# lambdaclass/AES_zero_knowledge_proof_circuit

Measured on AMD Instinct MI355X. Metric: AES-ECB blocks proven/sec (Marlin), proof verifies, higher is better.
Workload: dtype u32 limbs (253-bit Fr / 377-bit Fq modular integers)

## Files before the change

aes_zero_knowledge_proof_circuit_amd/csrc/ff29.cuh:

```cuda
#pragma once
#include "ff.cuh"

namespace zk {

template <class P>
struct Fp29 {
    static constexpr int N = 9;
    static constexpr int B = 29;
    static constexpr uint32_t MASK = (1u << B) - 1;
    uint32_t l[N];

    ZK_HD static constexpr uint32_t mod29(int i) {
        int bit = B * i, w = bit >> 5, sh = bit & 31;
        uint64_t two = (w < P::N ? (uint64_t)P::mod(w) : 0) | ((w + 1 < P::N ? (uint64_t)P::mod(w + 1) : 0) << 32);
        return (uint32_t)(two >> sh) & MASK;
    }
    static constexpr uint32_t PINV = P::INV & MASK;
    template <int K> ZK_HD static constexpr uint32_t kp_limb(int i) {
        uint64_t c = 0, v = 0;
        for (int j = 0; j <= i; j++) { v = (uint64_t)K * mod29(j) + c; c = v >> B; }
        return i == N - 1 ? (uint32_t)v : (uint32_t)v & MASK;
    }
    template <int K> ZK_HD static constexpr uint32_t kp_spread(int i) {
        return i == 0 ? kp_limb<K>(0) + (1u << B) : (i == N - 1 ? kp_limb<K>(i) - 1u : kp_limb<K>(i) + MASK);
// ... 8 lines not shown
            uint64_t two = (k < P::N ? (uint64_t)w[k] : 0) | ((k + 1 < P::N ? (uint64_t)w[k + 1] : 0) << 32);
            r.l[i] = (uint32_t)(two >> sh) & MASK;
        }
        return r;
    }
    ZK_HD void pack(uint32_t *w) const {
#pragma unroll
        for (int k = 0; k < P::N; k++) {
            int bit = 32 * k, i = bit / B, sh = bit % B;
            uint64_t v = (uint64_t)l[i] >> sh;
            int have = B - sh;
            if (i + 1 < N) v |= (uint64_t)l[i + 1] << have;
            if (have + B < 32 && i + 2 < N) v |= (uint64_t)l[i + 2] << (have + B);
            w[k] = (uint32_t)v;
        }
    }
    ZK_HD Fp29 operator+(const Fp29 &b) const {
        Fp29 r;
        uint32_t c = 0;
#pragma unroll
        for (int i = 0; i < N - 1; i++) { uint32_t v = l[i] + b.l[i] + c; r.l[i] = v & MASK; c = v >> B; }
        r.l[N - 1] = l[N - 1] + b.l[N - 1] + c;
        return r;
    }
    template <int K>
    ZK_HD Fp29 sub(const Fp29 &b) const {
        Fp29 r;
        uint32_t c = 0;
#pragma unroll
        for (int i = 0; i < N - 1; i++) { uint32_t v = l[i] + kp_spread<K>(i) - b.l[i] + c; r.l[i] = v & MASK; c = v >> B; }
        r.l[N - 1] = l[N - 1] + kp_spread<K>(N - 1) - b.l[N - 1] + c;
        return r;
    }
    ZK_HD Fp29 add_lazy(const Fp29 &b) const { Fp29 r; for (int i = 0; i < N; i++) r.l[i] = l[i] + b.l[i]; return r; }
    template <int K> ZK_HD Fp29 sub_lazy(const Fp29 &b) const {
        Fp29 r;
#pragma unroll
        for (int i = 0; i < N; i++) {
#if defined(__HIP_DEVICE_COMPILE__)
            if (i < N - 1) { asm("v_sad_u32 %0, %1, %2, %3" : "=v"(r.l[i]) : "s"(kp_spread<K>(i)), "v"(b.l[i]), "v"(l[i])); continue; }
#endif
            r.l[i] = l[i] + kp_spread<K>(i) - b.l[i];
        }
        return r;
    }
    ZK_HD Fp29 normalized() const {
        Fp29 r;
        uint32_t c = 0;
#pragma unroll
        for (int i = 0; i < N - 1; i++) { const uint64_t v = (uint64_t)l[i] + c; r.l[i] = (uint32_t)v & MASK; c = (uint32_t)(v >> B); }
        r.l[N - 1] = l[N - 1] + c;
        return r;
    }
    ZK_HD Fp29 operator*(const Fp29 &b) const {
        uint64_t t[2 * N];
#pragma unroll
        for (int i = 0; i < 2 * N; i++) t[i] = 0;
#pragma unroll
        for (int i = 0; i < N; i++) {
#pragma unroll
            for (int j = 0; j < N; j++) t[i + j] += (uint64_t)l[j] * b.l[i];
            if constexpr (mod29(0) == 1u && PINV == MASK) {
                const uint64_t u = t[i] + MASK;
                const uint32_t m = ~(uint32_t)u & MASK;
#pragma unroll
                for (int j = 1; j < N; j++) t[i + j] += (uint64_t)m * mod29(j);
                t[i + 1] += u >> B;
            } else {
                uint32_t m = (((uint32_t)t[i] & MASK) * PINV) & MASK;
#pragma unroll
                for (int j = 0; j < N; j++) t[i + j] += (uint64_t)m * mod29(j);
                t[i + 1] += t[i] >> B;
            }
        }
        Fp29 r;
        uint64_t c = 0;
#pragma unroll
        for (int i = 0; i < N - 1; i++) { uint64_t v = t[N + i] + c; r.l[i] = (uint32_t)v & MASK; c = v >> B; }
        r.l[N - 1] = (uint32_t)(t[2 * N - 1] + c);
        return r;
    }
    template <int N>
    ZK_HD static Fp29 dot(const Fp29 *a, const Fp29 *b) {
        static_assert(N >= 1 && N <= 4, "column accumulators hold at most four products per limb pair");
        static_assert(mod29(0) == 1u && PINV == MASK, "written for p = 1 (mod 2^29)");
        uint64_t t[2 * Fp29::N];
#pragma unroll
        for (int i = 0; i < 2 * Fp29::N; i++) t[i] = 0;
#pragma unroll
        for (int i = 0; i < Fp29::N; i++) {
#pragma unroll
            for (int n = 0; n < N; n++)
#pragma unroll
                for (int j = 0; j < Fp29::N; j++) t[i + j] += (uint64_t)a[n].l[j] * b[n].l[i];
            const uint64_t u = t[i] + MASK;
            const uint32_t m = ~(uint32_t)u & MASK;
#pragma unroll
            for (int j = 1; j < Fp29::N; j++) t[i + j] += (uint64_t)m * mod29(j);
            t[i + 1] += u >> B;
        }
        Fp29 r;
        uint64_t c = 0;
#pragma unroll
        for (int i = 0; i < Fp29::N - 1; i++) { uint64_t v = t[Fp29::N + i] + c; r.l[i] = (uint32_t)v & MASK; c = v >> B; }
        r.l[Fp29::N - 1] = (uint32_t)(t[2 * Fp29::N - 1] + c);
        return r;
    }
    ZK_HD Fp29 shl5() const {
        Fp29 r;
        r.l[0] = (l[0] << 5) & MASK;
#pragma unroll
        for (int i = 1; i < N; i++) r.l[i] = ((l[i] << 5) | (l[i - 1] >> (B - 5))) & (i == N - 1 ? 0xffffffffu : MASK);
        return r;
    }
    template <int LOG>
    ZK_HD Fp29 canonical() const {
        Fp29 v = *this;
#pragma unroll
        for (int k = LOG; k >= 0; k--) {
            int64_t c = 0;
            uint32_t tl[N];
#pragma unroll
            for (int i = 0; i < N - 1; i++) { int64_t x = (int64_t)v.l[i] - ((int64_t)mod29(i) << k) + c; tl[i] = (uint32_t)x & MASK; c = x >> B; }
            int64_t top = (int64_t)v.l[N - 1] - ((int64_t)mod29(N - 1) << k) + c;
            if (top >= 0) {
#pragma unroll
                for (int i = 0; i < N - 1; i++) v.l[i] = tl[i];
                v.l[N - 1] = (uint32_t)top;
            }
        }
        return v;
    }
    ZK_HD Fp29 reduce_by_top_limb() const {
        constexpr uint32_t RECIP = (uint32_t)((1ull << 32) / ((uint64_t)mod29(N - 1) + 1));
        static_assert(mod29(N - 1) >= (1u << 20), "the estimate's error bound assumes a modulus of at least 253 bits");
        static_assert(P::mod(P::N - 1) < (1u << 31), "the callers pack a remainder < 2 p into 8 x 32-bit words: needs 2 p < 2^256");
#if defined(__HIP_DEVICE_COMPILE__)
        const uint32_t q = __umulhi(l[N - 1], RECIP);
#else
        const uint32_t q = (uint32_t)(((uint64_t)l[N - 1] * RECIP) >> 32);
#endif
        Fp29 r;
        int64_t c = 0;
#pragma unroll
        for (int i = 0; i < N - 1; i++) { const int64_t x = (int64_t)l[i] - (int64_t)((uint64_t)q * mod29(i)) + c; r.l[i] = (uint32_t)x & MASK; c = x >> B; }
        r.l[N - 1] = (uint32_t)((int64_t)l[N - 1] - (int64_t)((uint64_t)q * mod29(N - 1)) + c);
        return r;
    }
    ZK_HD static Fp29 twiddle_from_std(const Fp<P> &w) {
        Fp<P> v = w;
        for (int i = 0; i < 261 - 32 * P::N; i++) v = v.dbl();
        return split(v.l);
    }
    ZK_HD static Fp29 from_std_relimb(const Fp<P> &a) { return split(a.l); }
    template <int LOG> ZK_HD Fp<P> to_std_relimb() const { Fp<P> r; canonical<LOG>().pack(r.l); return r; }
};

}
```

aes_zero_knowledge_proof_circuit_amd/csrc/gpu.hpp:

```cpp
#pragma once
#include <cstddef>
#include <cstdint>
#include <stdexcept>
#include <string>
#include <utility>
#include <vector>
#include "ec.cuh"
#include "te28.cuh"

namespace zk {
namespace gpu {

struct GpuError : std::runtime_error { using std::runtime_error::runtime_error; };
typedef void *stream_t;

int device_count();
void require_device();
int current_device();
void set_device(int ordinal);
void *dmalloc(size_t bytes);
#ifdef ZKAES_MEASURE
int knockin();
#endif
size_t mem_free_bytes();
void dfree(void *p);
void h2d(void *dst, const void *src, size_t bytes, stream_t s);
void d2h(void *dst, const void *src, size_t bytes, stream_t s);
void d2d(void *dst, const void *src, size_t bytes, stream_t s);
void dzero(void *dst, size_t bytes, stream_t s);
void sync(stream_t s);
bool throughput_mode();
struct ThroughputWaits { explicit ThroughputWaits(bool on); ~ThroughputWaits(); ThroughputWaits(const ThroughputWaits &) = delete; ThroughputWaits &operator=(const ThroughputWaits &) = delete; private: bool on_; };
stream_t stream_create();
stream_t stream_create_background();
void stream_destroy(stream_t s);
void *event_create();
void event_record(void *ev, stream_t s);
void stream_wait_event(stream_t s, void *ev);
float event_elapsed_ms(void *start, void *stop);
void event_destroy(void *ev);

void *pinned_alloc(size_t bytes);
void *pinned_device_address(void *host);
void pinned_free(void *host);

template <class T> struct DevElem { static constexpr size_t bytes = sizeof(T); };
template <> struct DevElem<void> { static constexpr size_t bytes = 1; };
template <class T> struct DevPtr {
    T *p = nullptr;
    size_t n = 0;
    DevPtr() = default;
    explicit DevPtr(size_t count) { alloc(count); }
    DevPtr(const DevPtr &) = delete; DevPtr &operator=(const DevPtr &) = delete;
    DevPtr(DevPtr &&o) noexcept : p(o.p), n(o.n) { o.p = nullptr; o.n = 0; }
    DevPtr &operator=(DevPtr &&o) noexcept { if (this != &o) { reset(); p = o.p; n = o.n; o.p = nullptr; o.n = 0; } return *this; }
    ~DevPtr() { dfree(p); }
    void reset() { dfree(p); p = nullptr; n = 0; }
    void alloc(size_t count) { reset(); p = (T *)dmalloc(count * DevElem<T>::bytes); n = count; }
    void grow(size_t count) { if (!p || count > n) alloc(count); }
    T *get() const { return p; }
    operator T *() const { return p; }
};
template <class... T> void grow_together(const size_t (&counts)[sizeof...(T)], DevPtr<T> &...bufs) {
    size_t i = 0;
    if (((bufs.p && counts[i++] <= bufs.n) && ...)) return;
    (bufs.reset(), ...);
    i = 0;
    try { (bufs.alloc(counts[i++]), ...); } catch (...) { (bufs.reset(), ...); throw; }
}
template <class H, H (*Create)(), void (*Destroy)(H)> struct Handle {
    H h = nullptr;
    Handle() : h(Create()) {}
    explicit Handle(H adopt) : h(adopt) {}
    Handle(const Handle &) = delete; Handle &operator=(const Handle &) = delete;
    Handle(Handle &&o) noexcept : h(o.h) { o.h = nullptr; }
    Handle &operator=(Handle &&o) noexcept { if (this != &o) { Destroy(h); h = o.h; o.h = nullptr; } return *this; }
    ~Handle() { Destroy(h); }
    operator H() const { return h; }
};
using StreamGuard = Handle<stream_t, stream_create, stream_destroy>;
using EventGuard = Handle<void *, event_create, event_destroy>;
struct PinnedPtr {
    void *host = nullptr, *dev = nullptr;
    PinnedPtr() = default;
    PinnedPtr(const PinnedPtr &) = delete; PinnedPtr &operator=(const PinnedPtr &) = delete;
    ~PinnedPtr() { pinned_free(host); }
    void alloc(size_t bytes) { pinned_free(host); host = dev = nullptr; host = pinned_alloc(bytes); dev = pinned_device_address(host); }
};

enum : int { OP_MSM_BUCKETS = 0, OP_MSM_SECOND_BASES = 1, OP_MSM_CLASS_SUM = 2 };
struct OpRecord { std::vector<std::pair<uint64_t, int>> ntt , msm ; };
void oplog_begin();
OpRecord oplog_end();
void oplog_ntt(uint64_t n, int count);
void oplog_msm(uint64_t points, int kind);

template <class Fr> void ntt(Fr *dst, const Fr *src, size_t in_len, int lg, bool inverse, stream_t s);
template <class Fr> void ntt_coset(Fr *dst, const Fr *src, size_t in_len, int lg, bool inverse, int coset_c, int lg_big, stream_t s);
template <class Fr> struct NttJob { Fr *dst; const Fr *src; int coset_c; };
template <class Fr> void ntt_batch(const NttJob<Fr> *jobs, int count, size_t in_len, int lg, bool inverse, int lg_big, stream_t s);
template <class Fr> DevPtr<void> coset_power_table(const Fr &g, size_t n, stream_t s);
template <class Fr> void ntt_scaled(Fr *dst, const Fr *src, size_t in_len, int lg, bool inverse, const void *table, stream_t s);
template <class Fr> const Fr *domain_elements(int lg);

struct MsmWorkspace;
MsmWorkspace *msm_workspace_create();
void msm_workspace_destroy(MsmWorkspace *ws);
using WorkspaceGuard = Handle<MsmWorkspace *, msm_workspace_create, msm_workspace_destroy>;
template <class Curve> void convert_bases(Affine28<typename Curve::FqP> *dst, const Affine<typename Curve::Fq> *src, size_t n, stream_t s);
template <class Curve>
XYZZ<typename Curve::Fq> msm(MsmWorkspace *ws, const Affine28<typename Curve::FqP> *bases, const typename Curve::Fr *scalars, size_t n, stream_t s);
template <class Curve>
void msm_prepare(MsmWorkspace *ws, const typename Curve::Fr *scal1, size_t n1, const typename Curve::Fr *scal2, size_t n2, size_t val_off2, stream_t s, int force_c = 0);
template <class Curve>
XYZZ<typename Curve::Fq> msm_finish(MsmWorkspace *ws, const Affine28<typename Curve::FqP> *bases, stream_t s);
template <class Curve> void convert_bases_te(Niels28<typename Curve::FqP> *dst, const Affine<typename Curve::Fq> *src, size_t n, stream_t s);
template <class Curve>
XYZZ<typename Curve::Fq> msm(MsmWorkspace *ws, const Niels28<typename Curve::FqP> *bases, const typename Curve::Fr *scalars, size_t n, stream_t s);
template <class Curve>
XYZZ<typename Curve::Fq> msm_finish(MsmWorkspace *ws, const Niels28<typename Curve::FqP> *bases, stream_t s);
template <class Curve>
void msm_finish2(MsmWorkspace *ws, const Niels28<typename Curve::FqP> *bases, const Niels28<typename Curve::FqP> *bases2, XYZZ<typename Curve::Fq> *out, stream_t s);
template <class Curve>
XYZZ<typename Curve::Fq> msm_table(MsmWorkspace *ws, const Niels28<typename Curve::FqP> *tables, size_t stride, size_t off, int c, const typename Curve::Fr *scalars, size_t n, stream_t s);
template <class Curve>
bool class_sum(MsmWorkspace *ws, const Niels28<typename Curve::FqP> *bases, const int8_t *vals, size_t n, XYZZ<typename Curve::Fq> *out, stream_t s);
template <class Curve> void msm_sharded_plan(size_t n_total, int *window_bits, int *n_windows);
template <class Curve>
void msm_window_sums_device(MsmWorkspace *ws, const Affine28<typename Curve::FqP> *bases, const typename Curve::Fr *scalars, size_t n_local, size_t n_total,
                            XYZZ<typename Curve::Fq> *dev_out, stream_t s);
template <class Curve>
XYZZ<typename Curve::Fq> msm_fold_window_sums_device(const XYZZ<typename Curve::Fq> *dev_in, int world, size_t n_total, stream_t s);
template <class Curve>
void msm_table_sum_device(MsmWorkspace *ws, const Niels28<typename Curve::FqP> *tables, size_t stride, size_t off, int c, const typename Curve::Fr *scalars, size_t n,
                          XYZZ<typename Curve::Fq> *dev_out, stream_t s);
template <class Curve>
XYZZ<typename Curve::Fq> msm_fold_points_device(const XYZZ<typename Curve::Fq> *dev_in, int world, stream_t s);
template <class Curve> int table_windows(int c);
template <class Curve> void build_window_tables(Affine<typename Curve::Fq> *tables, size_t stride, int c, stream_t s);
template <class Curve> void table_next(Affine<typename Curve::Fq> *next, const Affine<typename Curve::Fq> *prev, size_t count, int c, int j, stream_t s);
template <class Curve>
void msm_prepare_table(MsmWorkspace *ws, const typename Curve::Fr *scal1, size_t n1, size_t off1, const typename Curve::Fr *scal2, size_t n2, size_t off2, int c, size_t stride, stream_t s);
template <class Curve>
XYZZ<typename Curve::Fq> msm_table(MsmWorkspace *ws, const Affine28<typename Curve::FqP> *tables, size_t stride, size_t off, int c, const typename Curve::Fr *scalars, size_t n, stream_t s);
template <class Curve>
void fixed_base_powers(Affine<typename Curve::Fq> *out, const Affine<typename Curve::Fq> &base, const typename Curve::Fr &beta, size_t from, size_t count, stream_t s, size_t chunk = 0);
template <class Curve>
void fixed_base_scalars(Affine<typename Curve::Fq> *out, const Affine<typename Curve::Fq> &base, const typename Curve::Fr *scalars, size_t count, stream_t s, size_t chunk = 0);
template <class Curve>
bool class_sum(MsmWorkspace *ws, const Affine28<typename Curve::FqP> *bases, const int8_t *vals, size_t n, XYZZ<typename Curve::Fq> *out, stream_t s);
struct MsmStats { double accumulate_ms = 0; double total_ms = 0; uint64_t points = 0; uint64_t launches = 0; uint64_t pairs = 0; };
MsmStats msm_stats(bool reset);

}
}

namespace zk {
struct G1Compressed;
namespace gpu {
using F = Fr377;

void g1_decompress_check(const G1Compressed *pts, size_t n, Affine<Fq377> *out, uint8_t *status, stream_t s);
void fq_sqrt_batch(const Fq377 *in, size_t n, Fq377 *out, uint8_t *ok, stream_t s);
void public_input_eval(F *out, const F *betas, const uint32_t *bits, size_t words, size_t n, size_t n_bits, int lg_m, const F &gx, stream_t s);

void poly_set_at(F *p, size_t idx, const F &val, stream_t s);
void poly_add_at(F *p, size_t idx, const F &val, stream_t s);
void poly_scale(F *p, const F &sc, size_t n, stream_t s);
void poly_lincomb_n(F *out, size_t n, const F *const *polys, const size_t *lens, const F *scalars, int count, stream_t s);
size_t divide_by_vanishing_scratch(size_t len, size_t m);
void divide_by_vanishing(F *q, F *rem, const F *p, size_t len, size_t m, stream_t s, F *scratch = nullptr, size_t scratch_len = 0);
void divide_by_linear(F *q, const F *p, size_t len, const F &z, F *scratch, size_t scratch_elems, stream_t s);
size_t divide_by_linear_scratch(size_t len);
F poly_eval(const F *p, size_t len, const F &x, F *scratch, stream_t s);
size_t poly_eval_scratch(size_t len);
void poly_eval_multi(const F *const *p, const size_t *len, const F *x, int count, F *out, F *scratch, size_t scratch_elems, stream_t s);
void batch_inverse(F *v, size_t n, const F *post_or_null, stream_t s);
size_t vanishing_quotient_scratch(int lg_n, int ncosets);
void vanishing_quotient_evals(F *const *out, const F *g, int ncosets, const F &a, const F *elems, uint32_t n, int lg_n, F *scratch, size_t scratch_elems, stream_t s);
void f_evals_from_tables(F *out, const F *va, const F *vb, const F *vc, const F &ea, const F &eb, const F &ec, const F *ra, const F *rb, const uint32_t *ri, const uint32_t *ci, size_t k,
                         stream_t s);

void upload_sbox(const uint8_t table[256]);
void aes_trace(uint8_t *trace, size_t trace_stride, const uint8_t *msgs, const uint8_t *keys, uint32_t nproofs, uint32_t nblocks, stream_t s, size_t key_bytes = 16);
void aes_trace_cbc(uint8_t *trace, size_t trace_stride, const uint8_t *msgs, const uint8_t *keys, const uint8_t *ivs, uint32_t nproofs, uint32_t nblocks, stream_t s, size_t key_bytes = 16);
void aes_trace_ctr(uint8_t *trace, size_t trace_stride, const uint8_t *msgs, const uint8_t *keys, const uint8_t *icbs, uint32_t nproofs, uint32_t msg_len, stream_t s, size_t key_bytes = 16);
void aes_trace_gcm(uint8_t *trace, size_t trace_stride, const uint8_t *msgs, const uint8_t *keys, const uint8_t *hdrs, uint32_t nproofs, uint32_t msg_len, uint32_t aad_len, stream_t s, size_t key_bytes = 16);
void ghash_trace(uint8_t *trace, size_t trace_stride, uint32_t nproofs, uint32_t msg_len, uint32_t aad_len, stream_t s, size_t key_bytes = 16);
void key_tag_trace(uint8_t *trace, size_t trace_stride, size_t tag_off, const uint8_t *keys, uint32_t nproofs, uint32_t tag_blocks, stream_t s, size_t key_bytes = 16);
void sha256_trace(uint8_t *trace, size_t trace_stride, size_t digest_off, const uint8_t *msgs, const uint8_t *hdrs, size_t hdr_stride, size_t hin_off, uint32_t nproofs, size_t msg_len, int digest_kind,
                  uint64_t digest_prefix, stream_t s);
void aes_trace_gcm_seg(uint8_t *trace, size_t trace_stride, const uint8_t *msgs, const uint8_t *keys, const uint8_t *hdrs, uint32_t nproofs, int role, uint32_t msg_len, uint32_t aad_len, stream_t s,
                       size_t key_bytes = 16);
void ghash_trace_seg(uint8_t *trace, size_t trace_stride, uint32_t nproofs, int role, uint32_t msg_len, uint32_t aad_len, stream_t s, size_t key_bytes = 16);
void commit_trace(uint8_t *trace, size_t trace_stride, size_t seg_off, size_t yout_off, const uint8_t *keys, size_t key_bytes, const uint8_t *hdrs, size_t hdr_stride, uint32_t nproofs, int role,
                  uint32_t nblocks, stream_t s);
void witness_expand(uint8_t *z, const uint32_t *desc, uint32_t ncols, const uint8_t *trace, const uint32_t *sbox_in_off, const uint32_t *sbox_tmpl, stream_t s);
void spmv_bits(F *out, int8_t *small_out, size_t rows_out, const uint32_t *rowptr, const uint32_t *col, const int64_t *coeff, size_t rows, const uint8_t *z, stream_t s);
void w_classes(int8_t *out, const uint8_t *z, uint32_t n, uint32_t m, uint32_t num_witness, stream_t s);
void lagrange_scalars(F *lag, F *lag_w, const F *elems, const F &beta, uint32_t n, uint32_t m, stream_t s);
void w_evals(F *out, const uint8_t *z, const F *x_evals, uint32_t n, uint32_t m, uint32_t num_witness, stream_t s);
void bits_to_field(F *out, const uint8_t *z, size_t n, stream_t s);
constexpr uint32_t T_SEG = 32, T_HEAVY_SEGMENTS = 256;
void t_evals(F *out, uint32_t n, F *partial, uint32_t nseg, const uint32_t *col_seg_ptr, const uint32_t *seg_start, const uint32_t *seg_end, const uint32_t *heavy, uint32_t n_heavy,
             const uint32_t *row, const uint8_t *mat, const int64_t *coeff, const F *r_alpha, const F &eta_a, const F &eta_b, const F &eta_c, stream_t s);
uint64_t chacha_field_stream(F *out, size_t count, const uint32_t key[8], int rounds, uint64_t word_pos, void *scratch, size_t scratch_bytes, stream_t s, uint32_t max_cand = 0);
void mask_fixup(F *p, size_t n, stream_t s);
void q1_coset_pointwise(F *out, const F *r, const F *za, const F *zb, const F *t, const F *z, const F &ca, const F &cb, const F &cz, const F &eta_a, const F &eta_b, const F &eta_c,
                        size_t n, stream_t s);
void z_evals_h(F *out, const uint8_t *z, uint32_t n, uint32_t m, uint32_t num_witness, stream_t s);
void q1_combine(F *h1, F *g1, const F *q0, const F *q1, const F *q3, const F *mask, const F &inv2, const F &inv2zeta, size_t n, stream_t s);
void coset_scale(F *out, const F *in, const F &g, size_t in_len, size_t n, stream_t s);
void h2_coset(F *out, const F *row, const F *col, const F *va, const F *vb, const F *vc, const F *rc, const F *f, const F &alpha, const F &beta, const F &alpha_beta,
              const F &ea, const F &eb, const F &ec, const F &vinv, size_t k, stream_t s);
void index_evals(F *row, F *col, F *rowcol, F *va, F *vb, F *vc, F *tmp, const uint32_t *ci, const uint32_t *ri, const int64_t *ca, const int64_t *cb, const int64_t *cc, size_t cnt,
                 size_t k, const F *elems, uint32_t n, stream_t s);
void z_poly_from_w(F *zp, const F *w, size_t wlen, const F *x_poly, uint32_t m, size_t n, stream_t s);

}
}
```

aes_zero_knowledge_proof_circuit_amd/csrc/kernels_msm.hip:

```cpp
#include <cstring>
#include <rocprim/device/device_radix_sort.hpp>
#include <rocprim/device/device_scan.hpp>
#include <chrono>
#include <cstdio>
#include <cstdlib>
#include <mutex>
#include <vector>
#include "hip_util.hpp"
#include "te28.cuh"

namespace zk {
namespace gpu {

template <class P> struct WeierLaw { using Params = P; using Base = Affine28<P>; using Acc = Acc28<P>; static constexpr bool edwards = false; };
template <class P> struct EdwardsLaw { using Params = P; using Base = Niels28<P>; using Acc = AccTE<P>; static constexpr bool edwards = true; };

static MsmStats g_stats;
static std::mutex g_stats_mu;
MsmStats msm_stats(bool reset) {
    std::lock_guard<std::mutex> g(g_stats_mu);
    MsmStats s = g_stats;
    if (reset) g_stats = MsmStats();
    return s;
}

constexpr uint32_t VAL_SKIP = 1u << 30, VAL_INDEX = VAL_SKIP - 1;
template <class Fr>
__global__ void k_digits(const Fr *__restrict__ scalars, uint32_t n, uint32_t i_off, uint32_t ntot, uint32_t val_off, int c, int nwin, uint32_t nb,
                         uint32_t *__restrict__ keys, uint32_t *__restrict__ vals) {
    uint32_t i = blockIdx.x * blockDim.x + threadIdx.x;
    if (i >= n) return;
    uint32_t raw[Fr::N + 1];
    scalars[i].to_raw(raw);
    raw[Fr::N] = 0;
    const uint32_t mask = (1u << c) - 1, half = 1u << (c - 1);
    uint32_t carry = 0;
    for (int w = 0; w < nwin; w++) {
        int bit = w * c, limb = bit >> 5, sh = bit & 31;
        uint64_t two = limb <= Fr::N - 1 ? ((uint64_t)raw[limb] | ((uint64_t)raw[limb + 1] << 32)) : 0;
        uint32_t v = ((uint32_t)(two >> sh) & mask) + carry;
        uint32_t neg = 0;
        carry = 0;
        if (v > half) { v = (1u << c) - v; neg = 1u << 31; carry = 1; }
        keys[(size_t)w * ntot + i_off + i] = ((uint32_t)w << (c - 1)) | (v ? v - 1 : 0u);
        vals[(size_t)w * ntot + i_off + i] = v ? ((val_off + i) | neg) : VAL_SKIP;
    }
}

struct TableLayout {
    int nwin, c_hi, n_hi;
    __host__ __device__ int width(int j) const { return j < n_hi ? c_hi : c_hi - 1; }
    __host__ __device__ int offset(int j) const { return j < n_hi ? j * c_hi : n_hi * c_hi + (j - n_hi) * (c_hi - 1); }
};
static TableLayout table_layout(int total_bits, int c) {
    TableLayout L;
    L.nwin = (total_bits + c - 1) / c;
    int base = total_bits / L.nwin, rem = total_bits % L.nwin;
    L.c_hi = base + (rem ? 1 : 0);
    L.n_hi = rem ? rem : L.nwin;
    return L;
}
template <class Fr>
__global__ void k_digits_table(const Fr *__restrict__ scalars, uint32_t n, uint32_t i_off, uint32_t ntot, uint32_t val_off, TableLayout L, uint32_t stride,
                               uint32_t *__restrict__ keys, uint32_t *__restrict__ vals) {
    uint32_t i = blockIdx.x * blockDim.x + threadIdx.x;
    if (i >= n) return;
    uint32_t raw[Fr::N + 1];
    scalars[i].to_raw(raw);
    raw[Fr::N] = 0;
    uint32_t carry = 0;
    for (int w = 0; w < L.nwin; w++) {
        const int c = L.width(w), bit = L.offset(w), limb = bit >> 5, sh = bit & 31;
        const uint32_t mask = (1u << c) - 1, half = 1u << (c - 1);
        uint64_t two = limb <= Fr::N - 1 ? ((uint64_t)raw[limb] | ((uint64_t)raw[limb + 1] << 32)) : 0;
        uint32_t v = ((uint32_t)(two >> sh) & mask) + carry;
        uint32_t neg = 0;
        carry = 0;
        if (v > half) { v = (1u << c) - v; neg = 1u << 31; carry = 1; }
        keys[(size_t)w * ntot + i_off + i] = v ? v - 1 : 0u;
        vals[(size_t)w * ntot + i_off + i] = v ? (((uint32_t)w * stride + val_off + i) | neg) : VAL_SKIP;
    }
}
template <class Fq>
__global__ void __launch_bounds__(64) k_table_next(const Affine<Fq> *__restrict__ prev, Affine<Fq> *__restrict__ next, uint32_t count, int c) {
    constexpr int B = 8;
    uint32_t t = blockIdx.x * blockDim.x + threadIdx.x;
    uint32_t s0 = t * B;
    if (s0 >= count) return;
    uint32_t e = s0 + B < count ? s0 + B : count;
    Fq xs[B], ys[B], zz[B], zzz[B], pre[B];
    Fq acc = Fq::one();
    for (uint32_t i = s0; i < e; i++) {
        XYZZ<Fq> p = XYZZ<Fq>::from_affine(prev[i]);
        for (int k = 0; k < c; k++) p = p.dbl();
        xs[i - s0] = p.x; ys[i - s0] = p.y; zz[i - s0] = p.zz; zzz[i - s0] = p.zzz;
        pre[i - s0] = acc;
        if (!p.zzz.is_zero()) acc = acc * p.zzz;
    }
    acc = acc.inverse();
    for (uint32_t i = e; i-- > s0;) {
        uint32_t q = i - s0;
        if (zzz[q].is_zero()) { next[i] = Affine<Fq>::inf(); continue; }
        Fq zi3 = acc * pre[q];
        acc = acc * zzz[q];
        Fq zi2 = (zi3 * zz[q]).sqr();
        Affine<Fq> a; a.x = xs[q] * zi2; a.y = ys[q] * zi3;
        next[i] = a;
    }
}

__device__ __forceinline__ uint32_t bounds_rank(uint32_t key, int cbits, uint32_t nwin) { return nwin == 1 ? key : (key & ((1u << cbits) - 1)) * nwin + (key >> cbits); }
__device__ __forceinline__ uint32_t bounds_key(uint32_t rank, int cbits, uint32_t nwin) { return nwin == 1 ? rank : ((rank % nwin) << cbits) | (rank / nwin); }
__global__ void k_bounds(const uint32_t *__restrict__ keys, size_t total, int cbits, uint32_t nwin, uint32_t *__restrict__ start, uint32_t *__restrict__ end) {
    size_t i0 = ((size_t)blockIdx.x * blockDim.x + threadIdx.x) * 4;
    if (i0 >= total) return;
    const uint32_t nb = nwin << cbits;
    uint32_t k[6];
    if (i0 + 4 <= total) { uint4 v = *reinterpret_cast<const uint4 *>(keys + i0); k[1] = v.x; k[2] = v.y; k[3] = v.z; k[4] = v.w; }
    else { for (int j = 0; j < 4; j++) k[1 + j] = i0 + j < total ? keys[i0 + j] : 0u; }
    k[0] = i0 ? keys[i0 - 1] : 0u;
    k[5] = i0 + 4 < total ? keys[i0 + 4] : 0u;
#pragma unroll
    for (int j = 0; j < 4; j++) {
        size_t i = i0 + j;
        if (i >= total) break;
        const uint32_t key = k[1 + j];
        if (i == 0 || k[j] != key) {
            const uint32_t r1 = bounds_rank(key, cbits, nwin);
            uint32_t r0 = 0;
            if (i != 0) { end[k[j]] = (uint32_t)i; r0 = bounds_rank(k[j], cbits, nwin) + 1; }
            for (uint32_t r = r0; r < r1; r++) { const uint32_t g = bounds_key(r, cbits, nwin); start[g] = (uint32_t)i; end[g] = (uint32_t)i; }
            start[key] = (uint32_t)i;
        }
        if (i + 1 == total) {
            end[key] = (uint32_t)total;
            for (uint32_t r = bounds_rank(key, cbits, nwin) + 1; r < nb; r++) { const uint32_t g = bounds_key(r, cbits, nwin); start[g] = (uint32_t)total; end[g] = (uint32_t)total; }
        }
    }
}

template <class P>
__global__ void k_convert_bases(const Affine<Fp<P>> *__restrict__ src, Affine28<P> *__restrict__ dst, size_t n) {
    size_t i = (size_t)blockIdx.x * blockDim.x + threadIdx.x;
    if (i < n) dst[i] = Affine28<P>::from_std(src[i]);
}

constexpr uint32_t BUCKET_CAP = 2048, BUCKET_CAP_TABLE = 512;
constexpr uint32_t NO_SLOT = 0xffffffffu;

constexpr int ORD_BINS = 1024, ORD_THREADS = 256, ORD_MAX_BLOCKS = 128;
__device__ __forceinline__ uint32_t order_key(uint32_t sz) { return (ORD_BINS - 1) - (sz > ORD_BINS - 1 ? ORD_BINS - 1 : sz); }
__global__ void __launch_bounds__(ORD_THREADS) k_order_hist(const uint32_t *__restrict__ start, const uint32_t *__restrict__ end, uint32_t nb, uint32_t per_block, uint32_t cap,
                                                             uint32_t *__restrict__ ovf_slot, uint32_t *__restrict__ ovf_bucket, uint32_t *__restrict__ ovf_nseg, uint32_t ovf_cap,
                                                             uint32_t *__restrict__ ctrl, uint32_t *__restrict__ hist) {
    __shared__ uint32_t h[ORD_BINS];
    for (int b = threadIdx.x; b < ORD_BINS; b += ORD_THREADS) h[b] = 0;
    __syncthreads();
    const uint32_t lo = blockIdx.x * per_block, hi = lo + per_block < nb ? lo + per_block : nb;
    for (uint32_t k = lo + threadIdx.x; k < hi; k += ORD_THREADS) {
        const uint32_t sz = end[k] - start[k];
        uint32_t slot = NO_SLOT;
        if (sz > cap) {
// ... 211 lines not shown
    } else {
        if (threadIdx.x != 0) return;
        accumulate_fixup<P>(bases, buckets, deferred, deferred_cap, deferred_count);
    }
}
template <class A>
__global__ void __launch_bounds__(64) k_fold_overflow(A *__restrict__ buckets, const uint32_t *__restrict__ ctrl, const uint32_t *__restrict__ ovf_bucket, const uint32_t *__restrict__ ovf_off,
                                                       uint32_t max_segments, const A *__restrict__ partial) {
    const uint32_t q = blockIdx.x * blockDim.x + threadIdx.x;
    if (q >= ctrl[1]) return;
    uint32_t a = ovf_off[q], b = ovf_off[q + 1];
    if (b > max_segments) b = max_segments;
    if (a >= b) return;
    const uint32_t k = ovf_bucket[q];
    A acc = buckets[k];
    for (uint32_t w = a / 64; w * 64 < b; w++) { uint32_t i = w * 64 > a ? w * 64 : a; if (i < b) PtOps<A>::add(acc, partial[i]); }
    buckets[k] = acc;
}

constexpr int RED_L1 = 8, RED_L2 = 8;
template <class A>
__global__ void __launch_bounds__(64) k_reduce_l1(const A *__restrict__ buckets, int c, int nwin, A *__restrict__ seg_s, A *__restrict__ seg_w) {
    uint32_t segs = (1u << c) / RED_L1;
    uint32_t t = blockIdx.x * blockDim.x + threadIdx.x;
    if (t >= segs * (uint32_t)nwin) return;
    uint32_t w = t / segs, g = t % segs;
    const size_t k0 = ((size_t)w << c) + (size_t)g * RED_L1;
    A run = buckets[k0 + RED_L1 - 1], tot = run;
    for (int d = RED_L1 - 2; d >= 0; d--) {
        A b = buckets[k0 + d];
        if (d != RED_L1 - 2) PtOps<A>::add_inline(tot, run);
        PtOps<A>::add_inline(run, b);
    }
    PtOps<A>::add(tot, run);
    seg_s[t] = run;
    seg_w[t] = tot;
}
template <class A>
__global__ void __launch_bounds__(64) k_reduce_l1_pair(const A *__restrict__ buckets, int c, int nwin, A *__restrict__ seg_s, A *__restrict__ seg_w) {
    using P = typename PtOps<A>::Params;
    using G = FpMsm<P>;
    const uint32_t segs = (1u << c) / RED_L1;
    const uint32_t t = blockIdx.x * blockDim.x + threadIdx.x, seg = t >> 1;
    const bool odd = t & 1;
    if (seg >= segs * (uint32_t)nwin) return;
    const uint32_t w = seg / segs, g = seg % segs;
    const size_t k0 = ((size_t)w << c) + g;
    A acc = odd ? PtOps<A>::identity() : buckets[k0 + (size_t)(RED_L1 - 1) * segs];
    for (int d = RED_L1 - 2; d >= 0; d--) {
        A opnd;
        opnd.x = quad_move<QP_SWAP_PAIRS, G>(acc.x); opnd.y = quad_move<QP_SWAP_PAIRS, G>(acc.y); opnd.z = quad_move<QP_SWAP_PAIRS, G>(acc.z); opnd.t = quad_move<QP_SWAP_PAIRS, G>(acc.t);
        if (!odd) opnd = buckets[k0 + (size_t)d * segs];
        PtOps<A>::add_inline(acc, opnd);
    }
    (odd ? seg_w : seg_s)[seg] = acc;
}
template <class A>
__global__ void __launch_bounds__(64) k_reduce_l2(const A *__restrict__ seg_s, const A *__restrict__ seg_w, int c, int nwin, A *__restrict__ partial) {
    uint32_t segs = (1u << c) / RED_L1, groups = (segs + RED_L2 - 1) / RED_L2;
    const uint32_t role = blockIdx.x & 1;
    uint32_t t = (blockIdx.x >> 1) * blockDim.x + threadIdx.x;
    if (t >= groups * (uint32_t)nwin) return;
    uint32_t w = t / groups, h = t % groups;
    uint32_t g0 = h * RED_L2, g1 = g0 + RED_L2 < segs ? g0 + RED_L2 : segs;
    const A *S = seg_s + (size_t)w * segs, *W = seg_w + (size_t)w * segs;
    A *out = partial + (size_t)w * 2 * groups + 2 * h + role;
    if (role == 0) {
        A run = PtOps<A>::identity(), tot2 = PtOps<A>::identity(), sw = PtOps<A>::identity();
        for (int g = (int)g1 - 1; g >= (int)g0; g--) {
            PtOps<A>::add(run, S[g]);
            PtOps<A>::add(tot2, run);
            PtOps<A>::add(sw, W[g]);
        }
        A a = tot2;
        PtOps<A>::add(a, PtOps<A>::neg(run));
        for (int i = 0; i < 3; i++) PtOps<A>::dbl(a);
        PtOps<A>::add(sw, a);
        *out = sw;
    } else {
        A acc = PtOps<A>::identity();
        if (g0 != 0) {
            A run = PtOps<A>::identity();
            for (int g = (int)g1 - 1; g >= (int)g0; g--) PtOps<A>::add(run, S[g]);
            uint32_t m = RED_L1 * g0;
            int top = 31 - __clz(m);
            for (int bit = top; bit >= 0; bit--) {
                PtOps<A>::dbl(acc);
                if ((m >> bit) & 1) PtOps<A>::add(acc, run);
            }
        }
        *out = acc;
    }
}

template <class A>
__global__ void __launch_bounds__(256) k_reduce_window(const A *__restrict__ partial, uint32_t per_window, XYZZ<Fp<typename PtOps<A>::Params>> *__restrict__ out,
                                                        XYZZ<Fp<typename PtOps<A>::Params>> *__restrict__ out2) {
    __shared__ A sh[256];
    uint32_t w = blockIdx.x, t = threadIdx.x;
    A acc = PtOps<A>::identity();
    for (uint32_t i = t; i < per_window; i += 256) PtOps<A>::add(acc, partial[(size_t)w * per_window + i]);
    sh[t] = acc;
    __syncthreads();
    int s0 = 128;
    while (s0 >= 1 && (uint32_t)s0 >= per_window) s0 >>= 1;
    for (int s = s0; s > 0; s >>= 1) {
        if ((int)t < s) { A a = sh[t]; PtOps<A>::add(a, sh[t + s]); sh[t] = a; }
        __syncthreads();
    }
    if (t == 0) {
        const auto r = PtOps<A>::to_std(sh[0]);
        out[w] = r;
        if (out2) out2[w] = r;
    }
}

constexpr int RQ_THREADS = 256, RQ_QUADS = RQ_THREADS / 4;
constexpr int PT_WORDS = 4 * FpMsm<Fq377P>::N;
template <class P> __device__ __forceinline__ FpMsm<P> quad_load(const uint32_t *pt, int q) {
    FpMsm<P> r;
#pragma unroll
    for (int i = 0; i < FpMsm<P>::N; i++) r.l[i] = pt[q * FpMsm<P>::N + i];
    return r;
}
template <class P> __device__ __forceinline__ void quad_store(uint32_t *pt, int q, const FpMsm<P> &v) {
#pragma unroll
    for (int i = 0; i < FpMsm<P>::N; i++) pt[q * FpMsm<P>::N + i] = v.l[i];
}
template <class P>
__device__ __forceinline__ void quad_tree_sum(uint32_t *pt, uint32_t count, uint32_t quad, int q) {
    for (uint32_t half = count >> 1; half >= 1; half >>= 1) {
        if (quad < half) quad_store<P>(pt + quad * PT_WORDS, q, te_add_quad<P>(quad_load<P>(pt + quad * PT_WORDS, q), quad_load<P>(pt + (quad + half) * PT_WORDS, q), q));
        __syncthreads();
    }
}
template <class P>
__global__ void __launch_bounds__(RQ_THREADS) k_reduce_rc(const AccTE<P> *__restrict__ seg_s, const AccTE<P> *__restrict__ seg_w, int lgR, int lgC, AccTE<P> *__restrict__ out) {
    __shared__ uint32_t pt[RQ_QUADS * PT_WORDS];
    const uint32_t R = 1u << lgR, C = 1u << lgC, jobs = 2 * R + C;
    const uint32_t set = blockIdx.x / jobs, job = blockIdx.x % jobs, quad = threadIdx.x >> 2;
    const int q = threadIdx.x & 3;
    const AccTE<P> *src = (job < R ? seg_w : seg_s) + ((size_t)set << (lgR + lgC));
    uint32_t first, stride, len;
    if (job < 2 * R) { first = (job < R ? job : job - R) << lgC; stride = 1; len = C; }
    else { first = job - 2 * R; stride = C; len = R; }
    FpMsm<P> acc = te_identity_quad<P>(q);
    for (uint32_t i = quad; i < len; i += RQ_QUADS)
        acc = te_add_quad<P>(acc, quad_load<P>(reinterpret_cast<const uint32_t *>(src + first + (size_t)i * stride), q), q);
    quad_store<P>(pt + quad * PT_WORDS, q, acc);
    __syncthreads();
    quad_tree_sum<P>(pt, RQ_QUADS, quad, q);
    if (quad == 0) quad_store<P>(reinterpret_cast<uint32_t *>(out + (size_t)set * jobs + job), q, quad_load<P>(pt, q));
}
ZK_HD int quad_weighted_lc(uint32_t M) { int m = 0; while ((1u << m) < M) m++; return M <= 16 ? m : (m + 1) / 2; }
constexpr int RF_OUT = 6;
constexpr int RT_THREADS = 256, RT_QUADS = RT_THREADS / 4;
constexpr int RT_PLANES = RT_QUADS, RT_IDENT = RT_QUADS + 32, RT_SLOTS = RT_IDENT + 1;
__device__ __forceinline__ uint32_t rt_plane_member(uint32_t b, uint32_t i) {
    const uint32_t lo = i & ((1u << b) - 1), hi = i >> b;
    return (hi << (b + 1)) | (1u << b) | lo;
}
template <class P>
__global__ void __launch_bounds__(RT_THREADS) k_reduce_terms(const AccTE<P> *__restrict__ rc, int lgR, int lgC, AccTE<P> *__restrict__ part, XYZZ<Fp<P>> *__restrict__ out, bool to_host) {
    __shared__ uint32_t pt[RT_SLOTS * PT_WORDS];
    const uint32_t R = 1u << lgR, C = 1u << lgC, jobs = 2 * R + C;
    const uint32_t set = blockIdx.x / RF_OUT, term = blockIdx.x % RF_OUT, quad = threadIdx.x >> 2;
    const int q = threadIdx.x & 3;
    const bool plain = term < 2, second = term & 1;
    const AccTE<P> *src = rc + (size_t)set * jobs + (term == 0 ? 0 : (term == 2 || term == 3) ? 2 * R : R);
    const uint32_t M = (term == 2 || term == 3) ? C : R;
    uint32_t first = 0, stride = 0, count = 0;
    if (plain) { first = quad; stride = RT_QUADS; count = quad < M ? (M - quad + RT_QUADS - 1) / RT_QUADS : 0; }
    else {
        const int lc = quad_weighted_lc(M);
        const uint32_t c1 = 1u << lc, r1 = M >> lc, G = second ? r1 : c1, S = second ? c1 : r1, g = quad >> 2, p = quad & 3;
        if (g < G && p < S) { count = (S - p + 3) / 4; first = second ? g * c1 + p : p * c1 + g; stride = second ? 4 : 4 * c1; }
    }
    FpMsm<P> acc = te_identity_quad<P>(q);
    for (uint32_t i = 0; i < count; i++) acc = te_add_quad<P>(acc, quad_load<P>(reinterpret_cast<const uint32_t *>(src + first + (size_t)i * stride), q), q);
    quad_store<P>(pt + quad * PT_WORDS, q, acc);
    if (quad == 0) quad_store<P>(pt + RT_IDENT * PT_WORDS, q, te_identity_quad<P>(q));
    __syncthreads();
    const int nsteps = plain ? 6 : 11;
    for (int step = 0; step < nsteps; step++) {
        bool active = false;
        uint32_t dst = 0, a = 0, b = 0;
        if (plain) { const uint32_t half = (RT_QUADS / 2) >> step; active = quad < half; dst = a = quad; b = quad + half; }
        else if (step == 0) { active = (quad & 3) < 2; dst = a = quad; b = quad + 2; }
        else if (step == 1) { active = (quad & 3) == 0; dst = a = quad; b = quad + 1; }
        else if (step == 2) { active = quad < 16; const uint32_t pl = quad >> 2, j = quad & 3; dst = RT_PLANES + 8 * pl + j; a = 4 * rt_plane_member(pl, 2 * j); b = 4 * rt_plane_member(pl, 2 * j + 1); }
        else if (step == 3) { active = quad < 8; const uint32_t pl = quad >> 1, j = quad & 1; dst = a = RT_PLANES + 8 * pl + j; b = a + 2; }
        else if (step == 4) { active = quad < 4; dst = a = RT_PLANES + 8 * quad; b = a + 1; }
        else { active = quad == 0; dst = a = RT_PLANES + 24; const int h = step - 5; b = (h & 1) ? RT_PLANES + 8 * (2 - h / 2) : a; }
        if (active) quad_store<P>(pt + dst * PT_WORDS, q, te_add_quad<P>(quad_load<P>(pt + a * PT_WORDS, q), quad_load<P>(pt + b * PT_WORDS, q), q));
        __syncthreads();
    }
    const uint32_t *res = pt + (plain ? 0 : RT_PLANES + 24) * PT_WORDS;
    if (to_host) { if (threadIdx.x == 0) out[(size_t)set * RF_OUT + term] = te_to_std_point<P>(*reinterpret_cast<const AccTE<P> *>(res)); }
    else if (quad == 0) quad_store<P>(reinterpret_cast<uint32_t *>(part + (size_t)set * RF_OUT + term), q, quad_load<P>(res, q));
}
template <class P>
__global__ void __launch_bounds__(64) k_reduce_combine(const AccTE<P> *__restrict__ part, int lgR, int lgC, XYZZ<Fp<P>> *__restrict__ out, XYZZ<Fp<P>> *__restrict__ dev_total) {
    __shared__ uint32_t pt[RF_OUT * PT_WORDS];
    __shared__ uint8_t prog[64][3];
    __shared__ int nprog;
    const uint32_t set = blockIdx.x, quad = threadIdx.x >> 2;
    const int q = threadIdx.x & 3;
    if (quad < RF_OUT) quad_store<P>(pt + quad * PT_WORDS, q, quad_load<P>(reinterpret_cast<const uint32_t *>(part + (size_t)set * RF_OUT + quad), q));
    if (threadIdx.x == 0) {
        int n = 0;
        auto op = [&](int d, int a, int b) { prog[n][0] = (uint8_t)d; prog[n][1] = (uint8_t)a; prog[n][2] = (uint8_t)b; n++; };
        const int lcC = quad_weighted_lc(1u << lgC), lcR = quad_weighted_lc(1u << lgR);
        for (int i = 0; i < lcR; i++) op(5, 5, 5);
        op(5, 5, 4);
        for (int i = 0; i < lcC; i++) op(3, 3, 3);
        op(3, 3, 2);
        for (int i = 0; i < lgR; i++) op(0, 0, 0);
        op(0, 0, 5);
        for (int i = 0; i < lgC; i++) op(0, 0, 0);
        op(0, 0, 3); op(0, 0, 1);
        nprog = n;
    }
    __syncthreads();
    const int n = nprog;
    for (int i = 0; i < n; i++) {
        const FpMsm<P> v = te_add_quad<P>(quad_load<P>(pt + prog[i][1] * PT_WORDS, q), quad_load<P>(pt + prog[i][2] * PT_WORDS, q), q);
        __syncthreads();
        if (quad == 0) quad_store<P>(pt + prog[i][0] * PT_WORDS, q, v);
        __syncthreads();
    }
    if (threadIdx.x == 0) {
        const auto r = te_to_std_point<P>(*reinterpret_cast<const AccTE<P> *>(pt));
        out[set] = r;
        if (dev_total) dev_total[set] = r;
    }
}
template <class Fq>
static XYZZ<Fq> reduce_host_tail(const XYZZ<Fq> *o, int lgR, int lgC) {
    auto shl = [](XYZZ<Fq> v, int k) { for (int i = 0; i < k; i++) v = v.dbl(); return v; };
    const int lcC = quad_weighted_lc(1u << lgC), lcR = quad_weighted_lc(1u << lgR);
    XYZZ<Fq> row = shl(o[5], lcR);
    row.add(o[4]);
    XYZZ<Fq> col = shl(o[3], lcC);
    col.add(o[2]);
    XYZZ<Fq> t = shl(o[0], lgR);
    t.add(row);
    t = shl(t, lgC);
    t.add(col);
    t.add(o[1]);
    return t;
}

template <class A> __global__ void k_sum_tree(const A *__restrict__ in, uint32_t total, uint32_t per, A *__restrict__ out, uint32_t in_stride, uint32_t out_stride);

constexpr uint32_t DEFERRED_CAP = 1u << 20;
constexpr size_t ACC_BYTES = sizeof(Acc28<Fq377P>);
static_assert(sizeof(Acc28<Fq381P>) == ACC_BYTES, "bucket size differs between the curves");
static_assert(sizeof(AccTE<Fq377P>) == ACC_BYTES, "the Edwards accumulator must fit the XYZZ bucket slots");
constexpr int MAX_WSUMS = 64;
struct MsmWorkspace {
    DevPtr<uint32_t> keys_a, keys_b, vals_a, vals_b;
    uint32_t *sorted_keys = nullptr, *sorted_vals = nullptr;
    DevPtr<uint32_t> start, end, order, ovf_slot;
    DevPtr<uint32_t> ovf_bucket, ovf_nseg, ovf_off; DevPtr<void> ovf_partial;
    DevPtr<uint32_t> part_hist, part_offs;
    DevPtr<uint32_t> canon;
    DevPtr<void> buckets, seg_s, seg_w, partial;
    DevPtr<void> tmp;
    bool ctrl_dirty = false;
    size_t plan_n = 0, plan_pairs = 0; int plan_c = 0, plan_nwin = 0;
    bool plan_table = false; uint32_t plan_cap = BUCKET_CAP;
    EventGuard ev[4] = {EventGuard(nullptr), EventGuard(nullptr), EventGuard(nullptr), EventGuard(nullptr)};
    DevPtr<uint32_t> deferred, deferred_count;
    DevPtr<uint32_t> ord_hist, ord_offs;
    DevPtr<uint32_t> ctrl;
    PinnedPtr h_res;
};
constexpr size_t RES_BYTES = 192 * MAX_WSUMS * 6 + 64;
static void ensure_result(MsmWorkspace &S, size_t buckets) {
    grow_together({buckets * ACC_BYTES, (buckets / RED_L1 + 64) * ACC_BYTES, (buckets / RED_L1 + 64) * ACC_BYTES, (2 * (buckets / (RED_L1 * RED_L2)) + 2 * 64 * 64) * ACC_BYTES},
                  S.buckets, S.seg_s, S.seg_w, S.partial);
}
static void ensure_scratch(MsmWorkspace &S, size_t pairs, size_t buckets, size_t cap) {
    if (cap == 0) cap = BUCKET_CAP;
    if (!S.h_res.dev) {
        for (auto &e : S.ev) e = EventGuard();
        S.deferred.alloc(2 * DEFERRED_CAP); S.deferred_count.alloc(2);
        HIP_CHECK(hipMemset(S.deferred_count, 0, 8));
        S.ord_hist.alloc((size_t)ORD_BINS * ORD_MAX_BLOCKS); S.ord_offs.alloc((size_t)ORD_BINS * ORD_MAX_BLOCKS);
        S.ctrl.alloc(8);
        HIP_CHECK(hipMemset(S.ctrl, 0, 32));
        S.h_res.alloc(RES_BYTES);
    }
    const size_t ovf = pairs / cap + 64;
    grow_together({2 * ovf * ACC_BYTES , ovf, ovf, ovf + 1}, S.ovf_partial, S.ovf_bucket, S.ovf_nseg, S.ovf_off);
    grow_together({pairs, pairs, pairs, pairs}, S.keys_a, S.keys_b, S.vals_a, S.vals_b);
    grow_together({buckets, buckets, buckets, buckets}, S.start, S.end, S.order, S.ovf_slot);
    ensure_result(S, buckets);
}
MsmWorkspace *msm_workspace_create() { return new MsmWorkspace(); }
void msm_workspace_destroy(MsmWorkspace *w) { delete w; }

static void order_buckets(MsmWorkspace &S, size_t nb, uint32_t cap, hipStream_t s) {
    if (S.ctrl_dirty) HIP_CHECK(hipMemsetAsync(S.ctrl, 0, 8, s));
    S.ctrl_dirty = true;
    unsigned nblk = (unsigned)((nb + 4095) / 4096);
    if (nblk > (unsigned)ORD_MAX_BLOCKS) nblk = ORD_MAX_BLOCKS;
    if (nblk < 1) nblk = 1;
    const uint32_t per_block = (uint32_t)((nb + nblk - 1) / nblk);
    hipLaunchKernelGGL(k_order_hist, dim3(nblk), dim3(ORD_THREADS), 0, s, S.start, S.end, (uint32_t)nb, per_block, cap, S.ovf_slot, S.ovf_bucket, S.ovf_nseg, (uint32_t)S.ovf_bucket.n - 1, S.ctrl, S.ord_hist);
    HIP_LAUNCH_CHECK();
    hipLaunchKernelGGL(k_order_scan, dim3(1), dim3(ORD_BINS), 0, s, S.ord_hist, S.ord_offs, nblk, S.ctrl, S.ovf_nseg, S.ovf_off, (uint32_t)S.ovf_bucket.n - 1);
    HIP_LAUNCH_CHECK();
    hipLaunchKernelGGL(k_order_scatter, dim3(nblk), dim3(ORD_THREADS), 0, s, S.start, S.end, (uint32_t)nb, per_block, S.ord_offs, S.order);
    HIP_LAUNCH_CHECK();
    S.ctrl_dirty = false;
}

template <class P>
static void prepare_buckets(MsmWorkspace &S, size_t pairs, int c, int nsets, int sort_bits, uint32_t cap, hipStream_t s, int begin_bit = 0) {
    size_t nb = (size_t)nsets << c;
    int key_bits = 1;
    while (((size_t)1 << key_bits) < nb) key_bits++;
    if (sort_bits > 0 && sort_bits < key_bits) key_bits = sort_bits;
    size_t tmp_bytes = 0;
    rocprim::double_buffer<uint32_t> dk(S.keys_a, S.keys_b), dv(S.vals_a, S.vals_b);
    HIP_CHECK(rocprim::radix_sort_pairs(nullptr, tmp_bytes, dk, dv, pairs, (unsigned)begin_bit, (unsigned)key_bits, s));
    S.tmp.grow(tmp_bytes);
    HIP_CHECK(rocprim::radix_sort_pairs(S.tmp.p, tmp_bytes, dk, dv, pairs, (unsigned)begin_bit, (unsigned)key_bits, s));
#ifdef ZKAES_MEASURE
    if (knockin() & 1) HIP_CHECK(rocprim::radix_sort_pairs(S.tmp.p, tmp_bytes, dk, dv, pairs, (unsigned)begin_bit, (unsigned)key_bits, s));
#endif
    S.sorted_keys = dk.current(); S.sorted_vals = dv.current();
    hipLaunchKernelGGL(k_bounds, dim3((unsigned)(((pairs + 3) / 4 + 255) / 256)), dim3(256), 0, s, S.sorted_keys, pairs, c, (uint32_t)nsets, S.start, S.end);
    HIP_LAUNCH_CHECK();
    order_buckets(S, nb, cap, s);
}
template <class Law>
static std::vector<XYZZ<Fp<typename Law::Params>>> run_buckets(MsmWorkspace &S, const typename Law::Base *bases, size_t pairs, int c, int nsets_one, size_t n_points, uint32_t cap, hipStream_t s, float *acc_ms,
                                            XYZZ<Fp<typename Law::Params>> *dev_wsum_out = nullptr, const typename Law::Base *bases2 = nullptr) {
    using P = typename Law::Params;
    using A = typename Law::Acc;
    using Fq = Fp<P>;
    const int nrep = bases2 ? 2 : 1, nsets = nsets_one * nrep;
    if (bases2 && !Law::edwards) throw GpuError("msm: two base arrays per prepared state need the Edwards law");
    if (nsets > MAX_WSUMS) throw GpuError("msm: too many windows");
    const size_t nb = (size_t)nsets_one << c;
    ensure_result(S, nb * nrep);
    if constexpr (!Law::edwards) HIP_CHECK(hipMemsetAsync(S.deferred_count, 0, 8, s));
#ifdef ZKAES_MEASURE
    if (knockin() & 8) {
        hipLaunchKernelGGL((k_accumulate<Law>), dim3((unsigned)((nb + 63) / 64)), dim3(64), 0, s, bases, S.sorted_vals, S.start, S.end, S.order, (uint32_t)nb, cap,
                           (A *)S.buckets.p, S.deferred, DEFERRED_CAP, S.deferred_count);
        if constexpr (!Law::edwards) HIP_CHECK(hipMemsetAsync(S.deferred_count, 0, 8, s));
    }
#endif
    uint32_t max_seg = (uint32_t)(pairs / cap + 1);
    for (int rep = 0; rep < nrep; rep++) {
        const typename Law::Base *src = rep ? bases2 : bases;
        HIP_CHECK(hipEventRecord((hipEvent_t)S.ev[2 * rep].h, s));
        hipLaunchKernelGGL((k_accumulate<Law>), dim3((unsigned)((nb + 63) / 64)), dim3(64), 0, s, src, S.sorted_vals, S.start, S.end, S.order, (uint32_t)nb, cap,
                           (A *)S.buckets.p + rep * nb, S.deferred, DEFERRED_CAP, S.deferred_count);
        HIP_LAUNCH_CHECK();
        HIP_CHECK(hipEventRecord((hipEvent_t)S.ev[2 * rep + 1].h, s));
        hipLaunchKernelGGL((k_accumulate_tail<Law>), dim3((max_seg + 63) / 64), dim3(64), 0, s, src, S.sorted_vals, S.start, S.end, S.ctrl, S.ovf_bucket, S.ovf_off, max_seg, cap,
                           (A *)S.ovf_partial.p + rep * S.ovf_bucket.n, (A *)S.buckets.p + rep * nb, S.deferred, DEFERRED_CAP, S.deferred_count);
        HIP_LAUNCH_CHECK();
    }
    if constexpr (!Law::edwards) for (int rep = 0; rep < nrep; rep++) {
        hipLaunchKernelGGL((k_fold_overflow<A>), dim3((max_seg + 63) / 64), dim3(64), 0, s, (A *)S.buckets.p + rep * nb, S.ctrl, S.ovf_bucket, S.ovf_off, max_seg, (const A *)S.ovf_partial.p + rep * S.ovf_bucket.n);
        HIP_LAUNCH_CHECK();
    }
    XYZZ<Fq> *res = (XYZZ<Fq> *)S.h_res.dev;
    uint32_t segs = (1u << c) / RED_L1, groups = (segs + RED_L2 - 1) / RED_L2;
    [[maybe_unused]] int te_lgR = 0, te_lgC = 0;
    [[maybe_unused]] bool te_host_tail = false;
#ifdef ZKAES_MEASURE
    for (int rep = (knockin() & 2) ? 0 : 1; rep < 2; rep++)
#endif
    {
    if constexpr (Law::edwards)
        hipLaunchKernelGGL((k_reduce_l1_pair<A>), dim3((unsigned)((2 * segs * nsets + 63) / 64)), dim3(64), 0, s, (const A *)S.buckets.p, c, nsets, (A *)S.seg_s.p, (A *)S.seg_w.p);
    else
        hipLaunchKernelGGL((k_reduce_l1<A>), dim3((unsigned)((segs * nsets + 63) / 64)), dim3(64), 0, s, (const A *)S.buckets.p, c, nsets, (A *)S.seg_s.p, (A *)S.seg_w.p);
    HIP_LAUNCH_CHECK();
    if constexpr (Law::edwards) {
        const int lgG = c - 3 > 0 ? c - 3 : 0, lgC = (lgG + 1) / 2, lgR = lgG - lgC;
        if (lgC > 8) throw GpuError("msm: more than 2^19 buckets per set");
        const unsigned jobs = 2u * (1u << lgR) + (1u << lgC);
        A *rc = (A *)S.partial.p, *part = rc + (size_t)nsets * jobs;
        hipLaunchKernelGGL((k_reduce_rc<P>), dim3((unsigned)nsets * jobs), dim3(RQ_THREADS), 0, s, (const A *)S.seg_s.p, (const A *)S.seg_w.p, lgR, lgC, rc);
        HIP_LAUNCH_CHECK();
        te_host_tail = !dev_wsum_out && nsets <= 4;
        hipLaunchKernelGGL((k_reduce_terms<P>), dim3((unsigned)(RF_OUT * nsets)), dim3(RT_THREADS), 0, s, (const A *)rc, lgR, lgC, part, res, te_host_tail);
        HIP_LAUNCH_CHECK();
        if (!te_host_tail) {
            hipLaunchKernelGGL((k_reduce_combine<P>), dim3((unsigned)nsets), dim3(64), 0, s, (const A *)part, lgR, lgC, res, dev_wsum_out);
            HIP_LAUNCH_CHECK();
        }
        te_lgR = lgR; te_lgC = lgC;
    } else {
    hipLaunchKernelGGL((k_reduce_l2<A>), dim3(2u * (unsigned)((groups * nsets + 63) / 64)), dim3(64), 0, s, (const A *)S.seg_s.p, (const A *)S.seg_w.p, c, nsets, (A *)S.partial.p);
    HIP_LAUNCH_CHECK();
    const uint32_t parts = 2 * groups;
    if (nsets == 1 && parts > 2048) {
        uint32_t mid = (parts + 255) / 256;
        hipLaunchKernelGGL((k_sum_tree<A>), dim3(mid), dim3(256), 0, s, (const A *)S.partial.p, parts, 256u, (A *)S.seg_s.p, 0u, 0u);
        HIP_LAUNCH_CHECK();
        hipLaunchKernelGGL((k_reduce_window<A>), dim3(1), dim3(256), 0, s, (const A *)S.seg_s.p, mid, res, dev_wsum_out);
    } else {
        hipLaunchKernelGGL((k_reduce_window<A>), dim3((unsigned)nsets), dim3(256), 0, s, (const A *)S.partial.p, parts, res, dev_wsum_out);
    }
    HIP_LAUNCH_CHECK();
    }
    }
    std::vector<XYZZ<Fq>> ws(nsets);
    uint32_t n_deferred = 0;
    sync((stream_t)s);
    if (Law::edwards && te_host_tail) {
        std::vector<XYZZ<Fq>> terms((size_t)nsets * RF_OUT);
        memcpy(terms.data(), S.h_res.host, sizeof(XYZZ<Fq>) * terms.size());
        for (int i = 0; i < nsets; i++) ws[i] = reduce_host_tail<Fq>(terms.data() + (size_t)i * RF_OUT, te_lgR, te_lgC);
    } else memcpy(ws.data(), S.h_res.host, sizeof(XYZZ<Fq>) * nsets);
    if constexpr (!Law::edwards) {
        HIP_CHECK(hipMemcpyAsync(&n_deferred, S.deferred_count, 4, hipMemcpyDeviceToHost, s));
        sync((stream_t)s);
        if (n_deferred > DEFERRED_CAP) throw GpuError("msm: more than 2^20 degenerate additions (repeated base points); refusing to return a wrong sum");
    }
    for (int rep = 0; rep < nrep; rep++) HIP_CHECK(hipEventElapsedTime(acc_ms + rep, (hipEvent_t)S.ev[2 * rep].h, (hipEvent_t)S.ev[2 * rep + 1].h));
    (void)n_points;
    return ws;
}
static void add_stats(const float *acc_ms, int launches, size_t n, size_t pairs, std::chrono::steady_clock::time_point t_begin) {
    std::lock_guard<std::mutex> g(g_stats_mu);
    for (int i = 0; i < launches; i++) g_stats.accumulate_ms += acc_ms[i];
    g_stats.points += n * (size_t)launches;
    g_stats.pairs += pairs * (size_t)launches;
    g_stats.launches += (uint64_t)launches;
    g_stats.total_ms += std::chrono::duration<double, std::milli>(std::chrono::steady_clock::now() - t_begin).count();
}

__global__ void __launch_bounds__(64) k_convert_bases_te(const Affine<Fq377> *__restrict__ src, Niels28<Fq377P> *__restrict__ dst, size_t n, uint32_t *__restrict__ bad) {
    constexpr int B = 8;
    size_t s0 = ((size_t)blockIdx.x * blockDim.x + threadIdx.x) * B;
    if (s0 >= n) return;
    size_t e = s0 + B < n ? s0 + B : n;
    TeMapParts m[B];
    Fq377 pre[B];
    bool skip[B];
    Fq377 acc = Fq377::one();
    for (size_t i = s0; i < e; i++) {
        Affine<Fq377> p = src[i];
        int q = (int)(i - s0);
        skip[q] = p.is_inf();
        if (!skip[q]) {
            m[q] = te_map_parts(p);
            if (m[q].den.is_zero()) { skip[q] = true; atomicOr(bad, 1u); }
        }
        pre[q] = acc;
        if (!skip[q]) acc = acc * m[q].den;
    }
    acc = acc.inverse();
    for (size_t i = e; i-- > s0;) {
        int q = (int)(i - s0);
        if (skip[q]) { dst[i] = niels_identity<Fq377P>(); continue; }
        Fq377 inv = acc * pre[q];
        acc = acc * m[q].den;
        dst[i] = te_niels_finish(m[q], inv);
    }
}
template <class Curve>
void convert_bases_te(Niels28<typename Curve::FqP> *dst, const Affine<typename Curve::Fq> *src, size_t n, stream_t s_) {
    static_assert(Curve::ID == 377, "only BLS12-377's G1 has a twisted Edwards model");
    if (!n) return;
    hipStream_t s = (hipStream_t)s_;
    DevPtr<uint32_t> d_bad(1);
    uint32_t h_bad = 0;
    HIP_CHECK(hipMemsetAsync(d_bad, 0, 4, s));
    size_t lanes = (n + 7) / 8;
    hipLaunchKernelGGL(k_convert_bases_te, dim3((unsigned)((lanes + 63) / 64)), dim3(64), 0, s, src, dst, n, d_bad.get());
    HIP_LAUNCH_CHECK();
    sync((stream_t)s);
    HIP_CHECK(hipMemcpyAsync(&h_bad, d_bad, 4, hipMemcpyDeviceToHost, s));
    sync((stream_t)s);
    if (h_bad) throw GpuError("convert_bases_te: a base point has order 2 or 4 -- the Edwards path needs points of the prime-order subgroup");
}
template void convert_bases_te<Bls377>(Niels28<Fq377P> *, const Affine<Fq377> *, size_t, stream_t);

template <class Curve>
void convert_bases(Affine28<typename Curve::FqP> *dst, const Affine<typename Curve::Fq> *src, size_t n, stream_t s_) {
    if (!n) return;
    hipLaunchKernelGGL((k_convert_bases<typename Curve::FqP>), dim3((unsigned)((n + 255) / 256)), dim3(256), 0, (hipStream_t)s_, src, dst, n);
    HIP_LAUNCH_CHECK();
}

template <class Curve>
void msm_prepare(MsmWorkspace *ws_, const typename Curve::Fr *scal1, size_t n1, const typename Curve::Fr *scal2, size_t n2, size_t val_off2, stream_t s_, int force_c) {
    using Fr = typename Curve::Fr;
    hipStream_t s = (hipStream_t)s_;
    if (!ws_) throw GpuError("msm: null workspace");
    MsmWorkspace &S = *ws_;
    size_t n = n1 + n2;
    S.plan_n = n;
    if (n == 0) return;
    if (n >= (1u << 30) || val_off2 + n2 >= (1u << 30)) throw GpuError("msm: too many points");
    int lg = 0;
    while (((size_t)1 << lg) < n) lg++;
    int c = lg - 2;
    if (c < 7) c = 7;
    if (c > 17) c = 17;
    if (force_c >= 4 && force_c <= 22) c = force_c;
    const int nwin = (Fr::BITS + 1 + c - 1) / c;
    size_t pairs = n * (size_t)nwin;
    if (pairs >= ((size_t)1 << 31)) throw GpuError("msm: n x windows exceeds the 2^31 pairs the sort indexes with int");
    const size_t nb = (size_t)nwin << (c - 1);
    S.plan_c = c; S.plan_nwin = nwin; S.plan_pairs = pairs; S.plan_table = false; S.plan_cap = BUCKET_CAP;
    ensure_scratch(S, pairs, nb, BUCKET_CAP);
    if (n1) { hipLaunchKernelGGL((k_digits<Fr>), dim3((unsigned)((n1 + 255) / 256)), dim3(256), 0, s, scal1, (uint32_t)n1, 0u, (uint32_t)n, 0u, c, nwin, (uint32_t)nb, S.keys_a, S.vals_a); HIP_LAUNCH_CHECK(); }
    if (n2) { hipLaunchKernelGGL((k_digits<Fr>), dim3((unsigned)((n2 + 255) / 256)), dim3(256), 0, s, scal2, (uint32_t)n2, (uint32_t)n1, (uint32_t)n, (uint32_t)val_off2, c, nwin, (uint32_t)nb, S.keys_a, S.vals_a); HIP_LAUNCH_CHECK(); }
    prepare_buckets<typename Curve::FqP>(S, pairs, c - 1, nwin, c - 1, BUCKET_CAP, s);
}
template <class Curve, class Law>
static XYZZ<typename Curve::Fq> msm_finish_impl(MsmWorkspace *ws_, const typename Law::Base *bases, stream_t s_, const typename Law::Base *bases2 = nullptr,
                                                XYZZ<typename Curve::Fq> *out2 = nullptr) {
    using Fq = typename Curve::Fq;
    static_assert(sizeof(XYZZ<Fq>) == 192, "XYZZ layout");
    hipStream_t s = (hipStream_t)s_;
    if (!ws_) throw GpuError("msm: null workspace");
    MsmWorkspace &S = *ws_;
    if (out2) *out2 = XYZZ<Fq>::inf();
    if (S.plan_n == 0) return XYZZ<Fq>::inf();
    auto t_begin = std::chrono::steady_clock::now();
    const int c = S.plan_c, nwin = S.plan_nwin;
    oplog_msm(S.plan_n, OP_MSM_BUCKETS);
    if (bases2) oplog_msm(S.plan_n, OP_MSM_SECOND_BASES);
    float ms[2] = {0, 0};
    if (S.plan_table) {
        std::vector<XYZZ<Fq>> one = run_buckets<Law>(S, bases, S.plan_pairs, c - 1, 1, S.plan_n, S.plan_cap, s, ms, nullptr, bases2);
        add_stats(ms, bases2 ? 2 : 1, S.plan_n, S.plan_pairs, t_begin);
        if (bases2) *out2 = one[1];
        return one[0];
    }
    if (bases2 && 2 * nwin > MAX_WSUMS) {
        *out2 = msm_finish_impl<Curve, Law>(ws_, bases2, s_);
// ... 64 lines not shown
        sync((stream_t)s);
        return;
    }
    msm_prepare<Curve>(ws_, scalars, n_local, nullptr, 0, 0, s_, c);
    MsmWorkspace &S = *ws_;
    if (S.plan_nwin != nwin) throw GpuError("msm_window_sums_device: window plan mismatch");
    float ms = 0;
    auto t_begin = std::chrono::steady_clock::now();
    oplog_msm(n_local, OP_MSM_BUCKETS);
    run_buckets<WeierLaw<typename Curve::FqP>>(S, bases, S.plan_pairs, c - 1, nwin, n_local, S.plan_cap, s, &ms, dev_out);
    add_stats(&ms, 1, n_local, S.plan_pairs, t_begin);
}
template <class Fq>
__global__ void k_fold_ranks(const XYZZ<Fq> *__restrict__ in, int world, int nwin, XYZZ<Fq> *__restrict__ out) {
    int w = blockIdx.x * blockDim.x + threadIdx.x;
    if (w >= nwin) return;
    XYZZ<Fq> acc = in[w];
    for (int r = 1; r < world; r++) acc.add(in[(size_t)r * nwin + w]);
    out[w] = acc;
}
template <class Curve>
XYZZ<typename Curve::Fq> msm_fold_window_sums_device(const XYZZ<typename Curve::Fq> *dev_in, int world, size_t n_total, stream_t s_) {
    using Fq = typename Curve::Fq;
    hipStream_t s = (hipStream_t)s_;
    int c, nwin;
    msm_sharded_plan<Curve>(n_total, &c, &nwin);
    DevPtr<XYZZ<Fq>> d_out((size_t)nwin);
    hipLaunchKernelGGL((k_fold_ranks<Fq>), dim3(1), dim3(64), 0, s, dev_in, world, nwin, d_out.get());
    HIP_LAUNCH_CHECK();
    std::vector<XYZZ<Fq>> ws(nwin);
    sync((stream_t)s);
    HIP_CHECK(hipMemcpyAsync(ws.data(), d_out, sizeof(XYZZ<Fq>) * nwin, hipMemcpyDeviceToHost, s));
    sync((stream_t)s);
    XYZZ<Fq> total = XYZZ<Fq>::inf();
    for (int w = nwin - 1; w >= 1; w--) {
        total.add(ws[w]);
        for (int k = 0; k < c; k++) total = total.dbl();
    }
    total.add(ws[0]);
    return total;
}

template <class Curve>
void msm_table_sum_device(MsmWorkspace *ws_, const Niels28<typename Curve::FqP> *tables, size_t stride, size_t off, int c, const typename Curve::Fr *scalars, size_t n,
                          XYZZ<typename Curve::Fq> *dev_out, stream_t s_) {
    using Fq = typename Curve::Fq;
    hipStream_t s = (hipStream_t)s_;
    if (n == 0) {
        HIP_CHECK(hipMemsetAsync(dev_out, 0, sizeof(XYZZ<Fq>), s));
        sync((stream_t)s);
        return;
    }
    msm_prepare_table<Curve>(ws_, scalars, n, off, nullptr, 0, 0, c, stride, s_);
    MsmWorkspace &S = *ws_;
    float ms = 0;
    auto t_begin = std::chrono::steady_clock::now();
    oplog_msm(n, OP_MSM_BUCKETS);
    run_buckets<EdwardsLaw<typename Curve::FqP>>(S, tables, S.plan_pairs, S.plan_c - 1, 1, n, S.plan_cap, s, &ms, dev_out);
    add_stats(&ms, 1, n, S.plan_pairs, t_begin);
}
template <class Curve>
XYZZ<typename Curve::Fq> msm_fold_points_device(const XYZZ<typename Curve::Fq> *dev_in, int world, stream_t s_) {
    using Fq = typename Curve::Fq;
    hipStream_t s = (hipStream_t)s_;
    DevPtr<XYZZ<Fq>> d_out(1);
    hipLaunchKernelGGL((k_fold_ranks<Fq>), dim3(1), dim3(64), 0, s, dev_in, world, 1, d_out.get());
    HIP_LAUNCH_CHECK();
    XYZZ<Fq> r;
    sync((stream_t)s);
    HIP_CHECK(hipMemcpyAsync(&r, d_out, sizeof r, hipMemcpyDeviceToHost, s));
    sync((stream_t)s);
    return r;
}

template <class Curve>
int table_windows(int c) { return table_layout(Curve::Fr::BITS + 1, c).nwin; }

template <class Curve>
void build_window_tables(Affine<typename Curve::Fq> *tables, size_t stride, int c, stream_t s_) {
    using Fq = typename Curve::Fq;
    hipStream_t s = (hipStream_t)s_;
    const TableLayout L = table_layout(Curve::Fr::BITS + 1, c);
    for (int j = 1; j < L.nwin; j++) {
        uint32_t lanes = (uint32_t)((stride + 7) / 8);
        hipLaunchKernelGGL((k_table_next<Fq>), dim3((lanes + 63) / 64), dim3(64), 0, s, tables + (size_t)(j - 1) * stride, tables + (size_t)j * stride, (uint32_t)stride, L.width(j - 1));
        HIP_LAUNCH_CHECK();
    }
    sync((stream_t)s);
}

template <class Curve>
void table_next(Affine<typename Curve::Fq> *next, const Affine<typename Curve::Fq> *prev, size_t count, int c, int j, stream_t s_) {
    const TableLayout L = table_layout(Curve::Fr::BITS + 1, c);
    if (j < 1 || j >= L.nwin) throw GpuError("table_next: window index out of range");
    uint32_t lanes = (uint32_t)((count + 7) / 8);
    hipLaunchKernelGGL((k_table_next<typename Curve::Fq>), dim3((lanes + 63) / 64), dim3(64), 0, (hipStream_t)s_, prev, next, (uint32_t)count, L.width(j - 1));
    HIP_LAUNCH_CHECK();
}

constexpr int PART_FINE_BITS = 9, PART_FINE = 1 << PART_FINE_BITS, PART_WBITS = 4, PART_KEYS = PART_FINE << PART_WBITS;
constexpr int PART_THREADS = 512, PART_SPT = 2, PART_TILE = PART_THREADS * PART_SPT;
constexpr int PART_MAXW = 1 << PART_WBITS;
constexpr int PART_STAGE = PART_TILE * PART_MAXW;
constexpr uint32_t PART_NBIN_MAX = 1024;
constexpr uint32_t PART_GRID = 512, PART_NONE = 0xffffffffu;
constexpr int PART_FINE_THREADS = 1024, PART_FINE_UNROLL = 8;

template <int NW>
__device__ __forceinline__ void part_digits(const uint32_t (&raw)[NW + 1], const TableLayout &L, uint32_t d[PART_MAXW]) {
    uint32_t carry = 0;
#pragma unroll
    for (int w = 0; w < PART_MAXW; w++) {
        d[w] = PART_NONE;
        if (w < L.nwin) {
            const int c = L.width(w), bit = L.offset(w), limb = bit >> 5, sh = bit & 31;
            const uint32_t mask = (1u << c) - 1, half = 1u << (c - 1);
            uint64_t two = limb <= NW - 1 ? ((uint64_t)raw[limb] | ((uint64_t)raw[limb + 1] << 32)) : 0;
            uint32_t v = ((uint32_t)(two >> sh) & mask) + carry;
            uint32_t neg = 0;
            carry = 0;
            if (v > half) { v = (1u << c) - v; neg = 1u << 31; carry = 1; }
            if (v) d[w] = (v - 1) | neg;
        }
    }
}
template <int THREADS>
__device__ __forceinline__ void part_block_scan(uint32_t *cnt, uint32_t len, uint32_t *wave_sums, uint32_t *total_out) {
    const uint32_t per = len / THREADS, t = threadIdx.x, base = t * per;
    uint32_t sum = 0;
    for (uint32_t i = 0; i < per; i++) sum += cnt[base + i];
    uint32_t incl = sum;
    for (int d = 1; d < 64; d <<= 1) { uint32_t v = __shfl_up(incl, d, 64); if ((int)(t & 63) >= d) incl += v; }
    if ((t & 63) == 63) wave_sums[t >> 6] = incl;
    __syncthreads();
    uint32_t run = incl - sum;
    for (uint32_t w = 0; w < (t >> 6); w++) run += wave_sums[w];
    for (uint32_t i = 0; i < per; i++) { const uint32_t c = cnt[base + i]; cnt[base + i] = run; run += c; }
    if (t == THREADS - 1) *total_out = run;
    __syncthreads();
}
template <class Fr>
__global__ void __launch_bounds__(PART_THREADS) k_part_hist(const Fr *__restrict__ s1, uint32_t n1, const Fr *__restrict__ s2, uint32_t n2, TableLayout L, uint32_t nbin,
                                                            uint32_t *__restrict__ canon, uint32_t *__restrict__ hist) {
    __shared__ uint32_t sh[PART_NBIN_MAX];
    for (uint32_t b = threadIdx.x; b < nbin; b += PART_THREADS) sh[b] = 0;
    __syncthreads();
    const uint32_t n = n1 + n2, ntiles = (n + PART_TILE - 1) / PART_TILE, per_wg = (ntiles + gridDim.x - 1) / gridDim.x;
    const uint32_t tile_lo = blockIdx.x * per_wg, tile_hi = tile_lo + per_wg < ntiles ? tile_lo + per_wg : ntiles;
    for (uint32_t tile = tile_lo; tile < tile_hi; tile++)
        for (int q = 0; q < PART_SPT; q++) {
            const uint32_t g = tile * PART_TILE + q * PART_THREADS + threadIdx.x;
            if (g >= n) continue;
            uint32_t d[PART_MAXW], raw[Fr::N + 1];
            (g < n1 ? s1[g] : s2[g - n1]).to_raw(raw);
            raw[Fr::N] = 0;
            part_digits<Fr::N>(raw, L, d);
#pragma unroll
            for (int w = 0; w < PART_MAXW; w++) if (d[w] != PART_NONE) atomicAdd(&sh[(d[w] & 0x7fffffffu) >> PART_FINE_BITS], 1u);
            static_assert(Fr::N == 8, "the canonical scalar is stored as two 16-byte words");
            uint4 *dst = reinterpret_cast<uint4 *>(canon + (size_t)g * Fr::N);
            dst[0] = make_uint4(raw[0], raw[1], raw[2], raw[3]); dst[1] = make_uint4(raw[4], raw[5], raw[6], raw[7]);
        }
    __syncthreads();
    for (uint32_t b = threadIdx.x; b < nbin; b += PART_THREADS) hist[(size_t)b * gridDim.x + blockIdx.x] = sh[b];
    if (blockIdx.x == 0 && threadIdx.x == 0) hist[(size_t)nbin * gridDim.x] = 0;
}
template <int NW>
__global__ void __launch_bounds__(PART_THREADS) k_part_scatter(const uint32_t *__restrict__ canon, uint32_t n, uint32_t n1, TableLayout L, uint32_t off1, uint32_t off2, uint32_t stride,
                                                               uint32_t nbin, const uint32_t *__restrict__ offs, uint32_t *__restrict__ out_val, uint16_t *__restrict__ out_key) {
    __shared__ uint32_t cursor[PART_NBIN_MAX], cnt[PART_NBIN_MAX], fill[PART_NBIN_MAX], st_val[PART_STAGE], st_key[PART_STAGE];
    __shared__ uint32_t wave_sums[PART_THREADS / 64], total;
    for (uint32_t b = threadIdx.x; b < nbin; b += PART_THREADS) cursor[b] = offs[(size_t)b * gridDim.x + blockIdx.x];
    const uint32_t ntiles = (n + PART_TILE - 1) / PART_TILE, per_wg = (ntiles + gridDim.x - 1) / gridDim.x;
    const uint32_t tile_lo = blockIdx.x * per_wg, tile_hi = tile_lo + per_wg < ntiles ? tile_lo + per_wg : ntiles;
    for (uint32_t tile = tile_lo; tile < tile_hi; tile++) {
        for (uint32_t b = threadIdx.x; b < PART_NBIN_MAX; b += PART_THREADS) { cnt[b] = 0; fill[b] = 0; }
        __syncthreads();
        uint32_t d[PART_SPT][PART_MAXW];
#pragma unroll
        for (int q = 0; q < PART_SPT; q++) {
            const uint32_t g = tile * PART_TILE + q * PART_THREADS + threadIdx.x;
            if (g < n) {
                uint32_t raw[NW + 1];
                const uint4 *src = reinterpret_cast<const uint4 *>(canon + (size_t)g * NW);
                const uint4 a = src[0], b = src[1];
                raw[0] = a.x; raw[1] = a.y; raw[2] = a.z; raw[3] = a.w; raw[4] = b.x; raw[5] = b.y; raw[6] = b.z; raw[7] = b.w; raw[NW] = 0;
                part_digits<NW>(raw, L, d[q]);
            } else {
#pragma unroll
                for (int w = 0; w < PART_MAXW; w++) d[q][w] = PART_NONE;
            }
#pragma unroll
            for (int w = 0; w < PART_MAXW; w++) if (d[q][w] != PART_NONE) atomicAdd(&cnt[(d[q][w] & 0x7fffffffu) >> PART_FINE_BITS], 1u);
        }
        __syncthreads();
        part_block_scan<PART_THREADS>(cnt, PART_NBIN_MAX, wave_sums, &total);
#pragma unroll
        for (int q = 0; q < PART_SPT; q++) {
            const uint32_t g = tile * PART_TILE + q * PART_THREADS + threadIdx.x;
            const uint32_t base = g < n1 ? off1 + g : off2 + (g - n1);
#pragma unroll
            for (int w = 0; w < PART_MAXW; w++) {
                if (d[q][w] == PART_NONE) continue;
                const uint32_t bucket = d[q][w] & 0x7fffffffu, bin = bucket >> PART_FINE_BITS;
                const uint32_t e = cnt[bin] + atomicAdd(&fill[bin], 1u);
                st_val[e] = ((uint32_t)w * stride + base) | (d[q][w] & 0x80000000u);
                st_key[e] = bucket | ((uint32_t)w << 20);
            }
        }
        __syncthreads();
        const uint32_t tot = total;
        for (uint32_t e = threadIdx.x; e < tot; e += PART_THREADS) {
            const uint32_t key = st_key[e], bucket = key & 0xfffffu, bin = bucket >> PART_FINE_BITS, dst = cursor[bin] + (e - cnt[bin]);
            out_val[dst] = st_val[e];
            out_key[dst] = (uint16_t)(((bucket & (PART_FINE - 1)) << PART_WBITS) | (key >> 20));
        }
        __syncthreads();
        for (uint32_t b = threadIdx.x; b < nbin; b += PART_THREADS) cursor[b] += fill[b];
        __syncthreads();
    }
}
constexpr uint32_t PART_FINE_STAGE = 30720;
__global__ void __launch_bounds__(PART_FINE_THREADS) k_part_fine(const uint32_t *__restrict__ offs, uint32_t grid_a, const uint32_t *__restrict__ in_val, const uint16_t *__restrict__ in_key,
                                                                 uint32_t *__restrict__ out_val, uint32_t *__restrict__ start, uint32_t *__restrict__ end) {
    __shared__ uint32_t cur[PART_KEYS], stage[PART_FINE_STAGE], wave_sums[PART_FINE_THREADS / 64], total, split_key;
    const uint32_t bin = blockIdx.x, t = threadIdx.x;
    const uint32_t lo = offs[(size_t)bin * grid_a], hi = offs[(size_t)(bin + 1) * grid_a];
    for (uint32_t f = t; f < PART_KEYS; f += PART_FINE_THREADS) cur[f] = 0;
    __syncthreads();
    for (uint32_t e0 = lo + t; e0 < hi; e0 += PART_FINE_THREADS * PART_FINE_UNROLL) {
        uint32_t key[PART_FINE_UNROLL];
#pragma unroll
        for (int u = 0; u < PART_FINE_UNROLL; u++) { const uint32_t e = e0 + u * PART_FINE_THREADS; key[u] = e < hi ? in_key[e] : PART_NONE; }
#pragma unroll
        for (int u = 0; u < PART_FINE_UNROLL; u++) if (key[u] != PART_NONE) atomicAdd(&cur[key[u]], 1u);
    }
    __syncthreads();
    part_block_scan<PART_FINE_THREADS>(cur, PART_KEYS, wave_sums, &total);
    for (uint32_t f = t; f < PART_FINE; f += PART_FINE_THREADS) {
        const uint32_t k = bin * PART_FINE + f;
        start[k] = lo + cur[f << PART_WBITS];
        end[k] = lo + (f + 1 < PART_FINE ? cur[(f + 1) << PART_WBITS] : total);
    }
    __syncthreads();
    const uint32_t tot = total;
    uint32_t k_lo = 0, base = 0;
    while (base < tot) {
        const uint32_t lim = base + PART_FINE_STAGE;
        if (tot <= lim) { if (t == 0) split_key = PART_KEYS; }
        else for (uint32_t f = k_lo + t; f < PART_KEYS; f += PART_FINE_THREADS) {
            const uint32_t e_f = f + 1 < PART_KEYS ? cur[f + 1] : tot;
            if (cur[f] <= lim && e_f > lim) split_key = f;
        }
        __syncthreads();
        uint32_t k_hi = split_key;
        const bool direct = k_hi == k_lo;
        if (direct) k_hi = k_lo + 1;
        const uint32_t stop = k_hi < PART_KEYS ? cur[k_hi] : tot;
        __syncthreads();
        for (uint32_t e0 = lo + t; e0 < hi; e0 += PART_FINE_THREADS * PART_FINE_UNROLL) {
            uint32_t key[PART_FINE_UNROLL], val[PART_FINE_UNROLL];
#pragma unroll
            for (int u = 0; u < PART_FINE_UNROLL; u++) {
                const uint32_t e = e0 + u * PART_FINE_THREADS;
                key[u] = PART_NONE;
                if (e < hi) { key[u] = in_key[e]; val[u] = in_val[e]; }
            }
#pragma unroll
            for (int u = 0; u < PART_FINE_UNROLL; u++) if (key[u] >= k_lo && key[u] < k_hi) {
                const uint32_t pos = atomicAdd(&cur[key[u]], 1u);
                if (direct) out_val[lo + pos] = val[u]; else stage[pos - base] = val[u];
            }
        }
        __syncthreads();
        if (!direct) for (uint32_t i = t; i < stop - base; i += PART_FINE_THREADS) out_val[lo + base + i] = stage[i];
        __syncthreads();
        base = stop; k_lo = k_hi;
    }
}
template <class Fr>
static void partition_buckets(MsmWorkspace &S, const Fr *scal1, size_t n1, size_t off1, const Fr *scal2, size_t n2, size_t off2, const TableLayout &L, size_t stride, uint32_t cap, hipStream_t s) {
    const int B = L.c_hi - 1;
    const uint32_t nbin = 1u << (B - PART_FINE_BITS), G = PART_GRID;
    const size_t n = n1 + n2, nb = (size_t)1 << B, nh = (size_t)nbin * G + 1;
    S.canon.grow(n * Fr::N);
    grow_together({nh, nh}, S.part_hist, S.part_offs);
#ifdef ZKAES_MEASURE
    for (int rep = (knockin() & 1) ? 0 : 1; rep < 2; rep++)
#endif
    {
    hipLaunchKernelGGL((k_part_hist<Fr>), dim3(G), dim3(PART_THREADS), 0, s, scal1, (uint32_t)n1, scal2, (uint32_t)n2, L, nbin, S.canon, S.part_hist);
    HIP_LAUNCH_CHECK();
    size_t tb = 0;
    HIP_CHECK(rocprim::exclusive_scan(nullptr, tb, S.part_hist.p, S.part_offs.p, 0u, nh, rocprim::plus<uint32_t>(), s));
    S.tmp.grow(tb);
    HIP_CHECK(rocprim::exclusive_scan(S.tmp.p, tb, S.part_hist.p, S.part_offs.p, 0u, nh, rocprim::plus<uint32_t>(), s));
    hipLaunchKernelGGL((k_part_scatter<Fr::N>), dim3(G), dim3(PART_THREADS), 0, s, (const uint32_t *)S.canon, (uint32_t)n, (uint32_t)n1, L, (uint32_t)off1, (uint32_t)off2, (uint32_t)stride, nbin,
                       (const uint32_t *)S.part_offs, S.vals_a, (uint16_t *)S.keys_a.p);
    HIP_LAUNCH_CHECK();
    hipLaunchKernelGGL(k_part_fine, dim3(nbin), dim3(PART_FINE_THREADS), 0, s, (const uint32_t *)S.part_offs, G, (const uint32_t *)S.vals_a, (const uint16_t *)S.keys_a.p, S.vals_b, S.start, S.end);
    HIP_LAUNCH_CHECK();
    }
    S.sorted_vals = S.vals_b; S.sorted_keys = nullptr;
    order_buckets(S, nb, cap, s);
}

template <class Curve>
// ... 290 lines not shown
```

aes_zero_knowledge_proof_circuit_amd/csrc/kernels_poly.hip:

```cpp
#include <cstring>
#include <rocprim/device/device_scan.hpp>
#include "ff29.cuh"
#include "hip_util.hpp"

namespace zk {
namespace gpu {

#define GRID(n) dim3((unsigned)(((n) + 255) / 256)), dim3(256)

__global__ void k_set_at(F *p, size_t idx, F val, bool add) { if (threadIdx.x == 0 && blockIdx.x == 0) p[idx] = add ? p[idx] + val : val; }
void poly_set_at(F *p, size_t idx, const F &val, stream_t s) { hipLaunchKernelGGL(k_set_at, dim3(1), dim3(64), 0, (hipStream_t)s, p, idx, val, false); HIP_LAUNCH_CHECK(); }
void poly_add_at(F *p, size_t idx, const F &val, stream_t s) { hipLaunchKernelGGL(k_set_at, dim3(1), dim3(64), 0, (hipStream_t)s, p, idx, val, true); HIP_LAUNCH_CHECK(); }

__global__ void k_scale(F *p, F sc, size_t n) { size_t i = (size_t)blockIdx.x * blockDim.x + threadIdx.x; if (i < n) p[i] = p[i] * sc; }
void poly_scale(F *p, const F &sc, size_t n, stream_t s) { if (!n) return; hipLaunchKernelGGL(k_scale, GRID(n), 0, (hipStream_t)s, p, sc, n); HIP_LAUNCH_CHECK(); }
using G29 = Fp29<Fr377P>;
__device__ __forceinline__ G29 ld29(const F &x) { return G29::split(x.l); }
__device__ __forceinline__ F st29(const G29 &g) { F r; g.template canonical<1>().pack(r.l); return r; }
struct LincombArgs { const F *p[8]; size_t len[8]; G29 sc[8]; int count; };
__global__ void k_lincomb_n(F *__restrict__ out, LincombArgs a, size_t n) {
    size_t i = (size_t)blockIdx.x * blockDim.x + threadIdx.x;
    if (i >= n) return;
    G29 v[8];
#pragma unroll
    for (int j = 0; j < 8; j++) v[j] = (j < a.count && i < a.len[j]) ? ld29(a.p[j][i]) : G29::zero();
    G29 acc = G29::dot<4>(v, a.sc);
    if (a.count > 4) acc = acc + G29::dot<4>(v + 4, a.sc + 4);
    out[i] = st29(acc);
}
void poly_lincomb_n(F *out, size_t n, const F *const *polys, const size_t *lens, const F *scalars, int count, stream_t s) {
    if (!n) return;
    if (count < 1 || count > 8) throw GpuError("poly_lincomb_n: 1..8 terms");
    LincombArgs a;
    a.count = count;
    for (int j = 0; j < 8; j++) { a.p[j] = j < count ? polys[j] : nullptr; a.len[j] = j < count ? lens[j] : 0; a.sc[j] = j < count ? G29::twiddle_from_std(scalars[j]) : G29::zero(); }
    hipLaunchKernelGGL(k_lincomb_n, GRID(n), 0, (hipStream_t)s, out, a, n); HIP_LAUNCH_CHECK();
}

__global__ void k_div_vanishing(F *__restrict__ q, F *__restrict__ rem, const F *__restrict__ p, size_t len, size_t m) {
    size_t j = (size_t)blockIdx.x * blockDim.x + threadIdx.x;
    if (j >= m) return;
    size_t qlen = len - m;
    F carry = F::zero();
    if (qlen > j) {
        size_t top = j + ((qlen - 1 - j) / m) * m;
        for (size_t i = top;; i -= m) {
            carry = p[i + m] + carry;
            q[i] = carry;
            if (i < m) break;
        }
    }
    if (rem) rem[j] = (j < len ? p[j] : F::zero()) + carry;
}
__global__ void k_divvan_sums(F *__restrict__ part, const F *__restrict__ p, size_t qlen, size_t m, size_t C, size_t S) {
    size_t idx = (size_t)blockIdx.x * blockDim.x + threadIdx.x;
    if (idx >= S * m) return;
    const size_t seg = idx / m, j = idx % m;
    F sum = F::zero();
    for (size_t t = seg * C; t < (seg + 1) * C; t++) { size_t i = j + t * m; if (i < qlen) sum = sum + p[i + m]; }
    part[idx] = sum;
}
__global__ void k_divvan_apply(F *__restrict__ q, F *__restrict__ rem, const F *__restrict__ p, const F *__restrict__ part, size_t len, size_t m, size_t C, size_t S) {
    size_t idx = (size_t)blockIdx.x * blockDim.x + threadIdx.x;
    if (idx >= S * m) return;
    const size_t seg = idx / m, j = idx % m, qlen = len - m;
    F carry = F::zero();
    for (size_t u = S; u-- > seg + 1;) carry = carry + part[u * m + j];
    for (size_t t = (seg + 1) * C; t-- > seg * C;) { size_t i = j + t * m; if (i < qlen) { carry = carry + p[i + m]; q[i] = carry; } }
    if (seg == 0 && rem) rem[j] = (j < len ? p[j] : F::zero()) + carry;
}
size_t divide_by_vanishing_scratch(size_t len, size_t m) {
    if (m == 0 || len <= m) return 0;
    const size_t chain = (len - m + m - 1) / m;
    return chain >= 64 ? (chain + 15) / 16 * m : 0;
}
void divide_by_vanishing(F *q, F *rem, const F *p, size_t len, size_t m, stream_t s, F *scratch, size_t scratch_len) {
    if (m == 0 || len <= m) throw GpuError("divide_by_vanishing: dividend shorter than divisor");
    const size_t chain = (len - m + m - 1) / m;
    const size_t C = 16, S = (chain + C - 1) / C;
    if (chain >= 64 && scratch && S * m <= scratch_len) {
        hipLaunchKernelGGL(k_divvan_sums, GRID(S * m), 0, (hipStream_t)s, scratch, p, len - m, m, C, S); HIP_LAUNCH_CHECK();
        hipLaunchKernelGGL(k_divvan_apply, GRID(S * m), 0, (hipStream_t)s, q, rem, p, (const F *)scratch, len, m, C, S); HIP_LAUNCH_CHECK();
        return;
    }
    hipLaunchKernelGGL(k_div_vanishing, GRID(m), 0, (hipStream_t)s, q, rem, p, len, m); HIP_LAUNCH_CHECK();
}

constexpr int DL_B = 16;
__global__ void k_divlin_local(F *__restrict__ q, const F *__restrict__ p, size_t len, F z, F *__restrict__ v, F *__restrict__ zp) {
    if (blockIdx.x == 0 && threadIdx.x < DL_B) zp[threadIdx.x] = z.pow_u64(threadIdx.x);
    const size_t t = (size_t)blockIdx.x * blockDim.x + threadIdx.x, s0 = t * DL_B;
    if (s0 >= len) return;
    const size_t e = s0 + DL_B < len ? s0 + DL_B : len;
    F l = F::zero();
    for (size_t i = e; i-- > s0;) {
        if (i + 1 < len) q[i] = l;
        l = p[i] + z * l;
    }
    v[t] = l;
}
constexpr int DL_TOP_THREADS = 256;
constexpr size_t DL_TOP = (size_t)DL_TOP_THREADS * DL_B;
__global__ void __launch_bounds__(DL_TOP_THREADS) k_divlin_top(F *__restrict__ q, const F *__restrict__ p, size_t len, F z) {
    __shared__ F sh[DL_TOP_THREADS];
    const uint32_t t = threadIdx.x;
    const size_t s0 = (size_t)t * DL_B, e = s0 + DL_B < len ? s0 + DL_B : len;
    F l = F::zero();
    if (s0 < len) {
        for (size_t i = e; i-- > s0;) {
            if (i + 1 < len) q[i] = l;
            l = p[i] + z * l;
        }
    }
    sh[t] = l;
    __syncthreads();
    F y = z.pow_u64(DL_B);
    for (int k = 1; k < DL_TOP_THREADS; k <<= 1) {
        const F other = t + k < DL_TOP_THREADS ? sh[t + k] : F::zero();
        __syncthreads();
        sh[t] = sh[t] + y * other;
        __syncthreads();
        y = y.sqr();
    }
    if (s0 >= len || e >= len) return;
    const F c = sh[t + 1];
    F w = F::one();
    for (size_t i = e; i-- > s0;) { q[i] = q[i] + w * c; w = w * z; }
}
__global__ void __launch_bounds__(256) k_divlin_apply(F *__restrict__ q, size_t qlen, const F *__restrict__ zp_table, const F *__restrict__ carry, size_t nblocks) {
    __shared__ F zp[DL_B];
    if (threadIdx.x < DL_B) zp[threadIdx.x] = zp_table[threadIdx.x];
    __syncthreads();
    const size_t i = (size_t)blockIdx.x * blockDim.x + threadIdx.x;
    if (i >= qlen) return;
    const size_t t = i / DL_B;
    if (t + 1 >= nblocks) return;
    const size_t e = (t + 1) * DL_B;
    q[i] = q[i] + zp[e - 1 - i] * carry[t];
}
size_t divide_by_linear_scratch(size_t len) {
    size_t total = 8;
    for (size_t n = len; n > DL_B; ) { n = (n + DL_B - 1) / DL_B; total += 2 * n + 2 + DL_B; }
    return total;
}
static void divlin_rec(F *q, const F *p, size_t len, const F &z, F *scratch, hipStream_t s) {
    if (len < 2) return;
    if (len <= DL_TOP) { hipLaunchKernelGGL(k_divlin_top, dim3(1), dim3(DL_TOP_THREADS), 0, s, q, p, len, z); HIP_LAUNCH_CHECK(); return; }
    const size_t nblocks = (len + DL_B - 1) / DL_B;
    F *v = scratch, *carry = scratch + nblocks + 1, *zp = carry + nblocks + 1;
    hipLaunchKernelGGL(k_divlin_local, GRID(nblocks), 0, s, q, p, len, z, v, zp); HIP_LAUNCH_CHECK();
    divlin_rec(carry, v, nblocks, z.pow_u64(DL_B), zp + DL_B, s);
    hipLaunchKernelGGL(k_divlin_apply, GRID(len - 1), 0, s, q, len - 1, (const F *)zp, (const F *)carry, nblocks); HIP_LAUNCH_CHECK();
}
void divide_by_linear(F *q, const F *p, size_t len, const F &z, F *scratch, size_t scratch_elems, stream_t s_) {
    hipStream_t s = (hipStream_t)s_;
    if (len < 2) return;
    if (len >= ((size_t)1 << 31)) throw GpuError("divide_by_linear: polynomial too long");
    if (z.is_zero()) { HIP_CHECK(hipMemcpyAsync(q, p + 1, (len - 1) * sizeof(F), hipMemcpyDeviceToDevice, s)); return; }
    if (divide_by_linear_scratch(len) > scratch_elems) throw GpuError("divide_by_linear: scratch too small");
    divlin_rec(q, p, len, z, scratch, s);
}

constexpr size_t EV_CHUNK = 16, EV_COMBINE_MAX = 1024;
__global__ void k_eval_chunks(const F *__restrict__ p, size_t len, F x, F *__restrict__ partial) {
    size_t t = (size_t)blockIdx.x * blockDim.x + threadIdx.x;
    size_t nch = (len + EV_CHUNK - 1) / EV_CHUNK;
    if (t >= nch) return;
    size_t s0 = t * EV_CHUNK, e = s0 + EV_CHUNK < len ? s0 + EV_CHUNK : len;
    F acc = F::zero();
    for (size_t i = e; i-- > s0;) acc = acc * x + p[i];
    partial[t] = acc;
}
__global__ void __launch_bounds__(256) k_eval_combine(const F *__restrict__ partial, size_t nch, F y, F *__restrict__ out) {
    __shared__ F sh[256];
    uint32_t t = threadIdx.x;
    F y256 = y.pow_u64(256), pw = y.pow_u64(t), acc = F::zero();
    for (size_t i = t; i < nch; i += 256) { acc = acc + partial[i] * pw; pw = pw * y256; }
    sh[t] = acc;
    __syncthreads();
    for (int s = 128; s > 0; s >>= 1) { if ((int)t < s) sh[t] = sh[t] + sh[t + s]; __syncthreads(); }
    if (t == 0) out[0] = sh[0];
}
size_t poly_eval_scratch(size_t len) {
    size_t tot = 0, n = len;
    do { n = (n + EV_CHUNK - 1) / EV_CHUNK; tot += n; } while (n > EV_COMBINE_MAX);
    return tot;
}
static void eval_launch(const F *p, size_t len, F x, F *scratch, F *out, hipStream_t s) {
    const F *src = p;
    size_t n = len;
    F y = x;
    do {
        size_t nch = (n + EV_CHUNK - 1) / EV_CHUNK;
        hipLaunchKernelGGL(k_eval_chunks, GRID(nch), 0, s, src, n, y, scratch); HIP_LAUNCH_CHECK();
        src = scratch; scratch += nch; n = nch; y = y.pow_u64(EV_CHUNK);
    } while (n > EV_COMBINE_MAX);
    hipLaunchKernelGGL(k_eval_combine, dim3(1), dim3(256), 0, s, src, n, y, out); HIP_LAUNCH_CHECK();
}
void poly_eval_multi(const F *const *p, const size_t *len, const F *x, int count, F *out, F *scratch, size_t scratch_elems, stream_t s_) {
    hipStream_t s = (hipStream_t)s_;
    if (count < 1 || count > 8) throw GpuError("poly_eval_multi: 1..8 polynomials");
    size_t need = 8;
    for (int i = 0; i < count; i++) need += poly_eval_scratch(len[i]);
    if (need > scratch_elems) throw GpuError("poly_eval_multi: scratch too small");
    F *res = scratch, *at = scratch + 8;
    bool any = false;
    for (int i = 0; i < count; i++) {
        if (!len[i]) continue;
        eval_launch(p[i], len[i], x[i], at, res + i, s);
        at += poly_eval_scratch(len[i]); any = true;
    }
    F host[8];
    if (any) {
        sync((stream_t)s);
        HIP_CHECK(hipMemcpyAsync(host, res, count * sizeof(F), hipMemcpyDeviceToHost, s));
        sync((stream_t)s);
    }
    for (int i = 0; i < count; i++) out[i] = len[i] ? host[i] : F::zero();
}
F poly_eval(const F *p, size_t len, const F &x, F *scratch, stream_t s_) {
    F out;
    poly_eval_multi(&p, &len, &x, 1, &out, scratch, 8 + poly_eval_scratch(len), s_);
    return out;
}

constexpr int BI_BLOCK = 512;
template <int BI_CHUNK>
__global__ void __launch_bounds__(BI_BLOCK) k_batch_inverse(F *__restrict__ v, size_t n, bool has_post, F post) {
    __shared__ F pre_s[BI_BLOCK], suf_s[BI_BLOCK];
    __shared__ F inv_total;
    const int lane = threadIdx.x;
    size_t t = (size_t)blockIdx.x * BI_BLOCK + lane;
    size_t s0 = t * BI_CHUNK;
    if (s0 > n) s0 = n;
    size_t e = s0 + BI_CHUNK < n ? s0 + BI_CHUNK : n;
    F pre[BI_CHUNK];
    F acc = F::one();
    for (size_t i = s0; i < e; i++) { pre[i - s0] = acc; F x = v[i]; if (!x.is_zero()) acc = acc * x; }
    pre_s[lane] = acc; suf_s[lane] = acc;
    __syncthreads();
    for (int d = 1; d < BI_BLOCK; d <<= 1) {
        F a, b;
        const bool ha = lane >= d, hb = lane + d < BI_BLOCK;
        if (ha) a = pre_s[lane - d];
        if (hb) b = suf_s[lane + d];
        __syncthreads();
        if (ha) pre_s[lane] = pre_s[lane] * a;
        if (hb) suf_s[lane] = suf_s[lane] * b;
        __syncthreads();
    }
    if (lane == 0) { F iv = BI_CHUNK == 4 ? suf_s[0].inverse() : suf_s[0].inverse_fermat(); inv_total = has_post ? iv * post : iv; }
    __syncthreads();
    acc = inv_total;
    if (lane > 0) acc = acc * pre_s[lane - 1];
    if (lane + 1 < BI_BLOCK) acc = acc * suf_s[lane + 1];
    for (size_t i = e; i-- > s0;) {
        F x = v[i];
        if (x.is_zero()) continue;
        v[i] = acc * pre[i - s0];
        acc = acc * x;
    }
}
constexpr int VQ_MAX_COSETS = 3, VQ_STEP = 10;
struct VqArgs { F *out[VQ_MAX_COSETS]; const F *tab; const F *elems; uint32_t n; int lg_n; bool unit_g[VQ_MAX_COSETS]; };
__device__ __forceinline__ F vq_factor(const VqArgs &A, int c, int k, uint32_t j) {
    const F e = A.elems[(size_t)j << k];
    return A.tab[k] + (A.unit_g[c] ? e : e * A.tab[(size_t)(c + 1) * A.lg_n + k]);
}
__global__ void __launch_bounds__(1024) k_vq_top(VqArgs A, F *__restrict__ mid) {
    __shared__ F buf[2][1 << VQ_STEP];
    const int c = blockIdx.x, L = A.lg_n, k_stop = L > VQ_STEP ? L - VQ_STEP : 0;
    const uint32_t t = threadIdx.x;
    if (t == 0) buf[0][0] = F::one();
    __syncthreads();
    int cur = 0;
    for (int k = L - 1; k >= k_stop; k--) {
        const uint32_t s = A.n >> k;
        if (t < s) buf[cur ^ 1][t] = vq_factor(A, c, k, t) * buf[cur][t & ((s >> 1) - 1)];
        __syncthreads();
        cur ^= 1;
    }
    const uint32_t s = A.n >> k_stop;
    F *dst = k_stop == 0 ? A.out[c] : mid + (size_t)c * (1u << VQ_STEP);
    if (t < s) dst[t] = buf[cur][t];
}
__global__ void __launch_bounds__(256) k_vq_expand(VqArgs A, const F *__restrict__ src, F *__restrict__ dst, int k_hi, int k_lo) {
    __shared__ F buf[2][1 << VQ_STEP];
    const uint32_t s_hi = A.n >> k_hi;
    const int c = blockIdx.x / s_hi;
    const uint32_t j = blockIdx.x % s_hi, t = threadIdx.x;
    if (t == 0) buf[0][0] = src[(size_t)c * s_hi + j];
    __syncthreads();
    int cur = 0;
    for (int k = k_hi - 1; k >= k_lo; k--) {
        const uint32_t cnt = 1u << (k_hi - k);
        for (uint32_t m = t; m < cnt; m += 256) buf[cur ^ 1][m] = vq_factor(A, c, k, j + m * s_hi) * buf[cur][m & ((cnt >> 1) - 1)];
        __syncthreads();
        cur ^= 1;
    }
    const uint32_t cnt = 1u << (k_hi - k_lo);
    F *o = k_lo == 0 ? A.out[c] : dst + (size_t)c * (A.n >> k_lo);
    for (uint32_t m = t; m < cnt; m += 256) o[j + (size_t)m * s_hi] = buf[cur][m];
}
static inline int vq_next_level(int k_hi) { const int r = k_hi % VQ_STEP; return k_hi - (r ? r : VQ_STEP); }
size_t vanishing_quotient_scratch(int lg_n, int ncosets) {
    size_t tab = (size_t)(ncosets + 1) * (lg_n > 0 ? lg_n : 1), mids = 0;
    for (int k = lg_n - VQ_STEP; k > 0; k = vq_next_level(k)) mids += (size_t)ncosets << (lg_n - k);
    return tab + mids + 8;
}
void vanishing_quotient_evals(F *const *out, const F *g, int ncosets, const F &a, const F *elems, uint32_t n, int lg_n, F *scratch, size_t scratch_elems, stream_t s_) {
    hipStream_t s = (hipStream_t)s_;
    if (ncosets < 1 || ncosets > VQ_MAX_COSETS) throw GpuError("vanishing_quotient_evals: 1..3 cosets");
    if (n == 0 || n != (1u << lg_n)) throw GpuError("vanishing_quotient_evals: n must be 2^lg_n");
    if (vanishing_quotient_scratch(lg_n, ncosets) > scratch_elems) throw GpuError("vanishing_quotient_evals: scratch too small");
    if (lg_n == 0) { for (int c = 0; c < ncosets; c++) { F one = F::one(); h2d(out[c], &one, sizeof(F), s_); } return; }
    std::vector<F> tab((size_t)(ncosets + 1) * lg_n);
    F v = a;
    for (int k = 0; k < lg_n; k++) { tab[k] = v; v = v.sqr(); }
    VqArgs A;
    for (int c = 0; c < VQ_MAX_COSETS; c++) { A.out[c] = c < ncosets ? out[c] : nullptr; A.unit_g[c] = true; }
    for (int c = 0; c < ncosets; c++) {
        A.unit_g[c] = g[c] == F::one();
        v = g[c];
        for (int k = 0; k < lg_n; k++) { tab[(size_t)(c + 1) * lg_n + k] = v; v = v.sqr(); }
    }
    h2d(scratch, tab.data(), tab.size() * sizeof(F), s_);
    A.tab = scratch; A.elems = elems; A.n = n; A.lg_n = lg_n;
    F *mid = scratch + tab.size();
    hipLaunchKernelGGL(k_vq_top, dim3(ncosets), dim3(1024), 0, s, A, mid); HIP_LAUNCH_CHECK();
    for (int k_hi = lg_n - VQ_STEP; k_hi > 0; ) {
        const int k_lo = vq_next_level(k_hi);
        F *dst = mid + ((size_t)ncosets << (lg_n - k_hi));
        hipLaunchKernelGGL(k_vq_expand, dim3((unsigned)((size_t)ncosets * (n >> k_hi))), dim3(256), 0, s, A, (const F *)mid, dst, k_hi, k_lo); HIP_LAUNCH_CHECK();
        mid = dst; k_hi = k_lo;
    }
}
__global__ void k_f_from_tables(F *__restrict__ out, const F *__restrict__ va, const F *__restrict__ vb, const F *__restrict__ vc, G29 ea, G29 eb, G29 ec, const F *__restrict__ ra,
                                const F *__restrict__ rb, const uint32_t *__restrict__ ri, const uint32_t *__restrict__ ci, size_t k) {
    size_t i = (size_t)blockIdx.x * blockDim.x + threadIdx.x;
    if (i >= k) return;
    const G29 v[3] = {ld29(va[i]), ld29(vb[i]), ld29(vc[i])}, w[3] = {ea, eb, ec};
    const F num = st29(G29::dot<3>(v, w));
    out[i] = num.is_zero() ? num : num * (rb[ci[i]] * ra[ri[i]]);
}
void f_evals_from_tables(F *out, const F *va, const F *vb, const F *vc, const F &ea, const F &eb, const F &ec, const F *ra, const F *rb, const uint32_t *ri, const uint32_t *ci, size_t k,
                         stream_t s) {
    if (!k) return;
    hipLaunchKernelGGL(k_f_from_tables, GRID(k), 0, (hipStream_t)s, out, va, vb, vc, G29::twiddle_from_std(ea), G29::twiddle_from_std(eb), G29::twiddle_from_std(ec), ra, rb, ri, ci, k);
    HIP_LAUNCH_CHECK();
}
void batch_inverse(F *v, size_t n, const F *post, stream_t s) {
    if (!n) return;
    const F post_v = post ? *post : F::one();
    if (throughput_mode() || n > ((size_t)1 << 21)) {
        size_t threads = (n + 15) / 16;
        hipLaunchKernelGGL(k_batch_inverse<16>, dim3((unsigned)((threads + BI_BLOCK - 1) / BI_BLOCK)), dim3(BI_BLOCK), 0, (hipStream_t)s, v, n, post != nullptr, post_v); HIP_LAUNCH_CHECK();
    } else {
        size_t threads = (n + 3) / 4;
        hipLaunchKernelGGL(k_batch_inverse<4>, dim3((unsigned)((threads + BI_BLOCK - 1) / BI_BLOCK)), dim3(BI_BLOCK), 0, (hipStream_t)s, v, n, post != nullptr, post_v); HIP_LAUNCH_CHECK();
    }
}

__global__ void k_q1_coset(F *__restrict__ out, const F *__restrict__ r, const F *__restrict__ za, const F *__restrict__ zb, const F *__restrict__ t, const F *__restrict__ z,
                           F ca, F cb, F cz, G29 ea, G29 eb, G29 ec, size_t n) {
    size_t i = (size_t)blockIdx.x * blockDim.x + threadIdx.x;
    if (i >= n) return;
    const G29 a = ld29(za[i]) + ld29(ca), b = ld29(zb[i]) + ld29(cb), zz = ld29(z[i]) + ld29(cz);
    const G29 v[3] = {a.shl5() * b, a, b}, w[3] = {ec, ea, eb};
    const G29 sum = G29::dot<3>(v, w);
    const G29 l[2] = {ld29(r[i]).shl5(), ld29(t[i]).shl5()}, m[2] = {sum, G29::zero().template sub<2>(zz)};
    out[i] = st29(G29::dot<2>(l, m));
}
void q1_coset_pointwise(F *out, const F *r, const F *za, const F *zb, const F *t, const F *z, const F &ca, const F &cb, const F &cz, const F &ea, const F &eb, const F &ec, size_t n, stream_t s) {
    hipLaunchKernelGGL(k_q1_coset, GRID(n), 0, (hipStream_t)s, out, r, za, zb, t, z, ca, cb, cz, G29::twiddle_from_std(ea), G29::twiddle_from_std(eb), G29::twiddle_from_std(ec), n); HIP_LAUNCH_CHECK();
}
__global__ void k_z_evals_h(F *__restrict__ out, const uint8_t *__restrict__ z, uint32_t n, uint32_t m, uint32_t num_witness) {
    uint32_t k = blockIdx.x * blockDim.x + threadIdx.x;
    if (k >= n) return;
    const uint32_t ratio = n / m;
    uint8_t bit;
    if (k % ratio == 0) bit = z[k / ratio];
    else { const uint32_t wi = k - k / ratio - 1; bit = wi < num_witness ? z[m + wi] : 0; }
    out[k] = bit ? F::one() : F::zero();
}
void z_evals_h(F *out, const uint8_t *z, uint32_t n, uint32_t m, uint32_t num_witness, stream_t s) {
    hipLaunchKernelGGL(k_z_evals_h, GRID(n), 0, (hipStream_t)s, out, z, n, m, num_witness); HIP_LAUNCH_CHECK();
}
__global__ void k_q1_combine(F *__restrict__ h1, F *__restrict__ g1, const F *__restrict__ q0, const F *__restrict__ q1, const F *__restrict__ q3, const F *__restrict__ mask,
                             F inv2, F inv2zeta, size_t n) {
    size_t i = (size_t)blockIdx.x * blockDim.x + threadIdx.x;
    if (i >= n) return;
    const F a = q1[i], b = q3[i], c = q0[i];
    const F q_mid = (a - b) * inv2zeta;
    const F q_hi = ((c - q_mid) - (a + b) * inv2) * inv2;
    const F m_lo = mask[i], m_mid = mask[n + i], m_hi = mask[2 * n + i];
    h1[i] = q_mid + q_hi + m_mid + m_hi;
    h1[n + i] = q_hi + m_hi;
    if (i >= 1) g1[i - 1] = c + m_lo + m_mid + m_hi;
}
void q1_combine(F *h1, F *g1, const F *q0, const F *q1, const F *q3, const F *mask, const F &inv2, const F &inv2zeta, size_t n, stream_t s) {
    hipLaunchKernelGGL(k_q1_combine, GRID(n), 0, (hipStream_t)s, h1, g1, q0, q1, q3, mask, inv2, inv2zeta, n); HIP_LAUNCH_CHECK();
}
__global__ void k_coset_scale(F *__restrict__ out, const F *__restrict__ in, F g, size_t in_len, size_t n) {
    size_t t = (size_t)blockIdx.x * blockDim.x + threadIdx.x;
    size_t j0 = t * 16;
    if (j0 >= n) return;
    size_t e = j0 + 16 < n ? j0 + 16 : n;
    F pw = g.pow_u64(j0);
    for (size_t j = j0; j < e; j++) { out[j] = j < in_len ? in[j] * pw : F::zero(); pw = pw * g; }
}
void coset_scale(F *out, const F *in, const F &g, size_t in_len, size_t n, stream_t s) {
    if (!n) return;
    hipLaunchKernelGGL(k_coset_scale, GRID((n + 15) / 16), 0, (hipStream_t)s, out, in, g, in_len, n); HIP_LAUNCH_CHECK();
}
__global__ void k_h2_coset(F *__restrict__ out, const F *__restrict__ row, const F *__restrict__ col, const F *__restrict__ va, const F *__restrict__ vb,
                           const F *__restrict__ vc, const F *__restrict__ rc, const F *__restrict__ f, G29 alpha, G29 beta, F alpha_beta, G29 ea, G29 eb, G29 ec, G29 vinv, size_t k) {
    size_t i = (size_t)blockIdx.x * blockDim.x + threadIdx.x;
    if (i >= k) return;
    const G29 v3[3] = {ld29(va[i]), ld29(vb[i]), ld29(vc[i])}, w3[3] = {ea, eb, ec};
    const G29 a = G29::dot<3>(v3, w3);
    const G29 v2[2] = {ld29(row[i]), ld29(col[i])}, w2[2] = {alpha, beta};
    const G29 b = (ld29(alpha_beta) + ld29(rc[i])).template sub<2>(G29::dot<2>(v2, w2));
    const G29 bf = b.shl5() * ld29(f[i]);
    out[i] = st29(a.template sub<2>(bf) * vinv);
}
void h2_coset(F *out, const F *row, const F *col, const F *va, const F *vb, const F *vc, const F *rc, const F *f, const F &alpha, const F &beta, const F &alpha_beta,
              const F &ea, const F &eb, const F &ec, const F &vinv, size_t k, stream_t s) {
    hipLaunchKernelGGL(k_h2_coset, GRID(k), 0, (hipStream_t)s, out, row, col, va, vb, vc, rc, f, G29::twiddle_from_std(alpha), G29::twiddle_from_std(beta), alpha_beta,
                       G29::twiddle_from_std(ea), G29::twiddle_from_std(eb), G29::twiddle_from_std(ec), G29::twiddle_from_std(vinv), k); HIP_LAUNCH_CHECK();
}
__global__ void k_z_poly(F *__restrict__ zp, const F *__restrict__ w, size_t wlen, const F *__restrict__ x, uint32_t m, size_t n1) {
    size_t i = (size_t)blockIdx.x * blockDim.x + threadIdx.x;
    if (i >= n1) return;
    F v = F::zero();
    if (i >= m && i - m < wlen) v = w[i - m];
    if (i < wlen) v = v - w[i];
    if (i < m) v = v + x[i];
    zp[i] = v;
}
void z_poly_from_w(F *zp, const F *w, size_t wlen, const F *x_poly, uint32_t m, size_t n, stream_t s) { hipLaunchKernelGGL(k_z_poly, GRID(n + 1), 0, (hipStream_t)s, zp, w, wlen, x_poly, m, n + 1); HIP_LAUNCH_CHECK(); }

__device__ __forceinline__ uint32_t rotl32(uint32_t x, int n) { return (x << n) | (x >> (32 - n)); }
__global__ void k_chacha_blocks(uint32_t *__restrict__ words, uint64_t first_block, uint32_t nblocks, uint32_t k0, uint32_t k1, uint32_t k2, uint32_t k3, uint32_t k4, uint32_t k5,
                                uint32_t k6, uint32_t k7, int rounds) {
    uint32_t b = blockIdx.x * blockDim.x + threadIdx.x;
    if (b >= nblocks) return;
    uint64_t ctr = first_block + b;
    uint32_t s[16] = {0x61707865u, 0x3320646eu, 0x79622d32u, 0x6b206574u, k0, k1, k2, k3, k4, k5, k6, k7, (uint32_t)ctr, (uint32_t)(ctr >> 32), 0, 0};
    uint32_t x[16];
#pragma unroll
    for (int i = 0; i < 16; i++) x[i] = s[i];
#define ZK_QR(a, b, c, d) \
    x[a] += x[b]; x[d] = rotl32(x[d] ^ x[a], 16); x[c] += x[d]; x[b] = rotl32(x[b] ^ x[c], 12); \
    x[a] += x[b]; x[d] = rotl32(x[d] ^ x[a], 8); x[c] += x[d]; x[b] = rotl32(x[b] ^ x[c], 7);
    for (int r = 0; r < rounds; r += 2) {
        ZK_QR(0, 4, 8, 12) ZK_QR(1, 5, 9, 13) ZK_QR(2, 6, 10, 14) ZK_QR(3, 7, 11, 15)
        ZK_QR(0, 5, 10, 15) ZK_QR(1, 6, 11, 12) ZK_QR(2, 7, 8, 13) ZK_QR(3, 4, 9, 14)
    }
#undef ZK_QR
#pragma unroll
    for (int i = 0; i < 16; i++) words[(size_t)b * 16 + i] = x[i] + s[i];
}
__global__ void k_rand_flags(const uint32_t *__restrict__ words, uint32_t word_off, uint32_t ncand, uint32_t *__restrict__ flags) {
    uint32_t j = blockIdx.x * blockDim.x + threadIdx.x;
    if (j >= ncand) return;
    uint32_t l[8];
#pragma unroll
    for (int i = 0; i < 8; i++) l[i] = words[(size_t)word_off + 8 * (size_t)j + i];
    l[7] &= 0xffffffffu >> (256 - F::BITS);
    flags[j] = F::geq_mod(l) ? 0u : 1u;
}
__global__ void k_rand_compact(const uint32_t *__restrict__ words, uint32_t word_off, uint32_t ncand, const uint32_t *__restrict__ flags, const uint32_t *__restrict__ pos,
                               F *__restrict__ out, uint32_t count, uint32_t *__restrict__ last_cand) {
    uint32_t j = blockIdx.x * blockDim.x + threadIdx.x;
    if (j >= ncand || !flags[j]) return;
    uint32_t q = pos[j];
    if (q >= count) return;
    F v;
#pragma unroll
    for (int i = 0; i < 8; i++) v.l[i] = words[(size_t)word_off + 8 * (size_t)j + i];
    v.l[7] &= 0xffffffffu >> (256 - F::BITS);
    out[q] = v;
    if (q + 1 == count) *last_cand = j;
}
uint64_t chacha_field_stream(F *out, size_t count, const uint32_t key[8], int rounds, uint64_t word_pos, void *scratch, size_t scratch_bytes, stream_t s_, uint32_t max_cand) {
    hipStream_t s = (hipStream_t)s_;
    if (count == 0) return word_pos;
    const double accept = 0.58;
    uint64_t pos_words = word_pos;
    size_t done = 0;
    while (done < count) {
        size_t want = count - done;
        uint32_t ncand = (uint32_t)((double)want / accept * 1.02) + 4096;
        if (max_cand && ncand > max_cand) ncand = max_cand;
        uint64_t first_block = pos_words / 16;
        uint32_t word_off = (uint32_t)(pos_words % 16);
        uint32_t nblocks = (uint32_t)(((uint64_t)word_off + 8ull * ncand + 15) / 16);
        size_t need = (size_t)nblocks * 64 + (size_t)ncand * 8 + 64 + (1 << 20);
        if (need > scratch_bytes) throw GpuError("chacha_field_stream: scratch too small");
        uint32_t *words = (uint32_t *)scratch, *flags = words + (size_t)nblocks * 16, *pos = flags + ncand, *last = pos + ncand;
        void *tmp = (void *)(last + 16);
        size_t tmp_bytes = scratch_bytes - ((char *)tmp - (char *)scratch);
        hipLaunchKernelGGL(k_chacha_blocks, GRID(nblocks), 0, s, words, first_block, nblocks, key[0], key[1], key[2], key[3], key[4], key[5], key[6], key[7], rounds); HIP_LAUNCH_CHECK();
        hipLaunchKernelGGL(k_rand_flags, GRID(ncand), 0, s, (const uint32_t *)words, word_off, ncand, flags); HIP_LAUNCH_CHECK();
        size_t tb = 0;
        HIP_CHECK(rocprim::exclusive_scan(nullptr, tb, flags, pos, 0u, (size_t)ncand, rocprim::plus<uint32_t>(), s));
        if (tb > tmp_bytes) throw GpuError("chacha_field_stream: scan scratch too small");
        HIP_CHECK(rocprim::exclusive_scan(tmp, tb, flags, pos, 0u, (size_t)ncand, rocprim::plus<uint32_t>(), s));
        HIP_CHECK(hipMemsetAsync(last, 0xff, 4, s));
        hipLaunchKernelGGL(k_rand_compact, GRID(ncand), 0, s, (const uint32_t *)words, word_off, ncand, (const uint32_t *)flags, (const uint32_t *)pos, out + done, (uint32_t)want, last); HIP_LAUNCH_CHECK();
        uint32_t h_last = 0, h_tail[2] = {0, 0};
        sync((stream_t)s);
        HIP_CHECK(hipMemcpyAsync(&h_last, last, 4, hipMemcpyDeviceToHost, s));
        HIP_CHECK(hipMemcpyAsync(&h_tail[0], pos + ncand - 1, 4, hipMemcpyDeviceToHost, s));
        HIP_CHECK(hipMemcpyAsync(&h_tail[1], flags + ncand - 1, 4, hipMemcpyDeviceToHost, s));
        sync((stream_t)s);
        if (h_last != 0xffffffffu) { pos_words += 8ull * ((uint64_t)h_last + 1); done = count; }
        else { done += (size_t)h_tail[0] + h_tail[1]; pos_words += 8ull * ncand; }
    }
    return pos_words;
}
__global__ void k_mask_fixup(F *p, size_t n) { if (blockIdx.x == 0 && threadIdx.x == 0) p[0] = p[0] - (p[0] + p[n] + p[2 * n]); }
void mask_fixup(F *p, size_t n, stream_t s) { hipLaunchKernelGGL(k_mask_fixup, dim3(1), dim3(64), 0, (hipStream_t)s, p, n); HIP_LAUNCH_CHECK(); }

__global__ void k_index_rowcol(F *__restrict__ row, F *__restrict__ col, F *__restrict__ rowcol, F *__restrict__ u, const uint32_t *__restrict__ ci, const uint32_t *__restrict__ ri,
                               size_t cnt, size_t k, const F *__restrict__ elems, uint32_t n, F n_fe) {
    size_t i = (size_t)blockIdx.x * blockDim.x + threadIdx.x;
    if (i >= k) return;
    if (i < cnt) {
        uint32_t c = ci[i], r = ri[i];
        F rv = elems[c], cv = elems[r];
        row[i] = rv; col[i] = cv; rowcol[i] = rv * cv;
        u[i] = elems[(n - c) & (n - 1)] * n_fe;
    } else {
        row[i] = elems[0]; col[i] = elems[0]; rowcol[i] = elems[0]; u[i] = F::zero();
    }
}
__global__ void k_index_vals(F *__restrict__ va, F *__restrict__ vb, F *__restrict__ vc, const F *__restrict__ uinv, const int64_t *__restrict__ ca, const int64_t *__restrict__ cb,
                             const int64_t *__restrict__ cc, size_t cnt, size_t k) {
    size_t i = (size_t)blockIdx.x * blockDim.x + threadIdx.x;
    if (i >= k) return;
    if (i < cnt) {
        F w = uinv[i];
        va[i] = ca[i] ? F::from_i64(ca[i]) * w : F::zero();
        vb[i] = cb[i] ? F::from_i64(cb[i]) * w : F::zero();
        vc[i] = cc[i] ? F::from_i64(cc[i]) * w : F::zero();
    } else { va[i] = F::zero(); vb[i] = F::zero(); vc[i] = F::zero(); }
}
void index_evals(F *row, F *col, F *rowcol, F *va, F *vb, F *vc, F *tmp, const uint32_t *ci, const uint32_t *ri, const int64_t *ca, const int64_t *cb, const int64_t *cc, size_t cnt,
                 size_t k, const F *elems, uint32_t n, stream_t s) {
    hipLaunchKernelGGL(k_index_rowcol, GRID(k), 0, (hipStream_t)s, row, col, rowcol, tmp, ci, ri, cnt, k, elems, n, F::from_u64(n)); HIP_LAUNCH_CHECK();
    batch_inverse(tmp, k, nullptr, s);
    hipLaunchKernelGGL(k_index_vals, GRID(k), 0, (hipStream_t)s, va, vb, vc, tmp, ca, cb, cc, cnt, k); HIP_LAUNCH_CHECK();
}
// ... 4 lines not shown
```

aes_zero_knowledge_proof_circuit_amd/csrc/kernels_witness.hip:

```cpp
#include <mutex>
#include "hip_util.hpp"
#include "trace_layout.h"

namespace zk {
namespace gpu {

#define GRID(n) dim3((unsigned)(((n) + 255) / 256)), dim3(256)

static uint8_t *g_sbox_dev[64] = {nullptr};
static std::mutex g_sbox_mu;
static uint8_t *sbox_here() {
    int d = 0;
    HIP_CHECK(hipGetDevice(&d));
    if (d < 0 || d >= 64) throw GpuError("device ordinal out of range");
    std::lock_guard<std::mutex> g(g_sbox_mu);
    return g_sbox_dev[d];
}
void upload_sbox(const uint8_t table[256]) {
    int d = 0;
    HIP_CHECK(hipGetDevice(&d));
    if (d < 0 || d >= 64) throw GpuError("device ordinal out of range");
    std::lock_guard<std::mutex> g(g_sbox_mu);
    if (!g_sbox_dev[d]) g_sbox_dev[d] = (uint8_t *)dmalloc(256);
    HIP_CHECK(hipMemcpy(g_sbox_dev[d], table, 256, hipMemcpyHostToDevice));
}

static int trace_nk(const char *who, size_t key_bytes) {
    if (key_bytes != 16 && key_bytes != 24 && key_bytes != 32) throw GpuError(std::string(who) + ": the AES key must have 16, 24 or 32 bytes");
    return (int)(key_bytes / 4);
}
static size_t trace_bytes_of(int nk, size_t b4, size_t b6, size_t b8) { return nk == 4 ? b4 : nk == 6 ? b6 : b8; }

__device__ __forceinline__ uint8_t xtime(uint8_t c) { return (uint8_t)((c << 1) ^ (((c >> 7) & 1) * 0x1B)); }

template <bool STORE, int NK = 4>
__device__ __forceinline__ void aes_block_rounds(uint8_t s[16], const uint8_t (*w)[4], const uint8_t *__restrict__ sbox, uint8_t *__restrict__ bl) {
    uint8_t u[16], v[16];
    for (int r = 1; r <= TRK_NR(NK); r++) {
        for (int i = 0; i < 16; i++) { v[i] = sbox[s[i]]; if (STORE) bl[TRK_BL_SB(NK) + 16 * (r - 1) + i] = v[i]; }
        for (int c = 0; c < 4; c++) for (int rr = 0; rr < 4; rr++) u[4 * c + rr] = v[4 * ((c + rr) & 3) + rr];
        if (r <= TRK_NR(NK) - 1) {
            for (int c = 0; c < 4; c++) {
                uint8_t a[4], xb[4];
                for (int k = 0; k < 4; k++) { a[k] = u[4 * c + k]; xb[k] = xtime(a[k]); if (STORE) bl[TRK_BL_XT(NK) + 16 * (r - 1) + 4 * c + k] = xb[k]; }
                const uint8_t term[4][5] = {{xb[0], a[3], a[2], xb[1], a[1]}, {xb[1], a[0], a[3], xb[2], a[2]}, {xb[2], a[1], a[0], xb[3], a[3]}, {xb[3], a[2], a[1], xb[0], a[0]}};
                for (int o = 0; o < 4; o++) {
                    uint8_t acc = term[o][0];
                    for (int q = 1; q < 5; q++) { acc ^= term[o][q]; if (STORE) bl[TRK_BL_MP(NK) + 64 * (r - 1) + 4 * (4 * c + o) + (q - 1)] = acc; }
                    v[4 * c + o] = acc;
                }
            }
        } else {
            for (int i = 0; i < 16; i++) v[i] = u[i];
        }
        for (int i = 0; i < 16; i++) { s[i] = v[i] ^ w[4 * r + i / 4][i % 4]; if (STORE) bl[TRK_BL_S(NK) + 16 * r + i] = s[i]; }
    }
}

template <int NK = 4>
__device__ __forceinline__ void aes_key_schedule(const uint8_t *__restrict__ key, const uint8_t *__restrict__ sbox, uint8_t (*w)[4], uint8_t *__restrict__ tr) {
    const uint8_t rc[10] = {0x01, 0x02, 0x04, 0x08, 0x10, 0x20, 0x40, 0x80, 0x1B, 0x36};
    for (int i = 0; i < NK; i++) for (int k = 0; k < 4; k++) w[i][k] = key[4 * i + k];
    for (int i = NK; i < TRK_KS_WORDS(NK); i++) {
        if (i % NK == 0) {
            int q = TRK_KS_INST_OF(NK, i);
            uint8_t sub[4], pre[4];
            for (int k = 0; k < 4; k++) sub[k] = sbox[w[i - 1][(k + 1) & 3]];
            for (int k = 0; k < 4; k++) { pre[k] = w[i - NK][k] ^ sub[k]; w[i][k] = pre[k]; }
            w[i][0] ^= rc[i / NK - 1];
            if (tr) for (int k = 0; k < 4; k++) { tr[TRK_KS_SUB(NK) + 4 * q + k] = sub[k]; tr[TRK_KS_PRE(NK) + 4 * q + k] = pre[k]; }
        } else if (NK == 8 && i % 8 == 4) {
            int q = TRK_KS_INST_OF(NK, i);
            uint8_t sub[4];
            for (int k = 0; k < 4; k++) sub[k] = sbox[w[i - 1][k]];
            for (int k = 0; k < 4; k++) w[i][k] = w[i - NK][k] ^ sub[k];
            if (tr) for (int k = 0; k < 4; k++) { tr[TRK_KS_SUB(NK) + 4 * q + k] = sub[k]; tr[TRK_KS_PRE(NK) + 4 * q + k] = w[i][k]; }
        } else {
            for (int k = 0; k < 4; k++) w[i][k] = w[i - NK][k] ^ w[i - 1][k];
        }
    }
}
template <int NK = 4>
__device__ __forceinline__ void aes_store_schedule(uint8_t *__restrict__ tr, const uint8_t *__restrict__ key, const uint8_t (*w)[4]) {
    for (int i = 0; i < TRK_KEY_BYTES(NK); i++) tr[TR_KEY + i] = key[i];
    for (int i = 0; i < TRK_KS_WORDS(NK); i++) for (int k = 0; k < 4; k++) tr[TRK_KS_W(NK) + 4 * i + k] = w[i][k];
}

template <bool CBC, int NK = 4>
__global__ void k_aes_trace(uint8_t *__restrict__ trace, size_t stride, const uint8_t *__restrict__ msgs, const uint8_t *__restrict__ keys, const uint8_t *__restrict__ ivs,
                            uint32_t nproofs, uint32_t nblocks, const uint8_t *__restrict__ sbox) {
    uint32_t t = blockIdx.x * blockDim.x + threadIdx.x;
    if (t >= nproofs * (nblocks + 1)) return;
    uint32_t p = t / (nblocks + 1), which = t % (nblocks + 1);
    uint8_t *tr = trace + (size_t)p * stride;
    const uint8_t *key = keys + TRK_KEY_BYTES(NK) * (size_t)p;
    uint8_t w[TRK_KS_WORDS(NK)][4];
    aes_key_schedule<NK>(key, sbox, w, which == 0 ? tr : nullptr);
    uint8_t *tail = tr + TRK_CBC(NK, (size_t)nblocks);
    if (which == 0) {
        aes_store_schedule<NK>(tr, key, w);
        if (CBC) for (int i = 0; i < 16; i++) tail[TR_CBC_IV + i] = ivs[16 * (size_t)p + i];
        return;
    }
    uint32_t b = which - 1;
    uint8_t *bl = tr + TRK_BLOCK0(NK) + (size_t)b * TRK_BLOCK_STRIDE(NK);
    const uint8_t *msg = msgs + ((size_t)p * nblocks + b) * 16;
    uint8_t s[16];
    if (CBC) {
        uint8_t prev[16];
        for (int i = 0; i < 16; i++) prev[i] = ivs[16 * (size_t)p + i];
        for (uint32_t j = 0; j < b; j++) {
            const uint8_t *mj = msgs + ((size_t)p * nblocks + j) * 16;
            for (int i = 0; i < 16; i++) s[i] = mj[i] ^ prev[i] ^ key[i];
            aes_block_rounds<false, NK>(s, w, sbox, nullptr);
            for (int i = 0; i < 16; i++) prev[i] = s[i];
        }
        for (int i = 0; i < 16; i++) {
            uint8_t x = msg[i] ^ prev[i];
            bl[TR_BL_MSG + i] = msg[i]; tail[TR_CBC_X + 16 * b + i] = x; s[i] = x ^ key[i]; bl[TR_BL_S + i] = s[i];
        }
    } else {
        for (int i = 0; i < 16; i++) { bl[TR_BL_MSG + i] = msg[i]; s[i] = msg[i] ^ key[i]; bl[TR_BL_S + i] = s[i]; }
    }
    aes_block_rounds<true, NK>(s, w, sbox, bl);
}

__device__ __forceinline__ void ctr_add(const uint8_t *__restrict__ in, uint32_t n, uint8_t out[16]) {
    uint32_t c = n;
    for (int i = 15; i >= 0; i--) { uint32_t t = in[i] + (c & 0xff); out[i] = (uint8_t)t; c = (c >> 8) + (t >> 8); }
}

template <int NK = 4>
__global__ void k_aes_trace_ctr(uint8_t *__restrict__ trace, size_t stride, const uint8_t *__restrict__ msgs, const uint8_t *__restrict__ keys, const uint8_t *__restrict__ icbs,
                                uint32_t nproofs, uint32_t nblocks, uint32_t msg_len, const uint8_t *__restrict__ sbox) {
    uint32_t t = blockIdx.x * blockDim.x + threadIdx.x;
    if (t >= nproofs * (nblocks + 1)) return;
    uint32_t p = t / (nblocks + 1), which = t % (nblocks + 1);
    uint8_t *tr = trace + (size_t)p * stride;
    const uint8_t *key = keys + TRK_KEY_BYTES(NK) * (size_t)p, *icb = icbs + 16 * (size_t)p;
    uint8_t w[TRK_KS_WORDS(NK)][4];
    aes_key_schedule<NK>(key, sbox, w, which == 0 ? tr : nullptr);
    uint8_t *tail = tr + TRK_CTR(NK, (size_t)nblocks);
    if (which == 0) {
        aes_store_schedule<NK>(tr, key, w);
        for (int i = 0; i < 16; i++) tail[TR_CTR_ICB + i] = icb[i];
        return;
    }
    uint32_t b = which - 1;
    uint8_t *bl = tr + TRK_BLOCK0(NK) + (size_t)b * TRK_BLOCK_STRIDE(NK), *slot = tail + TR_CTR_BLOCK0 + (size_t)b * TR_CTR_BLOCK_STRIDE;
    uint8_t ctr[16], carry[16], s[16], m[16];
    ctr_add(icb, b, ctr);
    for (int i = 0; i < 16; i++) carry[i] = 0;
    if (b) {
// ... 275 lines not shown
void ghash_trace(uint8_t *trace, size_t stride, uint32_t nproofs, uint32_t msg_len, uint32_t aad_len, stream_t s, size_t key_bytes) {
    uint32_t nblocks, naad;
    const int nk = gcm_shape("ghash_trace", trace, stride, nproofs, msg_len, aad_len, key_bytes, nblocks, naad);
    uint32_t lanes = nproofs * (naad + nblocks + 2) * 16;
    const dim3 grid((lanes + 63) / 64), block(64);
    if (nk == 4) hipLaunchKernelGGL(k_ghash_trace<4>, grid, block, 0, (hipStream_t)s, trace, stride, nproofs, nblocks, naad, msg_len, aad_len);
    else if (nk == 6) hipLaunchKernelGGL(k_ghash_trace<6>, grid, block, 0, (hipStream_t)s, trace, stride, nproofs, nblocks, naad, msg_len, aad_len);
    else hipLaunchKernelGGL(k_ghash_trace<8>, grid, block, 0, (hipStream_t)s, trace, stride, nproofs, nblocks, naad, msg_len, aad_len);
    HIP_LAUNCH_CHECK();
}
static int gcm_seg_shape(const char *who, const uint8_t *trace, size_t stride, uint32_t nproofs, int role, uint32_t msg_len, uint32_t aad_len, size_t key_bytes, uint32_t &nblocks, uint32_t &naad) {
    const int nk = trace_nk(who, key_bytes);
    if (role != TRS_HEAD && role != TRS_MID && role != TRS_TAIL) throw GpuError(std::string(who) + ": the role must be 0 (head), 1 (mid) or 2 (tail)");
    if (msg_len == 0 || msg_len > (1u << 16) || aad_len > (1u << 16)) throw GpuError(std::string(who) + ": the message must have 1 .. 65536 bytes, the aad at most 65536");
    if (role != TRS_TAIL && msg_len % 16) throw GpuError(std::string(who) + ": a head or mid segment takes whole blocks");
    if (role != TRS_HEAD && aad_len) throw GpuError(std::string(who) + ": only a head segment takes aad");
    if (!trace) throw GpuError(std::string(who) + ": no trace buffer");
    nblocks = (msg_len + 15) / 16; naad = (aad_len + 15) / 16;
    const size_t na = naad, nb = nblocks;
    if (stride < trace_bytes_of(nk, TRS_BYTES(4, role, na, nb), TRS_BYTES(6, role, na, nb), TRS_BYTES(8, role, na, nb))) throw GpuError(std::string(who) + ": trace stride is short of the segment region");
    if (stride % 16 || (uintptr_t)trace % 16) throw GpuError(std::string(who) + ": traces must be 16-byte aligned");
    if (nproofs == 0 || nproofs > (1u << 20)) throw GpuError(std::string(who) + ": 1 .. 2^20 proofs per launch");
    return nk;
}
void aes_trace_gcm_seg(uint8_t *trace, size_t stride, const uint8_t *msgs, const uint8_t *keys, const uint8_t *hdrs, uint32_t nproofs, int role, uint32_t msg_len, uint32_t aad_len, stream_t s, size_t key_bytes) {
    if (!msgs || !keys || !hdrs) throw GpuError("aes_trace_gcm_seg: no message, key or header buffer");
    uint32_t nblocks, naad;
    const int nk = gcm_seg_shape("aes_trace_gcm_seg", trace, stride, nproofs, role, msg_len, aad_len, key_bytes, nblocks, naad);
    uint8_t *g_sbox = sbox_here();
    if (!g_sbox) throw GpuError("aes_trace_gcm_seg: S-box table not uploaded on this device");
    uint32_t lanes = nproofs * (TRS_SLOTS(role, nblocks) + 1);
    const dim3 grid((lanes + 63) / 64), block(64);
    if (nk == 4) hipLaunchKernelGGL(k_aes_trace_gcm_seg<4>, grid, block, 0, (hipStream_t)s, trace, stride, msgs, keys, hdrs, nproofs, (uint32_t)role, nblocks, naad, msg_len, aad_len, g_sbox);
    else if (nk == 6) hipLaunchKernelGGL(k_aes_trace_gcm_seg<6>, grid, block, 0, (hipStream_t)s, trace, stride, msgs, keys, hdrs, nproofs, (uint32_t)role, nblocks, naad, msg_len, aad_len, g_sbox);
    else hipLaunchKernelGGL(k_aes_trace_gcm_seg<8>, grid, block, 0, (hipStream_t)s, trace, stride, msgs, keys, hdrs, nproofs, (uint32_t)role, nblocks, naad, msg_len, aad_len, g_sbox);
    HIP_LAUNCH_CHECK();
}
void ghash_trace_seg(uint8_t *trace, size_t stride, uint32_t nproofs, int role, uint32_t msg_len, uint32_t aad_len, stream_t s, size_t key_bytes) {
    uint32_t nblocks, naad;
    const int nk = gcm_seg_shape("ghash_trace_seg", trace, stride, nproofs, role, msg_len, aad_len, key_bytes, nblocks, naad);
    uint32_t lanes = nproofs * (TRS_MULS(role, naad, nblocks) + 1) * 16;
    const dim3 grid((lanes + 63) / 64), block(64);
    if (nk == 4) hipLaunchKernelGGL(k_ghash_trace_seg<4>, grid, block, 0, (hipStream_t)s, trace, stride, nproofs, (uint32_t)role, nblocks, naad);
    else if (nk == 6) hipLaunchKernelGGL(k_ghash_trace_seg<6>, grid, block, 0, (hipStream_t)s, trace, stride, nproofs, (uint32_t)role, nblocks, naad);
    else hipLaunchKernelGGL(k_ghash_trace_seg<8>, grid, block, 0, (hipStream_t)s, trace, stride, nproofs, (uint32_t)role, nblocks, naad);
    HIP_LAUNCH_CHECK();
}
void key_tag_trace(uint8_t *trace, size_t stride, size_t tag_off, const uint8_t *keys, uint32_t nproofs, uint32_t tag_blocks, stream_t s, size_t key_bytes) {
    const int nk = trace_nk("key_tag_trace", key_bytes);
    if (!trace || !keys) throw GpuError("key_tag_trace: no trace or key buffer");
    if (tag_blocks != 1 && tag_blocks != 2) throw GpuError("key_tag_trace: 1 or 2 tag blocks");
    const size_t slot = trace_bytes_of(nk, TRK_BLOCK_STRIDE(4), TRK_BLOCK_STRIDE(6), TRK_BLOCK_STRIDE(8));
    if (tag_off < trace_bytes_of(nk, TRK_BLOCK0(4), TRK_BLOCK0(6), TRK_BLOCK0(8)) || tag_off > stride || stride - tag_off < tag_blocks * slot)
        throw GpuError("key_tag_trace: trace stride " + std::to_string(stride) + " does not hold " + std::to_string(tag_blocks) + " tag slots of " + std::to_string(slot) + " bytes at offset " + std::to_string(tag_off));
    if (tag_off % 16 || stride % 16 || (uintptr_t)trace % 16) throw GpuError("key_tag_trace: tagged traces and the tag offset must be 16-byte aligned");
    if (nproofs == 0 || nproofs > (1u << 20)) throw GpuError("key_tag_trace: 1 .. 2^20 proofs per launch");
    uint8_t *g_sbox = sbox_here();
    if (!g_sbox) throw GpuError("key_tag_trace: S-box table not uploaded on this device");
    uint32_t lanes = nproofs * tag_blocks;
    const dim3 grid((lanes + 63) / 64), block(64);
    if (nk == 4) hipLaunchKernelGGL(k_key_tag_trace<4>, grid, block, 0, (hipStream_t)s, trace, stride, tag_off, keys, nproofs, tag_blocks, g_sbox);
    else if (nk == 6) hipLaunchKernelGGL(k_key_tag_trace<6>, grid, block, 0, (hipStream_t)s, trace, stride, tag_off, keys, nproofs, tag_blocks, g_sbox);
    else hipLaunchKernelGGL(k_key_tag_trace<8>, grid, block, 0, (hipStream_t)s, trace, stride, tag_off, keys, nproofs, tag_blocks, g_sbox);
    HIP_LAUNCH_CHECK();
}

__global__ void k_witness_expand(uint8_t *__restrict__ z, const uint32_t *__restrict__ desc, uint32_t ncols, const uint8_t *__restrict__ trace,
                                 const uint32_t *__restrict__ sbox_in_off, const uint32_t *__restrict__ sbox_tmpl, const uint8_t *__restrict__ sbox) {
    uint32_t i = blockIdx.x * blockDim.x + threadIdx.x;
    if (i >= ncols) return;
    uint32_t d = desc[i], kind = d >> WD_KIND_SHIFT, bit;
    if (kind == WD_BYTEBIT) {
        uint32_t off = (d >> 4) & 0x3ffffff, b = (d >> 1) & 7;
        bit = ((trace[off] >> b) & 1) ^ (d & 1);
    } else if (kind == WD_SBOX) {
        uint32_t inst = (d >> 11) & 0x7ffff, te = sbox_tmpl[(d >> 1) & 0x3ff];
        uint32_t lvl = (te >> 12) & 7, node = (te >> 4) & 0xff, b = (te >> 1) & 7;
        uint32_t x = trace[sbox_in_off[inst]];
        uint32_t idx = (node << (lvl + 1)) | (x & ((2u << lvl) - 1));
        bit = ((sbox[idx] >> b) & 1) ^ (d & 1);
    } else {
        bit = d & 1;
    }
    z[i] = (uint8_t)bit;
}
void witness_expand(uint8_t *z, const uint32_t *desc, uint32_t ncols, const uint8_t *trace, const uint32_t *sbox_in_off, const uint32_t *sbox_tmpl, stream_t s) {
    uint8_t *g_sbox = sbox_here();
    if (!g_sbox) throw GpuError("witness_expand: S-box table not uploaded on this device");
    hipLaunchKernelGGL(k_witness_expand, GRID(ncols), 0, (hipStream_t)s, z, desc, ncols, trace, sbox_in_off, sbox_tmpl, g_sbox);
    HIP_LAUNCH_CHECK();
}

__device__ __forceinline__ F small_to_field(long long v) { return F::from_i64(v); }

__global__ void k_spmv_bits(F *__restrict__ out, int8_t *__restrict__ small_out, size_t rows_out, const uint32_t *__restrict__ rowptr, const uint32_t *__restrict__ col, const int64_t *__restrict__ coeff,
                            size_t rows, const uint8_t *__restrict__ z) {
    size_t r = (size_t)blockIdx.x * blockDim.x + threadIdx.x;
    if (r >= rows_out) return;
    long long acc = 0;
    if (r < rows) for (uint32_t i = rowptr[r]; i < rowptr[r + 1]; i++) acc += z[col[i]] ? coeff[i] : 0;
    out[r] = acc == 0 ? F::zero() : small_to_field(acc);
    if (small_out) small_out[r] = (int8_t)(acc > 127 ? 127 : (acc < -127 ? -127 : acc));
}
void spmv_bits(F *out, int8_t *small_out, size_t rows_out, const uint32_t *rowptr, const uint32_t *col, const int64_t *coeff, size_t rows, const uint8_t *z, stream_t s) {
    hipLaunchKernelGGL(k_spmv_bits, GRID(rows_out), 0, (hipStream_t)s, out, small_out, rows_out, rowptr, col, coeff, rows, z); HIP_LAUNCH_CHECK();
}
__global__ void k_w_classes(int8_t *__restrict__ out, const uint8_t *__restrict__ z, uint32_t n, uint32_t m, uint32_t num_witness) {
    uint32_t k = blockIdx.x * blockDim.x + threadIdx.x;
    if (k >= n) return;
    uint32_t ratio = n / m;
    if (k % ratio == 0) { out[k] = 0; return; }
    uint32_t wi = k - k / ratio - 1;
    out[k] = (wi < num_witness && z[m + wi]) ? 1 : 0;
}
void w_classes(int8_t *out, const uint8_t *z, uint32_t n, uint32_t m, uint32_t num_witness, stream_t s) {
    hipLaunchKernelGGL(k_w_classes, GRID(n), 0, (hipStream_t)s, out, z, n, m, num_witness); HIP_LAUNCH_CHECK();
}
__global__ void k_lagrange_finish(F *__restrict__ lag, F *__restrict__ lag_w, const F *__restrict__ elems, uint32_t n, uint32_t m, F vx_inv, F n_inv) {
    uint32_t k = blockIdx.x * blockDim.x + threadIdx.x;
    if (k >= n) return;
    F v = lag[k] * (elems[k] * n_inv);
    lag[k] = v;
    lag_w[k] = (k % (n / m) == 0) ? F::zero() : v * vx_inv;
}
void lagrange_scalars(F *lag, F *lag_w, const F *elems, const F &beta, uint32_t n, uint32_t m, stream_t s) {
    int lg_n = 0;
    while ((1u << lg_n) < n) lg_n++;
    F vx_inv = (beta.pow_u64(m) - F::one()).inverse();
    const size_t need = vanishing_quotient_scratch(lg_n, 1);
    DevPtr<F> scratch(need);
    F *outs[1] = {lag};
    const F one = F::one();
    vanishing_quotient_evals(outs, &one, 1, beta, elems, n, lg_n, scratch, need, s);
    hipLaunchKernelGGL(k_lagrange_finish, GRID(n), 0, (hipStream_t)s, lag, lag_w, elems, n, m, vx_inv, F::from_u64(n).inverse()); HIP_LAUNCH_CHECK();
    sync(s);
}

__global__ void k_w_evals(F *__restrict__ out, const uint8_t *__restrict__ z, const F *__restrict__ x_evals, uint32_t n, uint32_t m, uint32_t num_witness) {
    uint32_t k = blockIdx.x * blockDim.x + threadIdx.x;
    if (k >= n) return;
    uint32_t ratio = n / m;
    if (k % ratio == 0) { out[k] = F::zero(); return; }
    uint32_t wi = k - k / ratio - 1;
    F w = (wi < num_witness && z[m + wi]) ? F::one() : F::zero();
    out[k] = w - x_evals[k];
}
void w_evals(F *out, const uint8_t *z, const F *x_evals, uint32_t n, uint32_t m, uint32_t num_witness, stream_t s) {
    hipLaunchKernelGGL(k_w_evals, GRID(n), 0, (hipStream_t)s, out, z, x_evals, n, m, num_witness); HIP_LAUNCH_CHECK();
}
__global__ void k_bits_to_field(F *__restrict__ out, const uint8_t *__restrict__ z, size_t n) { size_t i = (size_t)blockIdx.x * blockDim.x + threadIdx.x; if (i < n) out[i] = z[i] ? F::one() : F::zero(); }
void bits_to_field(F *out, const uint8_t *z, size_t n, stream_t s) { if (!n) return; hipLaunchKernelGGL(k_bits_to_field, GRID(n), 0, (hipStream_t)s, out, z, n); HIP_LAUNCH_CHECK(); }

__global__ void k_t_partials(F *__restrict__ partial, uint32_t nseg, const uint32_t *__restrict__ seg_start, const uint32_t *__restrict__ seg_end, const uint32_t *__restrict__ row,
                             const uint8_t *__restrict__ mat, const int64_t *__restrict__ coeff, const F *__restrict__ r_alpha, F eta_a, F eta_b, F eta_c) {
    uint32_t sgi = blockIdx.x * blockDim.x + threadIdx.x;
    if (sgi >= nseg) return;
    F acc = F::zero();
    for (uint32_t i = seg_start[sgi]; i < seg_end[sgi]; i++) {
        F eta = mat[i] == 0 ? eta_a : (mat[i] == 1 ? eta_b : eta_c);
        long long c = coeff[i];
        F term = eta * r_alpha[row[i]];
        if (c == 1) acc = acc + term;
        else if (c == -1) acc = acc - term;
        else acc = acc + term * small_to_field(c);
    }
    partial[sgi] = acc;
}
__global__ void k_t_columns(F *__restrict__ out, uint32_t n, const uint32_t *__restrict__ col_seg_ptr, const F *__restrict__ partial) {
    uint32_t h = blockIdx.x * blockDim.x + threadIdx.x;
    if (h >= n) return;
    uint32_t a = col_seg_ptr[h], b = col_seg_ptr[h + 1];
    if (b - a > T_HEAVY_SEGMENTS) return;
    F acc = F::zero();
    for (uint32_t i = a; i < b; i++) acc = acc + partial[i];
    out[h] = acc;
}
__global__ void __launch_bounds__(256) k_t_heavy(F *__restrict__ out, const uint32_t *__restrict__ heavy, const uint32_t *__restrict__ col_seg_ptr, const F *__restrict__ partial) {
    __shared__ F sh[256];
    uint32_t h = heavy[blockIdx.x], t = threadIdx.x;
    F acc = F::zero();
    for (uint32_t i = col_seg_ptr[h] + t; i < col_seg_ptr[h + 1]; i += 256) acc = acc + partial[i];
    sh[t] = acc;
    __syncthreads();
    for (int s = 128; s > 0; s >>= 1) { if ((int)t < s) sh[t] = sh[t] + sh[t + s]; __syncthreads(); }
    if (t == 0) out[h] = sh[0];
}
void t_evals(F *out, uint32_t n, F *partial, uint32_t nseg, const uint32_t *col_seg_ptr, const uint32_t *seg_start, const uint32_t *seg_end, const uint32_t *heavy, uint32_t n_heavy,
             const uint32_t *row, const uint8_t *mat, const int64_t *coeff, const F *r_alpha, const F &eta_a, const F &eta_b, const F &eta_c, stream_t s) {
    if (nseg) { hipLaunchKernelGGL(k_t_partials, GRID(nseg), 0, (hipStream_t)s, partial, nseg, seg_start, seg_end, row, mat, coeff, r_alpha, eta_a, eta_b, eta_c); HIP_LAUNCH_CHECK(); }
    hipLaunchKernelGGL(k_t_columns, GRID(n), 0, (hipStream_t)s, out, n, col_seg_ptr, partial); HIP_LAUNCH_CHECK();
    if (n_heavy) { hipLaunchKernelGGL(k_t_heavy, dim3(n_heavy), dim3(256), 0, (hipStream_t)s, out, heavy, col_seg_ptr, partial); HIP_LAUNCH_CHECK(); }
}

}
}
```

aes_zero_knowledge_proof_circuit_amd/csrc/marlin.cpp:

```cpp
#include "marlin.hpp"
#include "statement.hpp"
#include "../../include/zkaes.h"
#include <algorithm>
#include <cstdio>
#include <chrono>
#include <cstdlib>
#include <cstring>
#include <atomic>
#include <map>
#include <mutex>
#include <future>
#include <deque>
#include <condition_variable>
#include <thread>
#include <functional>
#include <stdexcept>
#include <cerrno>
#include <sys/random.h>
#include "gpu.hpp"
#include "trace_layout.h"
#include "transcript.hpp"
#include "marlin_host.hpp"
#include "verify_batch.hpp"

// ... 654 lines not shown
        for (int i = 0; i < 2; i++) {
            const Fr zc = i == 0 ? zeta : zeta.neg();
            gpu::q1_coset_pointwise(cs_buf[i][5], cs_buf[i][2], cs_buf[i][0], cs_buf[i][1], cs_buf[i][3], cs_buf[i][4], R.rhos[1] * zc, R.rhos[2] * zc, R.rhos[0] * zc, R.eta_a, R.eta_b, R.eta_c, n, s);
        }
        const Job inv13[2] = {{Q1, cs_buf[0][5], 1}, {Q3, cs_buf[1][5], 3}};
        gpu::ntt_batch<F>(inv13, 2, n, lg_n, true, lg_n4, s);
        gpu::q1_combine(cx.poly[6].p, cx.poly[5].p, Q0, Q1, Q3, cx.poly[3].p, inv2, inv2zeta, n, s);
        cx.poly_len[6] = 2 * n; cx.poly_len[5] = n - 1;
    }
    R.jobs.start(2, [&](Lane &ln) { mpc_commit(cx, ln, R.r2[1]); }, true);
    R.jobs.start(4, [&](Lane &ln) { mpc_commit(cx, ln, R.r2[2]); }, true);
    R.jobs.join();
    { Bytes o; for (auto &lp : R.r2) o.commitment_tobytes(lp.comm); R.fs.absorb(o.b); }
    R.beta = sample_outside_h(R.fs);
    cx.timings.round2_ms = ms_since(R.t0); R.t0 = Clock::now();
}

void ProvingKeyImpl::prove_round3(ProofRun &R) {
    ProverContext &cx = R.cx;
    gpu::stream_t s = cx.stream;
    const F *elems = gpu::domain_elements<F>(lg_n);
    for (auto &lp : R.r3) draw_rand(lp, R.zk);
    R.vh_beta = eval_vanishing(n, R.beta);
    const Fr vv = R.vh_alpha * R.vh_beta;
    R.ea_vv = R.eta_a * vv; R.eb_vv = R.eta_b * vv; R.ec_vv = R.eta_c * vv; R.alpha_beta = R.alpha * R.beta;
    {
        F *outs[1] = {cx.ra_poly.p};
        const Fr one = Fr::one();
        gpu::vanishing_quotient_evals(outs, &one, 1, R.beta, elems, (uint32_t)n, lg_n, cx.e[0].p, cx.e[0].n, s);
        gpu::f_evals_from_tables(cx.e[1].p, ix_ev[2].p, ix_ev[3].p, ix_ev[4].p, R.eta_a, R.eta_b, R.eta_c, cx.ra_ev.p, cx.ra_poly.p, d_ix_ri, d_ix_ci, k, s);
    }
    gpu::ntt<F>(cx.f_poly.p, cx.e[1].p, k, lg_k, true, s);
    gpu::d2d(cx.poly[7].p, cx.f_poly.p + 1, (k - 1) * sizeof(F), s); cx.poly_len[7] = k - 1;
    R.jobs.start(1, [&](Lane &ln) { mpc_commit(cx, ln, R.r3[0]); }, true);
    gpu::ntt_scaled<F>(cx.e[2].p, cx.f_poly.p, k, lg_k, false, coset_tab, s);
    gpu::h2_coset(cx.e[0].p, ix_cs[0].p, ix_cs[1].p, ix_cs[2].p, ix_cs[3].p, ix_cs[4].p, ix_cs[5].p, cx.e[2].p, R.alpha, R.beta, R.alpha_beta, R.ea_vv, R.eb_vv, R.ec_vv, coset_vk_inv, k, s);
    gpu::ntt_scaled<F>(cx.poly[8].p, cx.e[0].p, k, lg_k, true, coset_tab_inv, s);
    cx.poly_len[8] = k - 1;
    R.jobs.start(2, [&](Lane &ln) { mpc_commit(cx, ln, R.r3[1]); }, true);
    R.early_evals = R.jobs.async;
    if (R.early_evals) {
        const F *ps[3] = {cx.poly[5].p, cx.poly[4].p, cx.poly[2].p};
        const size_t ls[3] = {cx.poly_len[5], cx.poly_len[4], cx.poly_len[2]};
        const Fr at[3] = {R.beta, R.beta, R.beta};
        Fr ev[3];
        gpu::poly_eval_multi(ps, ls, at, 3, ev, cx.scratch.p, cx.scratch.n, s);
        R.pf.evals[0] = ev[0]; R.pf.evals[2] = ev[1]; R.pf.evals[3] = ev[2];
        gpu::divide_by_linear(cx.wit2.p, cx.poly[5].p, cx.poly_len[5], R.beta, cx.scratch.p, cx.scratch.n, s);
    }
    R.jobs.join();
    { Bytes o; for (auto &lp : R.r3) o.commitment_tobytes(lp.comm); R.fs.absorb(o.b); }
    R.gamma = R.fs.rng().rand_field<Fr>();
    cx.timings.round3_ms = ms_since(R.t0); R.t0 = Clock::now();
}

void ProvingKeyImpl::prove_open(ProofRun &R) {
    ProverContext &cx = R.cx;
    gpu::stream_t s = cx.stream;
    if (R.early_evals) {
        const F *ps[1] = {cx.poly[7].p};
        const size_t ls[1] = {cx.poly_len[7]};
        gpu::poly_eval_multi(ps, ls, &R.gamma, 1, &R.pf.evals[1], cx.scratch.p, cx.scratch.n, s);
    } else {
        const F *ps[4] = {cx.poly[5].p, cx.poly[7].p, cx.poly[4].p, cx.poly[2].p};
        const size_t ls[4] = {cx.poly_len[5], cx.poly_len[7], cx.poly_len[4], cx.poly_len[2]};
        const Fr at[4] = {R.beta, R.gamma, R.beta, R.beta};
        gpu::poly_eval_multi(ps, ls, at, 4, R.pf.evals, cx.scratch.p, cx.scratch.n, s);
    }
    const Fr g2_g = R.pf.evals[1], t_b = R.pf.evals[2], zb_b = R.pf.evals[3];
    { Bytes o; for (auto &v : R.pf.evals) o.field(v); R.fs.absorb(o.b); }
    Fr ch;
    { uint64_t lo = R.fs.rng().next_u64(), hi = R.fs.rng().next_u64(); uint32_t raw[8] = {(uint32_t)lo, (uint32_t)(lo >> 32), (uint32_t)hi, (uint32_t)(hi >> 32), 0, 0, 0, 0}; ch = Fr::from_raw(raw); }
    Fr r_alpha_at_beta = (R.vh_alpha - R.vh_beta) * (R.alpha - R.beta).inverse();
    Fr vx_beta = eval_vanishing(m, R.beta);
    Fr c_za = r_alpha_at_beta * (R.eta_a + R.eta_c * zb_b), c_w = (t_b * vx_beta).neg(), c_h1 = R.vh_beta.neg();
    Fr vk_gamma = eval_vanishing(k, R.gamma);
    Fr bmul = R.gamma * g2_g + t_b * Fr::from_u64(k).inverse();
    Fr c_row = R.alpha * bmul, c_col = R.beta * bmul, c_rc = bmul.neg(), c_h2 = vk_gamma.neg();
    Fr chp[5]; chp[0] = Fr::one(); for (int i = 1; i < 5; i++) chp[i] = chp[i - 1] * ch;
    auto rand_axpy = [](Fr out[3], const Fr &sc, const KzgRand &r) { if (r.hiding) for (int i = 0; i < 3; i++) out[i] = out[i] + sc * r.b[i]; };
    auto host_divide_by_linear = [](Fr q[2], const Fr p[3], const Fr &z) { q[1] = p[2]; q[0] = p[1] + z * p[2]; };
    auto host_eval3 = [](const Fr p[3], const Fr &z) { return p[0] + z * (p[1] + z * p[2]); };
    if (R.jobs.async && !cx.ev_aux) {
        cx.acc_b.alloc(cx.acc.n); cx.wit_b.alloc(cx.wit.n); cx.wit2_b.alloc(cx.wit2.n); cx.scratch_b.alloc(cx.scratch.n);
        cx.scratch_c.alloc(gpu::divide_by_linear_scratch(std::max(n, k) + 1)); cx.ev_aux = gpu::EventGuard();
    }
    const bool two_sets = cx.ev_aux != nullptr && R.jobs.async;
    if (R.jobs.async) gpu::sync(s);
    struct WaitJobs { RoundJobs &j; ~WaitJobs() { j.wait_all(); } } wait_jobs{R.jobs};
    R.jobs.start(1, [&](Lane &ln) {
        gpu::stream_t ls_ = ln.stream;
        size_t plen = 3 * n;
        Fr rb[3] = {Fr::zero(), Fr::zero(), Fr::zero()};
        {
            const F *ps[7] = {cx.poly[5].p, cx.poly[3].p, cx.poly[1].p, cx.poly[0].p, cx.poly[6].p, cx.poly[4].p, cx.poly[2].p};
            size_t ls[7] = {cx.poly_len[5], cx.poly_len[3], cx.poly_len[1], cx.poly_len[0], cx.poly_len[6], cx.poly_len[4], cx.poly_len[2]};
            Fr sc[7] = {chp[0], chp[2], chp[2] * c_za, chp[2] * c_w, chp[2] * c_h1, chp[3], chp[4]};
            gpu::poly_lincomb_n(cx.acc.p, plen, ps, ls, sc, 7, ls_);
        }
        rand_axpy(rb, chp[0], R.r2[1].rand); rand_axpy(rb, chp[2] * c_za, R.r1[1].rand); rand_axpy(rb, chp[2] * c_w, R.r1[0].rand); rand_axpy(rb, chp[4], R.r1[2].rand);
        if (!R.early_evals) gpu::divide_by_linear(cx.wit2.p, cx.poly[5].p, cx.poly_len[5], R.beta, cx.scratch.p, cx.scratch.n, ls_);
        gpu::divide_by_linear(cx.wit.p, cx.acc.p, plen, R.beta, cx.scratch.p, cx.scratch.n, ls_);
        gpu::poly_scale(cx.wit2.p, chp[1], cx.poly_len[5] - 1, ls_);
        msm_opening_prepare(cx, ln, cx.wit.p, plen - 1, cx.wit2.p, cx.poly_len[5] - 1, bounds[1] - (n - 2));
        XYZZ<Fq377> hw = XYZZ<Fq377>::inf();
        Fr rq[2]; host_divide_by_linear(rq, rb, R.beta);
        for (int i = 0; i < 2; i++) hw.add(srs->gamma_tab[i].mul(rq[i]));
        Fr rv = host_eval3(rb, R.beta);
        Fr srb[3]; for (int i = 0; i < 3; i++) srb[i] = chp[1] * R.r2[1].shifted_rand.b[i];
        host_divide_by_linear(rq, srb, R.beta);
        for (int i = 0; i < 2; i++) hw.add(srs->gamma_tab[i].mul(rq[i]));
        rv = rv + host_eval3(srb, R.beta);
        XYZZ<Fq377> w = msm_opening_finish(ln);
        w.add(hw);
        R.pf.w_beta = w.to_affine(); R.pf.random_v_beta = rv;
    }, false);
    R.jobs.start(2, [&](Lane &ln) {
        gpu::stream_t ls_ = ln.stream;
        DevPtr<F> &acc_ = two_sets ? cx.acc_b : cx.acc, &wit_ = two_sets ? cx.wit_b : cx.wit, &wit2_ = two_sets ? cx.wit2_b : cx.wit2, &scr_ = two_sets ? cx.scratch_b : cx.scratch;
        size_t plen = k;
        {
            const F *ps[8] = {cx.poly[7].p, ix_co[2].p, ix_co[3].p, ix_co[4].p, ix_co[0].p, ix_co[1].p, ix_co[5].p, cx.poly[8].p};
            size_t ls[8] = {cx.poly_len[7], k, k, k, k, k, k, cx.poly_len[8]};
            Fr sc[8] = {chp[0], chp[2] * R.ea_vv, chp[2] * R.eb_vv, chp[2] * R.ec_vv, chp[2] * c_row, chp[2] * c_col, chp[2] * c_rc, chp[2] * c_h2};
            gpu::poly_lincomb_n(acc_.p, plen, ps, ls, sc, 8, ls_);
        }
        gpu::divide_by_linear(wit_.p, acc_.p, plen, R.gamma, scr_.p, scr_.n, ls_);
        if (R.jobs.async) {
            while (!R.g2_quotient_queued.load(std::memory_order_acquire)) std::this_thread::yield();
            gpu::stream_wait_event(ls_, cx.ev_aux);
        } else {
            gpu::divide_by_linear(wit2_.p, cx.poly[7].p, cx.poly_len[7], R.gamma, scr_.p, scr_.n, ls_);
            gpu::poly_scale(wit2_.p, chp[1], cx.poly_len[7] - 1, ls_);
        }
        msm_opening_prepare(cx, ln, wit_.p, plen - 1, wit2_.p, cx.poly_len[7] - 1, bounds[1] - (k - 2));
        XYZZ<Fq377> w = msm_opening_finish(ln);
        R.pf.w_gamma = w.to_affine();
    }, false);
    if (R.jobs.async) {
        try {
            gpu::divide_by_linear(cx.wit2_b.p, cx.poly[7].p, cx.poly_len[7], R.gamma, cx.scratch_c.p, cx.scratch_c.n, s);
            gpu::poly_scale(cx.wit2_b.p, chp[1], cx.poly_len[7] - 1, s);
            gpu::event_record(cx.ev_aux, s);
        } catch (...) { R.g2_quotient_queued.store(true, std::memory_order_release); throw; }
        R.g2_quotient_queued.store(true, std::memory_order_release);
    }
    R.jobs.join();
}

Proof ProvingKeyImpl::prove(ProverContext &cx, const uint8_t *host_trace, const uint8_t *msg, size_t len, const uint8_t *key, const uint8_t *zk_seed, bool throughput, const uint8_t *iv) {
    gpu::set_device(device);
    std::lock_guard<std::mutex> busy(cx.in_use);
    cx.throughput = throughput;
    ProofRun R(*this, cx, host_trace, msg, len, key, iv, zk_seed);
    prove_round1(R);
    prove_round2(R);
    prove_round3(R);
    prove_open(R);
    for (int i = 0; i < 4; i++) R.pf.comms[i] = R.r1[i].comm;
    for (int i = 0; i < 3; i++) R.pf.comms[4 + i] = R.r2[i].comm;
    for (int i = 0; i < 2; i++) R.pf.comms[7 + i] = R.r3[i].comm;
    cx.timings.open_ms = ms_since(R.t0);
    cx.timings.total_ms = ms_since(R.t_all);
    { std::lock_guard<std::mutex> g(ctx_mu); last_timings = cx.timings; }
    return R.pf;
}

ProvingKey::~ProvingKey() { if (impl) { DeviceScope on(impl->device); delete impl; } }
const VerifyingKey &ProvingKey::vk() const { return impl->vk; }
const Circuit &ProvingKey::circuit() const { return impl->circuit; }
const ProverTimings &ProvingKey::last_timings() const { return impl->last_timings; }
bool ProvingKey::tables_built(uint64_t *bytes) const {
    if (bytes) *bytes = impl->use_tables ? impl->srs->bytes() : 0;
    return impl->use_tables;
}
void ProvingKey::srs_info(uint64_t out[6], double secs[2]) const {
    const UniversalSrs &U = *impl->srs;
    out[0] = U.max_degree; out[1] = U.stride; out[2] = U.n_tab; out[3] = U.bytes();
    out[4] = (uint64_t)impl->srs.use_count();
    out[5] = impl->lag ? 2 * (uint64_t)impl->lag->n * sizeof(SrsPoint) : 0;
    if (secs) { secs[0] = impl->setup_srs_s; secs[1] = impl->setup_total_s; }
}
size_t ProvingKey::contexts() const { size_t v = impl->n_contexts.load(); return v ? v : default_contexts(); }
void ProvingKey::set_contexts(size_t n) {
    if (n > 64) throw std::invalid_argument("set_contexts: at most 64 prover contexts per key");
    impl->n_contexts.store(n);
}
void ProvingKey::msm_powers_partial_device(const uint8_t *scalars, size_t n_local, size_t offset, void *dev_out) {
    gpu::set_device(impl->device);
    if (!impl->use_tables) throw std::runtime_error("msm_powers_partial_device: this key has no window tables (KEY_NO_TABLES, or the device was short of memory)");
    if (offset + n_local > impl->supported_degree + 1) throw std::runtime_error("msm_powers_partial_device: range exceeds the committer key");
    ProverContext &cx = impl->context(0);
    std::lock_guard<std::mutex> busy(cx.in_use);
    if (n_local > cx.acc.n) throw std::runtime_error("msm_powers_partial_device: more scalars than a prover context holds");
    if (n_local) gpu::h2d(cx.acc.p, scalars, n_local * sizeof(F), cx.stream);
    gpu::msm_table_sum_device<Bls377>(cx.msm_ws, impl->d_powers, impl->srs_stride, offset, impl->table_c, cx.acc.p, n_local, (XYZZ<Fq377> *)dev_out, cx.stream);
}
static void require_key(const Circuit &c, int kind, bool digest, size_t len, size_t aad_len) {
    if (digest && !c.digest_kind) throw std::invalid_argument("the _digest_ entry points take a proving key synthesized with a digest (digest_kind = 1 or 2)");
    if (!digest && c.digest_kind) throw std::invalid_argument("this proving key carries a plaintext digest: use the _digest_ entry points (zkaes_encrypt_digest_batch_seeded_at, zkaes_encrypt_digest_chunked_seeded_at, zkaes_aes_witness_pd)");
    if (kind != ProvingKey::ANY_AES_KIND) {
        static const char *const names[] = {"AES", "", "", "AES-CBC", "AES-CTR", "AES-GCM"};
        if (kind == CIRCUIT_AES_GCM && c.kind == CIRCUIT_AES_GCM_SEG) throw std::invalid_argument("this proving key is a GCM segment key: use the segment entry points (zkaes_encrypt_gcm_segments_seeded_at, zkaes_aes_witness_gcm_seg)");
        if (c.kind != kind) throw std::invalid_argument(std::string("proving key was not synthesized for the ") + names[kind] + " circuit");
        if (kind == CIRCUIT_AES && len % 16) throw std::invalid_argument("Input must be 16 bytes length when adding round key");
        if (kind == CIRCUIT_AES_CBC && (len == 0 || len % 16)) throw std::invalid_argument("CBC: the message must be a non-zero multiple of 16 bytes");
    }
    if (len != c.message_bytes) throw std::invalid_argument("InstanceDoesNotMatchIndex: proving key was synthesized for " + std::to_string(c.message_bytes) + " bytes");
    if (aad_len != ProvingKey::KEY_AAD && aad_len != c.aad_bytes) throw std::invalid_argument("InstanceDoesNotMatchIndex: proving key was synthesized for " + std::to_string(c.aad_bytes) + " bytes of aad");
}
std::string ProvingKey::op_lists_json(const uint8_t *message, size_t len, const uint8_t key[16], bool throughput_path) {
    require_key(impl->circuit, CIRCUIT_AES, impl->circuit.digest_kind != 0, len, KEY_AAD);
    gpu::OpRecord rec;
    gpu::oplog_begin();
    uint8_t h_in[32];
    sha256_chain(nullptr, nullptr, 0, h_in);
    try { impl->prove(impl->context(0), nullptr, message, len, key, nullptr, throughput_path, impl->circuit.digest_kind ? h_in : nullptr); }
    catch (...) { gpu::oplog_end(); throw; }
    rec = gpu::oplog_end();
    const Circuit &c = impl->circuit;
    std::string o = "{\"h\":" + std::to_string(impl->n) + ",\"k\":" + std::to_string(impl->k) + ",\"x\":" + std::to_string(impl->m) + ",\"variables\":" + std::to_string(c.num_variables()) +
                    ",\"constraints\":" + std::to_string(c.num_constraints) + ",\"nnz\":[" + std::to_string(c.A.nnz()) + "," + std::to_string(c.B.nnz()) + "," + std::to_string(c.C.nnz()) + "]" +
                    ",\"blocks\":" + std::to_string(c.n_blocks) + ",\"path\":\"" + (throughput_path ? "throughput" : "lone") + "\",\"ntt\":[";
    for (size_t i = 0; i < rec.ntt.size(); i++) o += (i ? "," : "") + std::string("[") + std::to_string(rec.ntt[i].first) + "," + std::to_string(rec.ntt[i].second) + "]";
    o += "],\"msm\":[";
    static const char *kinds[3] = {"buckets", "second_bases", "class_sum"};
    for (size_t i = 0; i < rec.msm.size(); i++) o += (i ? "," : "") + std::string("[") + std::to_string(rec.msm[i].first) + ",\"" + kinds[rec.msm[i].second % 3] + "\"]";
    o += "]}";
    return o;
}
static std::vector<uint8_t> witness_of(ProvingKeyImpl *impl, const uint8_t *message, size_t len, const uint8_t *key, const uint8_t *iv) {
    const Circuit &c = impl->circuit;
    ProverContext &cx = impl->context(0);
    std::lock_guard<std::mutex> busy(cx.in_use);
    gpu::stream_t s = cx.stream;
    impl->launch_trace(cx, message, len, key, iv);
    gpu::witness_expand(cx.d_z, impl->d_desc, (uint32_t)c.num_variables(), cx.d_trace, impl->d_sbox_in, impl->d_sbox_tmpl, s);
    std::vector<uint8_t> z(c.num_variables());
    gpu::d2h(z.data(), cx.d_z, z.size(), s);
    return z;
}
void os_random_seed(uint8_t out[32]) {
    size_t got = 0;
    while (got < 32) {
        ssize_t r = getrandom(out + got, 32 - got, 0);
        if (r < 0) { if (errno == EINTR) continue; throw std::runtime_error("getrandom failed: no entropy for the prover's zero-knowledge seed"); }
        got += (size_t)r;
    }
}
static void derive_zk_seed(uint8_t out[32], const uint8_t *seed32, uint64_t index) {
    uint8_t buf[40];
    memcpy(buf, seed32, 32);
    for (int i = 0; i < 8; i++) buf[32 + i] = (uint8_t)(index >> (8 * i));
    Blake2s::digest(out, buf, sizeof buf);
}
static std::vector<Proof> prove_many(ProvingKeyImpl *impl, const uint8_t *messages, const uint8_t *keys, size_t key_stride, size_t n_chunks, size_t n_contexts, const uint8_t *zk_seed, uint64_t index_offset,
                                     const uint8_t *ivs, size_t iv_stride = 16) {
    size_t chunk = impl->circuit.message_bytes;
    if (n_contexts == 0) n_contexts = 1;
    n_contexts = std::min(n_contexts, std::max<size_t>(n_chunks, 1));
    std::vector<Proof> proofs(n_chunks);
    for (size_t i = 0; i < n_contexts; i++) impl->context(i);
    std::atomic<size_t> next{0};
    std::vector<std::string> errors(n_contexts);
    const int device = impl->device;
    auto worker = [&](size_t ci) {
        try {
            gpu::set_device(device);
            ProverContext &cx = impl->context(ci);
            for (;;) {
                size_t i = next.fetch_add(1);
                if (i >= n_chunks) break;
                uint8_t seed_i[32];
                if (zk_seed) derive_zk_seed(seed_i, zk_seed, index_offset + (uint64_t)i);
                proofs[i] = impl->prove(cx, nullptr, messages + i * chunk, chunk, keys + i * key_stride, zk_seed ? seed_i : nullptr, n_chunks > 1, ivs ? ivs + iv_stride * i : nullptr);
            }
        } catch (const std::exception &e) { errors[ci] = e.what(); }
    };
    gpu::ThroughputWaits waits(n_contexts > 1);
    std::vector<std::thread> threads;
    for (size_t ci = 1; ci < n_contexts; ci++) threads.emplace_back(worker, ci);
    worker(0);
    for (auto &t : threads) t.join();
    for (auto &e : errors) if (!e.empty()) throw std::runtime_error(e);
    return proofs;
}
static void trace_header(const Circuit &c, const uint8_t *hdr, const uint8_t *h_in, uint8_t *out) {
    const size_t hb = mode_header_bytes(c);
    if (hb) memcpy(out, hdr, hb);
    if (!c.digest_kind) return;
    if (h_in) memcpy(out + hb, h_in, 32); else sha256_chain(nullptr, nullptr, 0, out + hb);
}
static size_t trace_header_bytes(const Circuit &c) { return mode_header_bytes(c) + (c.digest_kind ? 32 : 0); }
static void host_side(const Circuit &c, const uint8_t *msg, size_t len, const uint8_t *key, const uint8_t *hdr, uint8_t *ct_or_null, uint8_t *tag_or_null) {
    if (!ct_or_null && !(tag_or_null && c.kind == CIRCUIT_AES_GCM)) return;
    std::vector<uint8_t> unwanted(ct_or_null ? 0 : len);
    host_encrypt(c, msg, len, key, hdr, ct_or_null ? ct_or_null : unwanted.data(), tag_or_null);
}
std::vector<uint8_t> ProvingKey::witness(int kind, bool digest, const uint8_t *message, size_t len, const uint8_t *key, const uint8_t *hdr, size_t aad_len, const uint8_t *h_in) {
    const Circuit &c = impl->circuit;
    require_key(c, kind, digest, len, aad_len);
    if (!message || !key || (!hdr && mode_header_bytes(c))) throw std::invalid_argument("null argument");
    std::vector<uint8_t> h(trace_header_bytes(c));
    trace_header(c, hdr, h_in, h.data());
    return witness_of(impl, message, len, key, h.empty() ? nullptr : h.data());
}
// ... 316 lines not shown
```

Before: 96.14.

## Port poly and witness kernels to 29-bit limb arithmetic and add lane-parallel MSM reduce

Several field-arithmetic kernels (scale, divide-by-linear, chunked evaluation, vanishing-quotient tree, f-evals, q1 combine, t-partials) move from 32-bit Montgomery Fp to the 9x29-bit Fp29 representation, which has cheaper lazy carries and uses pre-converted twiddle scalars. t-partials now accumulates per matrix and does a single dot product with eta instead of one multiply per entry. MSM scalar digit extraction uses a new direct Montgomery-to-canonical conversion in Fp29. In throughput mode, a new row/column bucket-reduce kernel uses 16 lanes per job instead of a full block. Each change relies on correct representation conversion (shl5 factors) and enlarges the code surface.

Result: no change. 96.72, median of 6 (+0.6%).

```diff
diff --git a/aes_zero_knowledge_proof_circuit_amd/csrc/ff29.cuh b/aes_zero_knowledge_proof_circuit_amd/csrc/ff29.cuh
--- a/aes_zero_knowledge_proof_circuit_amd/csrc/ff29.cuh
+++ b/aes_zero_knowledge_proof_circuit_amd/csrc/ff29.cuh
@@ -184,6 +184,34 @@
         for (int i = 0; i < 261 - 32 * P::N; i++) v = v.dbl();
         return split(v.l);
     }
+    ZK_HD static void mont_to_canonical(const uint32_t *a, uint32_t *raw) {
+        static_assert(mod29(0) == 1u && PINV == MASK, "written for p = 1 (mod 2^29)");
+        static_assert(B * N - 32 * P::N == 5 && P::N == 8, "R' / R = 2^5");
+        uint64_t t[2 * N];
+        t[0] = (a[0] << 5) & MASK;
+#pragma unroll
+        for (int i = 1; i < N; i++) {
+            const int bit = B * i - 5, k = bit >> 5, sh = bit & 31;
+            const uint64_t two = (uint64_t)a[k] | ((k + 1 < P::N ? (uint64_t)a[k + 1] : 0) << 32);
+            t[i] = (uint32_t)(two >> sh) & MASK;
+        }
+#pragma unroll
+        for (int i = N; i < 2 * N; i++) t[i] = 0;
+#pragma unroll
+        for (int i = 0; i < N; i++) {
+            const uint64_t u = t[i] + MASK;
+            const uint32_t m = ~(uint32_t)u & MASK;
+#pragma unroll
+            for (int j = 1; j < N; j++) t[i + j] += (uint64_t)m * mod29(j);
+            t[i + 1] += u >> B;
+        }
+        Fp29 r;
+        uint64_t c = 0;
+#pragma unroll
+        for (int i = 0; i < N - 1; i++) { const uint64_t v = t[N + i] + c; r.l[i] = (uint32_t)v & MASK; c = v >> B; }
+        r.l[N - 1] = (uint32_t)(t[2 * N - 1] + c);
+        r.template canonical<0>().pack(raw);
+    }
     ZK_HD static Fp29 from_std_relimb(const Fp<P> &a) { return split(a.l); }
     template <int LOG> ZK_HD Fp<P> to_std_relimb() const { Fp<P> r; canonical<LOG>().pack(r.l); return r; }
 };
diff --git a/aes_zero_knowledge_proof_circuit_amd/csrc/gpu.hpp b/aes_zero_knowledge_proof_circuit_amd/csrc/gpu.hpp
--- a/aes_zero_knowledge_proof_circuit_amd/csrc/gpu.hpp
+++ b/aes_zero_knowledge_proof_circuit_amd/csrc/gpu.hpp
@@ -107,6 +107,7 @@
 MsmWorkspace *msm_workspace_create();
 void msm_workspace_destroy(MsmWorkspace *ws);
 using WorkspaceGuard = Handle<MsmWorkspace *, msm_workspace_create, msm_workspace_destroy>;
+void msm_workspace_set_throughput(MsmWorkspace *ws, bool on);
 template <class Curve> void convert_bases(Affine28<typename Curve::FqP> *dst, const Affine<typename Curve::Fq> *src, size_t n, stream_t s);
 template <class Curve>
 XYZZ<typename Curve::Fq> msm(MsmWorkspace *ws, const Affine28<typename Curve::FqP> *bases, const typename Curve::Fr *scalars, size_t n, stream_t s);
diff --git a/aes_zero_knowledge_proof_circuit_amd/csrc/kernels_msm.hip b/aes_zero_knowledge_proof_circuit_amd/csrc/kernels_msm.hip
--- a/aes_zero_knowledge_proof_circuit_amd/csrc/kernels_msm.hip
+++ b/aes_zero_knowledge_proof_circuit_amd/csrc/kernels_msm.hip
@@ -8,6 +8,7 @@
 #include <vector>
 #include "hip_util.hpp"
 #include "te28.cuh"
+#include "ff29.cuh"
 
 namespace zk {
 namespace gpu {
@@ -525,6 +526,29 @@
     quad_tree_sum<P>(pt, RQ_QUADS, quad, q);
     if (quad == 0) quad_store<P>(reinterpret_cast<uint32_t *>(out + (size_t)set * jobs + job), q, quad_load<P>(pt, q));
 }
+constexpr int RL_THREADS = 64, RL_LANES = 16, RL_JOBS = RL_THREADS / RL_LANES;
+template <class P>
+__global__ void __launch_bounds__(RL_THREADS) k_reduce_rc_lanes(const AccTE<P> *__restrict__ seg_s, const AccTE<P> *__restrict__ seg_w, int lgR, int lgC, uint32_t total_jobs, AccTE<P> *__restrict__ out) {
+    __shared__ AccTE<P> sh[RL_THREADS];
+    const uint32_t R = 1u << lgR, C = 1u << lgC, jobs = 2 * R + C;
+    const uint32_t gjob = blockIdx.x * RL_JOBS + threadIdx.x / RL_LANES, li = threadIdx.x % RL_LANES;
+    const bool live = gjob < total_jobs;
+    const uint32_t set = live ? gjob / jobs : 0, job = live ? gjob % jobs : 0;
+    const AccTE<P> *src = (job < R ? seg_w : seg_s) + ((size_t)set << (lgR + lgC));
+    uint32_t first, stride, len;
+    if (job < 2 * R) { first = (job < R ? job : job - R) << lgC; stride = 1; len = C; }
+    else { first = job - 2 * R; stride = C; len = R; }
+    if (!live) len = 0;
+    AccTE<P> acc = li < len ? src[first + (size_t)li * stride] : te_identity<P>();
+    for (uint32_t i = li + RL_LANES; i < len; i += RL_LANES) te_add<P>(acc, src[first + (size_t)i * stride]);
+    sh[threadIdx.x] = acc;
+    __syncthreads();
+    for (uint32_t half = RL_LANES / 2; half >= 1; half >>= 1) {
+        if (li < half) { te_add<P>(acc, sh[threadIdx.x + half]); if (half > 1) sh[threadIdx.x] = acc; }
+        __syncthreads();
+    }
+    if (live && li == 0) out[gjob] = acc;
+}
 ZK_HD int quad_weighted_lc(uint32_t M) { int m = 0; while ((1u << m) < M) m++; return M <= 16 ? m : (m + 1) / 2; }
 constexpr int RF_OUT = 6;
 constexpr int RT_THREADS = 256, RT_QUADS = RT_THREADS / 4;
@@ -643,6 +667,7 @@
     bool ctrl_dirty = false;
     size_t plan_n = 0, plan_pairs = 0; int plan_c = 0, plan_nwin = 0;
     bool plan_table = false; uint32_t plan_cap = BUCKET_CAP;
+    bool throughput = false;
     EventGuard ev[4] = {EventGuard(nullptr), EventGuard(nullptr), EventGuard(nullptr), EventGuard(nullptr)};
     DevPtr<uint32_t> deferred, deferred_count;
     DevPtr<uint32_t> ord_hist, ord_offs;
@@ -673,6 +698,7 @@
 }
 MsmWorkspace *msm_workspace_create() { return new MsmWorkspace(); }
 void msm_workspace_destroy(MsmWorkspace *w) { delete w; }
+void msm_workspace_set_throughput(MsmWorkspace *w, bool on) { w->throughput = on; }
 
 static void order_buckets(MsmWorkspace &S, size_t nb, uint32_t cap, hipStream_t s) {
     if (S.ctrl_dirty) HIP_CHECK(hipMemsetAsync(S.ctrl, 0, 8, s));
@@ -762,7 +788,11 @@
         if (lgC > 8) throw GpuError("msm: more than 2^19 buckets per set");
         const unsigned jobs = 2u * (1u << lgR) + (1u << lgC);
         A *rc = (A *)S.partial.p, *part = rc + (size_t)nsets * jobs;
-        hipLaunchKernelGGL((k_reduce_rc<P>), dim3((unsigned)nsets * jobs), dim3(RQ_THREADS), 0, s, (const A *)S.seg_s.p, (const A *)S.seg_w.p, lgR, lgC, rc);
+        if (S.throughput)
+            hipLaunchKernelGGL((k_reduce_rc_lanes<P>), dim3(((unsigned)nsets * jobs + RL_JOBS - 1) / RL_JOBS), dim3(RL_THREADS), 0, s, (const A *)S.seg_s.p, (const A *)S.seg_w.p, lgR, lgC,
+                               (uint32_t)nsets * jobs, rc);
+        else
+            hipLaunchKernelGGL((k_reduce_rc<P>), dim3((unsigned)nsets * jobs), dim3(RQ_THREADS), 0, s, (const A *)S.seg_s.p, (const A *)S.seg_w.p, lgR, lgC, rc);
         HIP_LAUNCH_CHECK();
         te_host_tail = !dev_wsum_out && nsets <= 4;
         hipLaunchKernelGGL((k_reduce_terms<P>), dim3((unsigned)(RF_OUT * nsets)), dim3(RT_THREADS), 0, s, (const A *)rc, lgR, lgC, part, res, te_host_tail);
@@ -1133,7 +1163,8 @@
             const uint32_t g = tile * PART_TILE + q * PART_THREADS + threadIdx.x;
             if (g >= n) continue;
             uint32_t d[PART_MAXW], raw[Fr::N + 1];
-            (g < n1 ? s1[g] : s2[g - n1]).to_raw(raw);
+            const Fr a = g < n1 ? s1[g] : s2[g - n1];
+            Fp29<typename Fr::Params>::mont_to_canonical(a.l, raw);
             raw[Fr::N] = 0;
             part_digits<Fr::N>(raw, L, d);
 #pragma unroll
diff --git a/aes_zero_knowledge_proof_circuit_amd/csrc/kernels_poly.hip b/aes_zero_knowledge_proof_circuit_amd/csrc/kernels_poly.hip
--- a/aes_zero_knowledge_proof_circuit_amd/csrc/kernels_poly.hip
+++ b/aes_zero_knowledge_proof_circuit_amd/csrc/kernels_poly.hip
@@ -12,11 +12,11 @@
 void poly_set_at(F *p, size_t idx, const F &val, stream_t s) { hipLaunchKernelGGL(k_set_at, dim3(1), dim3(64), 0, (hipStream_t)s, p, idx, val, false); HIP_LAUNCH_CHECK(); }
 void poly_add_at(F *p, size_t idx, const F &val, stream_t s) { hipLaunchKernelGGL(k_set_at, dim3(1), dim3(64), 0, (hipStream_t)s, p, idx, val, true); HIP_LAUNCH_CHECK(); }
 
-__global__ void k_scale(F *p, F sc, size_t n) { size_t i = (size_t)blockIdx.x * blockDim.x + threadIdx.x; if (i < n) p[i] = p[i] * sc; }
-void poly_scale(F *p, const F &sc, size_t n, stream_t s) { if (!n) return; hipLaunchKernelGGL(k_scale, GRID(n), 0, (hipStream_t)s, p, sc, n); HIP_LAUNCH_CHECK(); }
 using G29 = Fp29<Fr377P>;
 __device__ __forceinline__ G29 ld29(const F &x) { return G29::split(x.l); }
 __device__ __forceinline__ F st29(const G29 &g) { F r; g.template canonical<1>().pack(r.l); return r; }
+__global__ void k_scale(F *p, G29 sc, size_t n) { size_t i = (size_t)blockIdx.x * blockDim.x + threadIdx.x; if (i < n) p[i] = st29(ld29(p[i]) * sc); }
+void poly_scale(F *p, const F &sc, size_t n, stream_t s) { if (!n) return; hipLaunchKernelGGL(k_scale, GRID(n), 0, (hipStream_t)s, p, G29::twiddle_from_std(sc), n); HIP_LAUNCH_CHECK(); }
 struct LincombArgs { const F *p[8]; size_t len[8]; G29 sc[8]; int count; };
 __global__ void k_lincomb_n(F *__restrict__ out, LincombArgs a, size_t n) {
     size_t i = (size_t)blockIdx.x * blockDim.x + threadIdx.x;
@@ -87,17 +87,17 @@
 }
 
 constexpr int DL_B = 16;
-__global__ void k_divlin_local(F *__restrict__ q, const F *__restrict__ p, size_t len, F z, F *__restrict__ v, F *__restrict__ zp) {
-    if (blockIdx.x == 0 && threadIdx.x < DL_B) zp[threadIdx.x] = z.pow_u64(threadIdx.x);
+__global__ void k_divlin_local(F *__restrict__ q, const F *__restrict__ p, size_t len, F z, G29 z29, F *__restrict__ v, F *__restrict__ zp) {
+    if (blockIdx.x == 0 && threadIdx.x < DL_B) G29::twiddle_from_std(z.pow_u64(threadIdx.x)).pack(zp[threadIdx.x].l);
     const size_t t = (size_t)blockIdx.x * blockDim.x + threadIdx.x, s0 = t * DL_B;
     if (s0 >= len) return;
     const size_t e = s0 + DL_B < len ? s0 + DL_B : len;
-    F l = F::zero();
+    G29 l = G29::zero();
     for (size_t i = e; i-- > s0;) {
-        if (i + 1 < len) q[i] = l;
-        l = p[i] + z * l;
-    }
-    v[t] = l;
+        if (i + 1 < len) q[i] = st29(l);
+        l = ld29(p[i]) + l * z29;
+    }
+    v[t] = st29(l);
 }
 constexpr int DL_TOP_THREADS = 256;
 constexpr size_t DL_TOP = (size_t)DL_TOP_THREADS * DL_B;
@@ -128,15 +128,15 @@
     for (size_t i = e; i-- > s0;) { q[i] = q[i] + w * c; w = w * z; }
 }
 __global__ void __launch_bounds__(256) k_divlin_apply(F *__restrict__ q, size_t qlen, const F *__restrict__ zp_table, const F *__restrict__ carry, size_t nblocks) {
-    __shared__ F zp[DL_B];
-    if (threadIdx.x < DL_B) zp[threadIdx.x] = zp_table[threadIdx.x];
+    __shared__ G29 zp[DL_B];
+    if (threadIdx.x < DL_B) zp[threadIdx.x] = ld29(zp_table[threadIdx.x]);
     __syncthreads();
     const size_t i = (size_t)blockIdx.x * blockDim.x + threadIdx.x;
     if (i >= qlen) return;
     const size_t t = i / DL_B;
     if (t + 1 >= nblocks) return;
     const size_t e = (t + 1) * DL_B;
-    q[i] = q[i] + zp[e - 1 - i] * carry[t];
+    q[i] = st29(ld29(q[i]) + ld29(carry[t]) * zp[e - 1 - i]);
 }
 size_t divide_by_linear_scratch(size_t len) {
     size_t total = 8;
@@ -148,7 +148,7 @@
     if (len <= DL_TOP) { hipLaunchKernelGGL(k_divlin_top, dim3(1), dim3(DL_TOP_THREADS), 0, s, q, p, len, z); HIP_LAUNCH_CHECK(); return; }
     const size_t nblocks = (len + DL_B - 1) / DL_B;
     F *v = scratch, *carry = scratch + nblocks + 1, *zp = carry + nblocks + 1;
-    hipLaunchKernelGGL(k_divlin_local, GRID(nblocks), 0, s, q, p, len, z, v, zp); HIP_LAUNCH_CHECK();
+    hipLaunchKernelGGL(k_divlin_local, GRID(nblocks), 0, s, q, p, len, z, G29::twiddle_from_std(z), v, zp); HIP_LAUNCH_CHECK();
     divlin_rec(carry, v, nblocks, z.pow_u64(DL_B), zp + DL_B, s);
     hipLaunchKernelGGL(k_divlin_apply, GRID(len - 1), 0, s, q, len - 1, (const F *)zp, (const F *)carry, nblocks); HIP_LAUNCH_CHECK();
 }
@@ -162,14 +162,14 @@
 }
 
 constexpr size_t EV_CHUNK = 16, EV_COMBINE_MAX = 1024;
-__global__ void k_eval_chunks(const F *__restrict__ p, size_t len, F x, F *__restrict__ partial) {
+__global__ void k_eval_chunks(const F *__restrict__ p, size_t len, G29 x, F *__restrict__ partial) {
     size_t t = (size_t)blockIdx.x * blockDim.x + threadIdx.x;
     size_t nch = (len + EV_CHUNK - 1) / EV_CHUNK;
     if (t >= nch) return;
     size_t s0 = t * EV_CHUNK, e = s0 + EV_CHUNK < len ? s0 + EV_CHUNK : len;
-    F acc = F::zero();
-    for (size_t i = e; i-- > s0;) acc = acc * x + p[i];
-    partial[t] = acc;
+    G29 acc = G29::zero();
+    for (size_t i = e; i-- > s0;) acc = (acc * x).add_lazy(ld29(p[i]));
+    partial[t] = st29(acc.normalized());
 }
 __global__ void __launch_bounds__(256) k_eval_combine(const F *__restrict__ partial, size_t nch, F y, F *__restrict__ out) {
     __shared__ F sh[256];
@@ -192,7 +192,7 @@
     F y = x;
     do {
         size_t nch = (n + EV_CHUNK - 1) / EV_CHUNK;
-        hipLaunchKernelGGL(k_eval_chunks, GRID(nch), 0, s, src, n, y, scratch); HIP_LAUNCH_CHECK();
+        hipLaunchKernelGGL(k_eval_chunks, GRID(nch), 0, s, src, n, G29::twiddle_from_std(y), scratch); HIP_LAUNCH_CHECK();
         src = scratch; scratch += nch; n = nch; y = y.pow_u64(EV_CHUNK);
     } while (n > EV_COMBINE_MAX);
     hipLaunchKernelGGL(k_eval_combine, dim3(1), dim3(256), 0, s, src, n, y, out); HIP_LAUNCH_CHECK();
@@ -263,9 +263,10 @@
 }
 constexpr int VQ_MAX_COSETS = 3, VQ_STEP = 10;
 struct VqArgs { F *out[VQ_MAX_COSETS]; const F *tab; const F *elems; uint32_t n; int lg_n; bool unit_g[VQ_MAX_COSETS]; };
-__device__ __forceinline__ F vq_factor(const VqArgs &A, int c, int k, uint32_t j) {
-    const F e = A.elems[(size_t)j << k];
-    return A.tab[k] + (A.unit_g[c] ? e : e * A.tab[(size_t)(c + 1) * A.lg_n + k]);
+__device__ __forceinline__ F vq_node(const VqArgs &A, int c, int k, uint32_t j, const F &parent) {
+    const G29 e = ld29(A.elems[(size_t)j << k]);
+    const G29 f = ld29(A.tab[k]) + (A.unit_g[c] ? e : e * ld29(A.tab[(size_t)(c + 1) * A.lg_n + k]));
+    return st29(f.shl5() * ld29(parent));
 }
 __global__ void __launch_bounds__(1024) k_vq_top(VqArgs A, F *__restrict__ mid) {
     __shared__ F buf[2][1 << VQ_STEP];
@@ -276,7 +277,7 @@
     int cur = 0;
     for (int k = L - 1; k >= k_stop; k--) {
         const uint32_t s = A.n >> k;
-        if (t < s) buf[cur ^ 1][t] = vq_factor(A, c, k, t) * buf[cur][t & ((s >> 1) - 1)];
+        if (t < s) buf[cur ^ 1][t] = vq_node(A, c, k, t, buf[cur][t & ((s >> 1) - 1)]);
         __syncthreads();
         cur ^= 1;
     }
@@ -294,7 +295,7 @@
     int cur = 0;
     for (int k = k_hi - 1; k >= k_lo; k--) {
         const uint32_t cnt = 1u << (k_hi - k);
-        for (uint32_t m = t; m < cnt; m += 256) buf[cur ^ 1][m] = vq_factor(A, c, k, j + m * s_hi) * buf[cur][m & ((cnt >> 1) - 1)];
+        for (uint32_t m = t; m < cnt; m += 256) buf[cur ^ 1][m] = vq_node(A, c, k, j + m * s_hi, buf[cur][m & ((cnt >> 1) - 1)]);
         __syncthreads();
         cur ^= 1;
     }
@@ -322,7 +323,7 @@
     for (int c = 0; c < ncosets; c++) {
         A.unit_g[c] = g[c] == F::one();
         v = g[c];
-        for (int k = 0; k < lg_n; k++) { tab[(size_t)(c + 1) * lg_n + k] = v; v = v.sqr(); }
+        for (int k = 0; k < lg_n; k++) { G29::twiddle_from_std(v).pack(tab[(size_t)(c + 1) * lg_n + k].l); v = v.sqr(); }
     }
     h2d(scratch, tab.data(), tab.size() * sizeof(F), s_);
     A.tab = scratch; A.elems = elems; A.n = n; A.lg_n = lg_n;
@@ -341,7 +342,9 @@
     if (i >= k) return;
     const G29 v[3] = {ld29(va[i]), ld29(vb[i]), ld29(vc[i])}, w[3] = {ea, eb, ec};
     const F num = st29(G29::dot<3>(v, w));
-    out[i] = num.is_zero() ? num : num * (rb[ci[i]] * ra[ri[i]]);
+    if (num.is_zero()) { out[i] = num; return; }
+    const G29 quot = ld29(rb[ci[i]]).shl5() * ld29(ra[ri[i]]);
+    out[i] = st29(ld29(num).shl5() * quot);
 }
 void f_evals_from_tables(F *out, const F *va, const F *vb, const F *vc, const F &ea, const F &eb, const F &ec, const F *ra, const F *rb, const uint32_t *ri, const uint32_t *ci, size_t k,
                          stream_t s) {
@@ -387,19 +390,20 @@
     hipLaunchKernelGGL(k_z_evals_h, GRID(n), 0, (hipStream_t)s, out, z, n, m, num_witness); HIP_LAUNCH_CHECK();
 }
 __global__ void k_q1_combine(F *__restrict__ h1, F *__restrict__ g1, const F *__restrict__ q0, const F *__restrict__ q1, const F *__restrict__ q3, const F *__restrict__ mask,
-                             F inv2, F inv2zeta, size_t n) {
+                             G29 inv2, G29 inv2zeta, size_t n) {
     size_t i = (size_t)blockIdx.x * blockDim.x + threadIdx.x;
     if (i >= n) return;
-    const F a = q1[i], b = q3[i], c = q0[i];
-    const F q_mid = (a - b) * inv2zeta;
-    const F q_hi = ((c - q_mid) - (a + b) * inv2) * inv2;
-    const F m_lo = mask[i], m_mid = mask[n + i], m_hi = mask[2 * n + i];
-    h1[i] = q_mid + q_hi + m_mid + m_hi;
-    h1[n + i] = q_hi + m_hi;
-    if (i >= 1) g1[i - 1] = c + m_lo + m_mid + m_hi;
+    const G29 a = ld29(q1[i]), b = ld29(q3[i]), c = ld29(q0[i]);
+    const G29 q_mid = a.template sub<1>(b) * inv2zeta;
+    const G29 half = (a + b) * inv2;
+    const G29 q_hi = c.template sub<2>(q_mid).template sub<2>(half) * inv2;
+    const G29 m_lo = ld29(mask[i]), m_mid = ld29(mask[n + i]), m_hi = ld29(mask[2 * n + i]);
+    h1[i] = (q_mid + q_hi + m_mid + m_hi).template to_std_relimb<2>();
+    h1[n + i] = st29(q_hi + m_hi);
+    if (i >= 1) g1[i - 1] = st29(c + m_lo + m_mid + m_hi);
 }
 void q1_combine(F *h1, F *g1, const F *q0, const F *q1, const F *q3, const F *mask, const F &inv2, const F &inv2zeta, size_t n, stream_t s) {
-    hipLaunchKernelGGL(k_q1_combine, GRID(n), 0, (hipStream_t)s, h1, g1, q0, q1, q3, mask, inv2, inv2zeta, n); HIP_LAUNCH_CHECK();
+    hipLaunchKernelGGL(k_q1_combine, GRID(n), 0, (hipStream_t)s, h1, g1, q0, q1, q3, mask, G29::twiddle_from_std(inv2), G29::twiddle_from_std(inv2zeta), n); HIP_LAUNCH_CHECK();
 }
 __global__ void k_coset_scale(F *__restrict__ out, const F *__restrict__ in, F g, size_t in_len, size_t n) {
     size_t t = (size_t)blockIdx.x * blockDim.x + threadIdx.x;
diff --git a/aes_zero_knowledge_proof_circuit_amd/csrc/kernels_witness.hip b/aes_zero_knowledge_proof_circuit_amd/csrc/kernels_witness.hip
--- a/aes_zero_knowledge_proof_circuit_amd/csrc/kernels_witness.hip
+++ b/aes_zero_knowledge_proof_circuit_amd/csrc/kernels_witness.hip
@@ -1,4 +1,5 @@
 #include <mutex>
+#include "ff29.cuh"
 #include "hip_util.hpp"
 #include "trace_layout.h"
 
@@ -580,19 +581,26 @@
 void bits_to_field(F *out, const uint8_t *z, size_t n, stream_t s) { if (!n) return; hipLaunchKernelGGL(k_bits_to_field, GRID(n), 0, (hipStream_t)s, out, z, n); HIP_LAUNCH_CHECK(); }
 
 __global__ void k_t_partials(F *__restrict__ partial, uint32_t nseg, const uint32_t *__restrict__ seg_start, const uint32_t *__restrict__ seg_end, const uint32_t *__restrict__ row,
-                             const uint8_t *__restrict__ mat, const int64_t *__restrict__ coeff, const F *__restrict__ r_alpha, F eta_a, F eta_b, F eta_c) {
+                             const uint8_t *__restrict__ mat, const int64_t *__restrict__ coeff, const F *__restrict__ r_alpha, Fp29<Fr377P> eta_a, Fp29<Fr377P> eta_b, Fp29<Fr377P> eta_c) {
+    using G29 = Fp29<Fr377P>;
     uint32_t sgi = blockIdx.x * blockDim.x + threadIdx.x;
     if (sgi >= nseg) return;
-    F acc = F::zero();
+    G29 s[3] = {G29::zero(), G29::zero(), G29::zero()};
     for (uint32_t i = seg_start[sgi]; i < seg_end[sgi]; i++) {
-        F eta = mat[i] == 0 ? eta_a : (mat[i] == 1 ? eta_b : eta_c);
-        long long c = coeff[i];
-        F term = eta * r_alpha[row[i]];
-        if (c == 1) acc = acc + term;
-        else if (c == -1) acc = acc - term;
-        else acc = acc + term * small_to_field(c);
-    }
-    partial[sgi] = acc;
+        const long long c = coeff[i];
+        const G29 r = G29::split(r_alpha[row[i]].l);
+        G29 term = r;
+        if (c == -1) term = G29::zero().template sub<1>(r);
+        else if (c != 1) term = r.shl5() * G29::split(small_to_field(c).l);
+        const uint8_t m = mat[i];
+        if (m == 0) s[0] = s[0] + term;
+        else if (m == 1) s[1] = s[1] + term;
+        else s[2] = s[2] + term;
+    }
+    const G29 eta[3] = {eta_a, eta_b, eta_c};
+    F out;
+    G29::dot<3>(s, eta).template canonical<1>().pack(out.l);
+    partial[sgi] = out;
 }
 __global__ void k_t_columns(F *__restrict__ out, uint32_t n, const uint32_t *__restrict__ col_seg_ptr, const F *__restrict__ partial) {
     uint32_t h = blockIdx.x * blockDim.x + threadIdx.x;
@@ -615,7 +623,12 @@
 }
 void t_evals(F *out, uint32_t n, F *partial, uint32_t nseg, const uint32_t *col_seg_ptr, const uint32_t *seg_start, const uint32_t *seg_end, const uint32_t *heavy, uint32_t n_heavy,
              const uint32_t *row, const uint8_t *mat, const int64_t *coeff, const F *r_alpha, const F &eta_a, const F &eta_b, const F &eta_c, stream_t s) {
-    if (nseg) { hipLaunchKernelGGL(k_t_partials, GRID(nseg), 0, (hipStream_t)s, partial, nseg, seg_start, seg_end, row, mat, coeff, r_alpha, eta_a, eta_b, eta_c); HIP_LAUNCH_CHECK(); }
+    if (nseg) {
+        using G29 = Fp29<Fr377P>;
+        hipLaunchKernelGGL(k_t_partials, GRID(nseg), 0, (hipStream_t)s, partial, nseg, seg_start, seg_end, row, mat, coeff, r_alpha, G29::twiddle_from_std(eta_a), G29::twiddle_from_std(eta_b),
+                           G29::twiddle_from_std(eta_c));
+        HIP_LAUNCH_CHECK();
+    }
     hipLaunchKernelGGL(k_t_columns, GRID(n), 0, (hipStream_t)s, out, n, col_seg_ptr, partial); HIP_LAUNCH_CHECK();
     if (n_heavy) { hipLaunchKernelGGL(k_t_heavy, dim3(n_heavy), dim3(256), 0, (hipStream_t)s, out, heavy, col_seg_ptr, partial); HIP_LAUNCH_CHECK(); }
 }
diff --git a/aes_zero_knowledge_proof_circuit_amd/csrc/marlin.cpp b/aes_zero_knowledge_proof_circuit_amd/csrc/marlin.cpp
--- a/aes_zero_knowledge_proof_circuit_amd/csrc/marlin.cpp
+++ b/aes_zero_knowledge_proof_circuit_amd/csrc/marlin.cpp
@@ -830,6 +830,7 @@
     gpu::set_device(device);
     std::lock_guard<std::mutex> busy(cx.in_use);
     cx.throughput = throughput;
+    gpu::msm_workspace_set_throughput(cx.msm_ws, throughput);
     ProofRun R(*this, cx, host_trace, msg, len, key, iv, zk_seed);
     prove_round1(R);
     prove_round2(R);
```
